# rwl/CSparse.py

Hardware: AMD Instinct MI355X
Metric: cs_gaxpy achieved HBM GB/s (algorithmic bytes / time), 5M x 5M CSC, 64 nnz/col (higher is better)
Workload: dtype f64; 1 GPU; cs_gaxpy y += A x on G-rand: 5000000 x 5000000 CSC, 64 distinct rows per column drawn uniformly from [0, n), ascending (SURVEY 8d), int32 indices, fp64 values; one independent matrix per GPU; row_draw=uniform, n=5000000, nnz=320000000, kernel=gaxpy_tiled, plan_key_bytes=3, parallelism=independent matrices, 1 per GPU, no data-path collective

## Files before the change

### csparse.py_amd/_csx.py

```python
import ctypes as C
import os

import numpy as np

_HERE = os.path.dirname(os.path.abspath(__file__))
LIB_PATH = os.environ.get("CSX_LIB") or os.path.join(_HERE, "libcsx.so")

OK, EINVAL, EZEROPIVOT, ENOTSPD, ERUNTIME = 0, 1, 2, 3, 4
TRI_L, TRI_LT, TRI_U, TRI_UT = 0, 1, 2, 3
GAXPY_AUTO, GAXPY_EXACT, GAXPY_WAVE, GAXPY_TILED, GAXPY_ATOMIC = 0, 1, 2, 3, 4

H = C.c_uint64
_i32p = C.POINTER(C.c_int32)
_f64p = C.POINTER(C.c_double)
_vp = C.c_void_p

_PROTOS = {
    "csx_init": [C.c_int],
    "csx_finalize": [],
    "csx_sync": [],
    "csx_set_stream": [_vp],
    "csx_device_info": [C.c_char_p, C.c_int, C.POINTER(C.c_int), C.POINTER(C.c_int64)],
    "csx_compress": [C.c_int32, C.c_int32, C.c_int64, _i32p, _i32p, _f64p, C.POINTER(H)],
    "csx_add": [H, H, C.c_double, C.c_double, C.POINTER(H)],
    "csx_dupl": [H, C.POINTER(H)],
    "csx_drop": [H, C.c_int, C.c_double, C.POINTER(H)],
    "csx_permute": [H, _i32p, _i32p, C.c_int, C.POINTER(H)],
    "csx_symperm": [H, _i32p, C.c_int, C.POINTER(H)],
    "csx_schol": [H, _i32p, _i32p],
    "csx_order_nd_host": [C.c_int32, _i32p, _i32p, _i32p],
    "csx_norm1": [H, _f64p],
    "csx_cholsol_set_order": [H, C.c_int],
    "csx_cholsol_growth": [H, _f64p],
    "csx_cholsol_sn_info": [H, _i32p, _i32p, _i32p, _i32p, _f64p],
    "csx_cholsol_sn_geometry": [H, C.POINTER(C.c_int64), C.c_int32, _i32p],
    "csx_cholsol_sn_launches": [H, C.POINTER(C.c_int64), C.c_int32, _i32p],
    "csx_csc_invalidate": [H],
    "csx_set_option": [C.c_char_p, C.c_int],
    "csx_get_option": [C.c_char_p, C.POINTER(C.c_int)],
    "csx_gaxpy_host": [C.c_int32, C.c_int32, _i32p, _i32p, _f64p, _f64p, _f64p],
    "csx_csc_col_block": [H, C.c_int32, C.c_int32, C.POINTER(H)],
    "csx_mem_trim": [],
    "csx_mem_info": [C.POINTER(C.c_int64), C.POINTER(C.c_int64), C.POINTER(C.c_int64)],
    "csx_timer_start": [],
    "csx_timer_stop": [_f64p],
    "csx_csc_upload": [C.c_int32, C.c_int32, _i32p, _i32p, _f64p, C.POINTER(H)],
    "csx_csc_alloc": [C.c_int32, C.c_int32, C.c_int32, C.c_int, C.POINTER(H)],
    "csx_csc_wrap": [C.c_int32, C.c_int32, C.c_int32, _vp, _vp, _vp, C.POINTER(H)],
    "csx_csc_info": [H, _i32p, _i32p, _i32p, C.POINTER(C.c_int)],
    "csx_csc_download": [H, _i32p, _i32p, _f64p],
    "csx_csc_ptrs": [H, C.POINTER(_vp), C.POINTER(_vp), C.POINTER(_vp)],
    "csx_free": [H],
    "csx_vec_alloc": [C.c_int64, C.POINTER(H)],
    "csx_vec_upload": [_f64p, C.c_int64, C.POINTER(H)],
    "csx_vec_wrap": [_vp, C.c_int64, C.POINTER(H)],
    "csx_vec_download": [H, _f64p, C.c_int64],
    "csx_vec_write": [H, _f64p, C.c_int64],
    "csx_vec_fill": [H, C.c_double],
    "csx_vec_copy": [H, H],
    "csx_vec_ptr": [H, C.POINTER(_vp), C.POINTER(C.c_int64)],
    "csx_ivec_upload": [_i32p, C.c_int64, C.POINTER(H)],
    "csx_ivec_download": [H, _i32p, C.c_int64],
    "csx_gaxpy": [H, H, H, C.c_int],
    "csx_gaxpy_prepare": [H, C.c_int],
    "csx_gaxpy_block": [H, H, H, C.c_int32, C.c_int],
    "csx_residual_block": [H, H, H, H, C.c_int32, C.c_int, _f64p, _f64p],
    "csx_residual_host": [C.c_int32, C.c_int32, _i32p, _i32p, _f64p, C.c_int32, C.c_int, _f64p, _f64p, _f64p, _f64p, _f64p],
    "csx_residual_sym_block": [H, H, H, H, C.c_int32, _f64p, _f64p],
    "csx_residual_sym_host": [C.c_int32, _i32p, _i32p, _f64p, C.c_int32, _f64p, _f64p, _f64p, _f64p, _f64p],
    "csx_norm1_sym": [H, _f64p],
    "csx_block_add_cols": [H, H, H, C.c_int64, C.c_int32, _i32p],
    "csx_block_select_cols": [H, H, C.c_int64, C.c_int32, _i32p],
    "csx_transpose": [H, C.c_int, C.POINTER(H)],
    "csx_cumsum": [H, H, C.c_int64, C.POINTER(C.c_int64)],
    "csx_prim_limits": [_i32p],
    "csx_prim_scan": [_i32p, _i32p, C.c_int64, C.c_int, C.POINTER(C.c_int64)],
    "csx_prim_suffix_min": [_i32p, C.c_int64],
    "csx_prim_expand_columns": [_i32p, C.c_int32, C.c_int32, _i32p],
    "csx_prim_boundaries": [_vp, C.c_int64, C.c_int32, _i32p, C.c_int],
    "csx_prim_sort": [_vp, _vp, _f64p, C.c_int64, C.c_uint32, _vp, _vp, _f64p, _i32p, C.c_int32, _i32p, C.c_int32, C.c_int],
    "csx_prim_sort_info": [C.POINTER(C.c_int64), C.c_int32],
    "csx_multiply": [H, H, C.POINTER(H)],
    "csx_spgemm_limits": [_i32p],
    "csx_spgemm_info": [C.POINTER(C.c_int64), C.c_int32, _i32p],
    "csx_tri_analyse": [H, C.c_int, C.POINTER(H)],
    "csx_tri_info": [H, _i32p, _i32p, _i32p],
    "csx_tri_solve": [H, H, C.c_int32],
    "csx_tri_set_order": [H, C.c_int],
    "csx_tri_solve_list": [H, _f64p, C.POINTER(C.c_int)],
    "csx_cholsol_solve_list": [H, _f64p, C.POINTER(C.c_int)],
    "csx_tri_order_info": [H, _i32p, _f64p],
    "csx_tri_components": [H, _i32p],
    "csx_tri_limits": [_i32p],
    "csx_tri_route_info": [H, C.c_int32, C.POINTER(C.c_int64), C.c_int32, _i32p],
    "csx_tri_launches": [H, C.POINTER(C.c_int64), C.c_int32, _i32p],
    "csx_cholsol_tri_route_info": [H, C.c_int, C.c_int32, C.POINTER(C.c_int64), C.c_int32, _i32p],
    "csx_cholsol_tri_launches": [H, C.c_int, C.POINTER(C.c_int64), C.c_int32, _i32p],
    "csx_permute_vec": [H, H, H, C.c_int32, C.c_int32, C.c_int],
    "csx_lusol_solve": [H, H, H, H, H, H, C.c_int32, C.POINTER(C.c_int)],
    "csx_lusol_solve_trans": [H, H, H, H, H, H, C.c_int32, C.POINTER(C.c_int)],
    "csx_schol_host": [C.c_int32, _i32p, _i32p, _i32p, _i32p],
    "csx_counts_host": [C.c_int32, C.c_int32, _i32p, _i32p, _i32p, _i32p, C.c_int, _i32p],
    "csx_chol": [H, _i32p, _i32p, _i32p, C.POINTER(H)],
    "csx_chol_info": [_i32p, _f64p],
    "csx_cholsol_plan": [H, _i32p, C.POINTER(H)],
    "csx_cholsol_factor": [H, C.c_int, C.POINTER(H), C.POINTER(H)],
    "csx_cholsol_factor_info": [C.POINTER(C.c_int32), C.POINTER(C.c_double), C.POINTER(C.c_double), C.POINTER(C.c_double)],
    "csx_cholsol_solve": [H, H, C.c_int32],
    "csx_cholsol_graph_info": [H, _i32p, _f64p],
    "csx_cholsol_info": [H, _i32p, _i32p, _i32p],
    "csx_qr_host": [C.c_int32, C.c_int32, C.c_int32, _i32p, _i32p, _f64p, _i32p, _i32p, _i32p, _i32p, C.c_int32, C.c_int32,
                    _i32p, _i32p, _f64p, _i32p, _i32p, _f64p, _f64p],
    "csx_qr_apply_host": [C.c_int32, _i32p, _i32p, _f64p, _f64p, C.c_int, _f64p],
    "csx_lu_blocks": [H, C.c_double, C.POINTER(H), C.POINTER(H), _i32p, C.POINTER(C.c_int)],
    "csx_block_limits": [_i32p],
    "csx_prim_components": [C.c_int32, _i32p, _i32p, C.c_int, C.c_int, C.c_int, _i32p, _vp, _i32p, _i32p, _i32p, _i32p, _i32p,
                            C.POINTER(C.c_int)],
    "csx_lu_etree": [H, C.c_double, C.POINTER(H), C.POINTER(H), _i32p, C.POINTER(C.c_int)],
    "csx_updown": [H, C.c_int, C.c_int32, _i32p, _f64p, _i32p, C.POINTER(C.c_int)],
    "csx_updown_block": [H, H, _i32p, _i32p, C.c_int, _i32p],
    "csx_updown_block_info": [_i32p, _i32p, _i32p, _f64p],
    "csx_updown_block_classes": [_i32p, _i32p],
    "csx_chol_inverse": [H, C.POINTER(H)],
    "csx_chol_inverse_info": [_i32p, _i32p, C.POINTER(C.c_int64), _f64p],
    "csx_csc_diag": [H, H],
    "csx_ldl_inverse": [H, H, C.POINTER(H)],
    "csx_slu_inverse": [H, H, C.POINTER(H), C.POINTER(H)],
    "csx_inverse_at": [H, H, H, H, C.c_int64, _i32p, _i32p, H, C.POINTER(C.c_int64)],
    "csx_spsolve": [H, H, _i32p, C.c_int, C.c_int, C.POINTER(H)],
    "csx_happly": [H, H, H, C.c_int32, C.c_int],
    "csx_sqr_host": [C.c_int32, C.c_int32, _i32p, _i32p, _i32p, _i32p, _i32p, _i32p, C.POINTER(C.c_int32),
                     C.POINTER(C.c_int64), C.POINTER(C.c_int64)],
    "csx_qr_blocks": [H, _i32p, _i32p, _i32p, C.c_int32, C.POINTER(H), C.POINTER(H), _f64p, C.POINTER(C.c_int)],
    "csx_gaxpy_plan_info": [H, C.POINTER(C.c_int), C.POINTER(C.c_int), C.POINTER(C.c_int)],
    "csx_gaxpy_plan_shape": [H, C.POINTER(C.c_int), C.POINTER(C.c_double)],
    "csx_gaxpy_plan_geometry": [H, C.POINTER(C.c_int64)],
    "csx_gaxpy_plan_groups": [H, _i32p],
    "csx_lu_host": [C.c_int32, _i32p, _i32p, _f64p, C.c_double, C.POINTER(_i32p), C.POINTER(_i32p),
                    C.POINTER(_f64p), C.POINTER(_i32p), C.POINTER(_i32p), C.POINTER(_f64p), _i32p],
    "csx_comm_unique_id": [C.POINTER(C.c_uint8)],
    "csx_comm_init": [C.c_int, C.c_int, C.POINTER(C.c_uint8)],
    "csx_comm_finalize": [],
    "csx_comm_info": [C.POINTER(C.c_int), C.POINTER(C.c_int), C.POINTER(C.c_int)],
    "csx_comm_barrier": [],
    "csx_comm_allreduce_host": [_f64p, C.c_int, C.c_int],
    "csx_comm_bcast_host": [_vp, C.c_int64, C.c_int],
    "csx_comm_bcast_csc": [C.POINTER(H), C.c_int],
    "csx_comm_bcast_vec": [H, C.c_int],
    "csx_comm_reduce_scatter_vec": [H, H],
    "csx_comm_allreduce_vec": [H],
    "csx_comm_scatter_blocks": [H, H, C.c_int64, C.c_int],
    "csx_comm_gather_blocks": [H, H, C.c_int64, C.c_int],
    "csx_block_cols": [H, C.c_int64, C.c_int32, C.c_int32, C.c_int32, H, C.c_int],
    "csx_gaxpy_sharded_plan": [H, C.POINTER(H)],
    "csx_gaxpy_sharded_rows": [H, _i32p, _i32p],
    "csx_gaxpy_sharded": [H, H, H, C.c_int],
    "csx_gaxpy_sharded_plan_for": [H, C.c_int, C.POINTER(H)],
    "csx_gaxpy_sharded_piece": [H, C.c_int, H],
    "csx_gaxpy_sharded_buffers": [H, C.POINTER(_vp), C.POINTER(_vp), C.POINTER(C.c_int64)],
    "csx_gaxpy_sharded_sum": [H, C.c_int, C.c_int, H],
    "csx_maxtrans": [H, C.c_int64, _i32p, _i32p],
    "csx_scc": [H, _i32p, _i32p, _i32p],
    "csx_dmperm": [H, C.c_int64, _i32p, _i32p, _i32p, _i32p, _i32p, _i32p, _i32p],
    "csx_dmperm_times": [_f64p],
    "csx_dmperm_rounds": [C.POINTER(C.c_int64)],
    "csx_btf_split": [H, _i32p, _i32p, _i32p, C.c_int32, _i32p, _i32p, _i32p, _i32p, _i32p, C.POINTER(H), C.POINTER(H)],
    "csx_btf_plan": [H, H, H, _i32p, _i32p, _i32p, _i32p, _i32p, C.c_int32, C.POINTER(H)],
    "csx_btf_solve": [H, H, H, C.c_int32],
    "csx_btf_solve_trans": [H, H, H, C.c_int32],
    "csx_btf_info": [H, C.POINTER(C.c_int64)],
    "csx_btf_limits": [_i32p],
    "csx_btf_refactor": [H, H, H, H, C.POINTER(C.c_int), _f64p, C.POINTER(C.c_int64)],
    "csx_btf_refactor_dx": [H, _f64p],
    "csx_lu_refactor_plan": [H, H, H, _i32p, _i32p, C.POINTER(H)],
    "csx_lu_refactor": [H, H, C.POINTER(C.c_int), _f64p, C.POINTER(C.c_int64)],
    "csx_chol_refactor_plan": [H, H, _i32p, C.POINTER(H)],
    "csx_chol_refactor": [H, H, C.POINTER(C.c_int), _i32p],
    "csx_chol_refactor_info": [C.POINTER(C.c_double), C.POINTER(C.c_double)],
    "csx_chol_refactor_window": [H, C.POINTER(C.c_int32)],
    "csx_chol_limits": [_i32p],
    "csx_cholsol_forest_plan": [C.c_int, C.c_int32, C.c_int32, C.c_int, C.c_int, C.POINTER(C.c_int32)],
    "csx_lu_refactor_host": [C.c_int32, _i32p, _i32p, _f64p, _i32p, _i32p, _i32p, _f64p, _i32p, _i32p, _f64p,
                             C.POINTER(C.c_int), _f64p],
    "csx_assemble_plan_host": [C.c_int32, C.c_int32, C.c_int64, _i32p, _i32p, _i32p, _i32p, _i32p, _i32p, _i32p],
    "csx_assemble_host": [C.c_int32, _i32p, _i32p, _f64p, _f64p],
    "csx_assemble_plan": [C.c_int32, C.c_int32, C.c_int64, _i32p, _i32p, C.POINTER(H)],
    "csx_assemble_matrix": [H, H, C.POINTER(H)],
    "csx_assemble": [H, H, H],
    "csx_assemble_plan_info": [H, C.POINTER(C.c_int64)],
    "csx_assemble_pullback": [H, H, H],
    "csx_assemble_pullback_host": [C.c_int32, C.c_int64, _i32p, _i32p, _f64p, _f64p],
    "csx_pattern_outer": [H, H, H, C.c_int32, C.c_int, C.c_double, H],
    "csx_pattern_outer_host": [C.c_int32, C.c_int32, _i32p, _i32p, C.c_int32, C.c_int, C.c_double, _f64p, _f64p, _f64p],
    "csx_pattern_outer_limits": [C.POINTER(C.c_int64)],
    "csx_multiply_plan_count": [C.c_int32, C.c_int32, C.c_int32, _i32p, _i32p, _i32p, _i32p, C.POINTER(C.c_int64),
                                C.POINTER(C.c_int64)],
    "csx_multiply_plan_host": [C.c_int32, C.c_int32, C.c_int32, _i32p, _i32p, _i32p, _i32p, _i32p, _i32p, _i32p, _i32p],
    "csx_multiply_fold_host": [C.c_int32, _i32p, _i32p, _f64p, _f64p, _f64p],
    "csx_multiply_plan": [H, H, C.POINTER(H)],
    "csx_multiply_plan_matrix": [H, H, H, H, C.POINTER(H)],
    "csx_multiply_plan_run": [H, H, H, H, H],
    "csx_multiply_plan_info": [H, C.POINTER(C.c_int64)],
    "csx_add_plan_host": [C.c_int32, C.c_int32, C.c_int32, C.POINTER(_i32p), C.POINTER(_i32p), _i32p, _i32p, _i32p, _i32p, _i32p],
    "csx_add_fold_host": [C.c_int32, C.c_int32, _i32p, _i32p, _i32p, _f64p, C.POINTER(_f64p), _f64p],
    "csx_add_plan": [C.c_int32, C.POINTER(H), C.POINTER(H)],
    "csx_add_plan_matrix": [H, _f64p, C.POINTER(H), C.POINTER(H)],
    "csx_add_plan_run": [H, _f64p, C.POINTER(H), H],
    "csx_add_plan_info": [H, C.POINTER(C.c_int64)],
    "csx_ldl_factor": [H, _i32p, _i32p, _i32p, C.c_double, C.POINTER(H), C.POINTER(C.c_int)],
    "csx_ldl_refactor": [H, H, C.c_double, C.POINTER(C.c_int)],
    "csx_ldl_parts": [H, C.POINTER(H), C.POINTER(H)],
    "csx_ldl_info": [H, C.POINTER(C.c_int64)],
    "csx_ldl_stats": [H, _f64p],
    "csx_ldl_window": [C.POINTER(C.c_int32)],
    "csx_block_div_rows": [H, H, C.c_int64, C.c_int32],
    "csx_ldl_host": [C.c_int32, _i32p, _i32p, _f64p, _i32p, _i32p, _i32p, C.c_double, _f64p, _f64p, C.POINTER(C.c_int64)],
    "csx_schur_factor": [H, _i32p, _i32p, _i32p, C.c_int32, C.c_double, C.POINTER(H), C.POINTER(C.c_int)],
    "csx_schur_refactor": [H, H, C.c_double, C.POINTER(C.c_int)],
    "csx_schur_parts": [H, C.POINTER(H), C.POINTER(H), C.POINTER(H)],
    "csx_schur_info": [H, C.POINTER(C.c_int64)],
    "csx_schur_stats": [H, _f64p],
    "csx_schur_host": [C.c_int32, _i32p, _i32p, _f64p, _i32p, _i32p, _i32p, C.c_int32, C.c_double, _f64p, _f64p, _f64p,
                       C.POINTER(C.c_int64)],
    "csx_slu_factor": [H, _i32p, _i32p, _i32p, _i32p, C.c_double, C.POINTER(H), C.POINTER(C.c_int)],
    "csx_slu_refactor": [H, H, C.c_double, C.POINTER(C.c_int)],
    "csx_slu_parts": [H, C.POINTER(H), C.POINTER(H)],
    "csx_slu_info": [H, C.POINTER(C.c_int64)],
    "csx_slu_stats": [H, _f64p],
    "csx_slu_window": [C.POINTER(C.c_int32), C.POINTER(C.c_int32)],
    "csx_slu_host": [C.c_int32, _i32p, _i32p, _f64p, _i32p, _i32p, _i32p, _i32p, C.c_double, _f64p, _f64p, C.POINTER(C.c_int64)],
    "csx_slu_batch_factor": [H, H, C.c_int32, _f64p, C.POINTER(H), C.POINTER(C.c_int)],
    "csx_slu_batch_refactor": [H, H, _f64p, C.POINTER(C.c_int)],
    "csx_slu_batch_norm1": [H, H, C.c_int32, _f64p],
    "csx_slu_batch_solve": [H, H, C.c_int32, C.c_int],
    "csx_slu_batch_info": [H, C.POINTER(C.c_int64), C.POINTER(C.c_int64)],
    "csx_slu_batch_stats": [H, _f64p],
    "csx_slu_batch_member": [H, C.c_int32, _f64p, _f64p],
    "csx_slu_batch_limits": [_i32p],
    "csx_ldl_batch_factor": [H, H, C.c_int32, _f64p, C.POINTER(H), C.POINTER(C.c_int)],
    "csx_ldl_batch_refactor": [H, H, _f64p, C.POINTER(C.c_int)],
    "csx_ldl_batch_norm1": [H, H, C.c_int32, _f64p],
    "csx_ldl_batch_solve": [H, H, C.c_int32],
    "csx_ldl_batch_info": [H, C.POINTER(C.c_int64), C.POINTER(C.c_int64)],
    "csx_ldl_batch_stats": [H, _f64p],
    "csx_ldl_batch_member": [H, C.c_int32, _f64p, _f64p],
    "csx_ldl_batch_d": [H, _f64p],
    "csx_ldl_batch_limits": [_i32p],
    "csx_hqr_symbolic_host": [C.c_int32, C.c_int32, C.c_int32, _i32p, _i32p, _i32p, _i32p, _i32p, _i32p, C.c_int32, C.c_int32,
                              _i32p, _i32p, _i32p, _i32p],
    "csx_hqr_host": [C.c_int32, C.c_int32, C.c_int32, _i32p, _i32p, _f64p, _i32p, _i32p, _i32p, _i32p, C.c_int32, C.c_int32,
                     _i32p, _i32p, _f64p, _i32p, _i32p, _f64p, _f64p],
    "csx_hqr_factor": [H, _i32p, _i32p, _i32p, _i32p, C.c_int32, C.POINTER(H), C.POINTER(C.c_int)],
    "csx_hqr_refactor": [H, H, C.POINTER(C.c_int)],
    "csx_hqr_parts": [H, C.POINTER(H), C.POINTER(H), C.POINTER(H)],
    "csx_hqr_info": [H, C.POINTER(C.c_int64)],
    "csx_hqr_stats": [H, _f64p],
    "csx_hqr_window": [C.POINTER(C.c_int32), C.POINTER(C.c_int32)],
    "csx_level_schedule": [C.c_int32, _i32p, C.c_int32, C.c_int32, C.POINTER(C.c_int64), C.c_int64, _i32p, C.POINTER(C.c_int32)],
    "csx_gmres_limits": [_i32p],
    "csx_gs_work_len": [C.c_int64, C.c_int32, C.c_int32, C.POINTER(C.c_int64)],
    "csx_gs_project": [H, C.c_int32, H, H, C.c_int64, C.c_int32, _i32p, C.c_int, _f64p],
    "csx_gs_update": [H, C.c_int32, H, H, C.c_int64, C.c_int32, _i32p, C.c_int, _f64p, _f64p],
    "csx_gs_scale": [H, H, C.c_int32, H, C.c_int64, C.c_int32, _i32p, _f64p],
    "csx_gs_combine": [H, C.c_int32, H, H, C.c_int64, C.c_int32, _i32p, _f64p, _i32p],
    "csx_gs_host": [C.c_int, C.c_int64, C.c_int32, C.c_int32, _f64p, _f64p, _i32p, C.c_int, _f64p, _i32p, _f64p],
    "csx_bgs_limits": [_i32p],
    "csx_bgs_work_len": [C.c_int64, C.c_int32, C.c_int32, C.c_int32, C.POINTER(C.c_int64)],
    "csx_bgs_gram": [H, C.c_int32, C.c_int32, H, C.c_int32, H, C.c_int64, C.c_int, _f64p],
    "csx_bgs_update": [H, C.c_int32, C.c_int32, H, C.c_int32, H, C.c_int64, _f64p],
    "csx_bgs_combine": [H, C.c_int32, C.c_int32, H, C.c_int32, H, C.c_int64, _f64p],
    "csx_bgs_host": [C.c_int, C.c_int64, C.c_int32, C.c_int32, C.c_int32, _f64p, _f64p, C.c_int, _f64p, _f64p],
    "csx_gen_grand": [C.c_int32, C.c_int32, C.c_uint64, C.POINTER(H)],
    "csx_gen_grand_uniform": [C.c_int32, C.c_int32, C.c_uint64, C.POINTER(H)],
    "csx_gen_gspd": [C.c_int32, C.c_int32, C.c_uint64, C.POINTER(H)],
    "csx_gen_vec": [C.c_int64, C.c_uint64, C.c_double, C.c_double, C.POINTER(H)],
    "csx_gen_rhs": [C.c_int32, C.c_int32, C.c_int32, C.POINTER(H)],
}

_lib = None
_ready = False


class CsxError(RuntimeError):
    pass


class NotPositiveDefinite(ArithmeticError):
    pass


def _share_torch_hip_runtime():
    import sys
    if "torch" in sys.modules:
        return "torch (already imported)"
    want = os.environ.get("CSX_SHARE_TORCH_HIP")
    if want == "0" or (want is None and (int(os.environ.get("WORLD_SIZE", "1")) <= 1
                                         or os.environ.get("CSX_COMM_BACKEND") != "gloo")):
        return None
    import importlib.util
    spec = importlib.util.find_spec("torch")
    if spec is None or not spec.origin:
        return None
    path = os.path.join(os.path.dirname(spec.origin), "lib", "libamdhip64.so")
    if not os.path.exists(path):
        return None
    C.CDLL(path, mode=C.RTLD_GLOBAL)
    return path


HIP_RUNTIME = None


def load():
    global _lib, HIP_RUNTIME
    if _lib is None:
        if not os.path.exists(LIB_PATH):
            raise ImportError("libcsx.so is not built: run `python csparse.py_amd/build.py` "
                              "(hipcc --offload-arch=gfx950); there is no CPU fallback")
        HIP_RUNTIME = _share_torch_hip_runtime()
        lib = C.CDLL(LIB_PATH)
        for name, args in _PROTOS.items():
            fn = getattr(lib, name)
            fn.argtypes = args
            fn.restype = C.c_int
        lib.csx_last_error.restype = C.c_char_p
        lib.csx_last_error.argtypes = []
        lib.csx_host_free.restype = None
        lib.csx_host_free.argtypes = [_vp]
        _lib = lib
    return _lib


def ldl_window():
    out = C.c_int32(0)
    check(load().csx_ldl_window(C.byref(out)), "csx_ldl_window")
    return out.value


_CHOL_LIMITS = ("CH_ACC", "CH_NARROW", "CH_SMALL_TREE", "CD_MAX", "CC_ACC", "CC_MAP", "CC_RUN_MIN", "CC_RUN_MAX", "CC_WAVES",
                "SN_MIN_WIDTH")


def chol_limits():
    out = (C.c_int32 * 16)()
    check(load().csx_chol_limits(out), "csx_chol_limits")
    d = {name: int(out[k]) for k, name in enumerate(_CHOL_LIMITS)}
    d["windows"] = tuple(int(out[k]) for k in range(10, 15))
    d["max_need"] = int(out[15])
    return d


FOREST_PLAN_KINDS = ("General", "EmitEqual", "Programs", "BlockListExact", "EmitRagged", "BlockListLite")


def cholsol_forest_plan(sparse, min_bs, max_bs, exact, dense_blocks):
    kind = C.c_int32(-1)
    check(load().csx_cholsol_forest_plan(int(sparse), min_bs, max_bs, int(exact), int(dense_blocks), C.byref(kind)),
          "csx_cholsol_forest_plan")
    return FOREST_PLAN_KINDS[kind.value]


def slu_window():
    a, b = C.c_int32(0), C.c_int32(0)
    check(load().csx_slu_window(C.byref(a), C.byref(b)), "csx_slu_window")
    return a.value, b.value


SLU_BATCH_LIMITS = ("MAX_MEMBERS", "WALK_WAVES", "SOLVE_THREADS", "SOLVE_FETCH", "RUN_WAVES", "RUN_FETCH")


def slu_batch_limits():
    out = (C.c_int32 * len(SLU_BATCH_LIMITS))()
    check(load().csx_slu_batch_limits(out), "csx_slu_batch_limits")
    return {name: int(out[k]) for k, name in enumerate(SLU_BATCH_LIMITS)}


def ldl_batch_limits():
    out = (C.c_int32 * len(SLU_BATCH_LIMITS))()
    check(load().csx_ldl_batch_limits(out), "csx_ldl_batch_limits")
    return {name: int(out[k]) for k, name in enumerate(SLU_BATCH_LIMITS)}


def hqr_window():
    a, b = C.c_int32(0), C.c_int32(0)
    check(load().csx_hqr_window(C.byref(a), C.byref(b)), "csx_hqr_window")
    return a.value, b.value


def level_schedule(level_ptr, waves, run_levels, work=None, run_work=0):
    lp = i32(level_ptr)
    nlev = len(lp) - 1
    out, count = np.zeros(3 * max(nlev, 1), np.int32), C.c_int32(0)
    w = None if work is None else np.ascontiguousarray(work, np.int64)
    check(load().csx_level_schedule(nlev, pi(lp), waves, run_levels, None if w is None else w.ctypes.data_as(C.POINTER(C.c_int64)),
                                    run_work, pi(out), C.byref(count)), "csx_level_schedule")
    return [(bool(out[3 * t]), int(out[3 * t + 1]), int(out[3 * t + 2])) for t in range(count.value)]


SN_GEOMETRY_PLAN = ("chunk", "has_relaxed", "matrix_cores", "leaf_subtrees", "leaf_cols", "leaf_tasks", "leaf_slots",
                    "fundamental", "relaxed")
SN_GEOMETRY_DIR = ("steps", "tasks", "max_step_tasks", "cut_lines", "slots", "narrow", "medium", "wide", "one_triangle_steps")
SN_LAUNCHES = ("outside_wg", "outside", "thin1", "thin2", "thin4", "thin8", "thin16", "thin32", "combine", "mfma_w128",
               "mfma_leaf_ct1", "mfma_leaf_ct4", "mfma_ct1", "mfma_ct4", "tri16", "tri32", "tri64", "leaf", "use0")


def _sn_fields(fn, plan, what):
    n = C.c_int32(0)
    check(fn(plan, None, 0, C.byref(n)), what)
    out = (C.c_int64 * n.value)()
    check(fn(plan, out, n.value, C.byref(n)), what)
    return list(out)


def cholsol_sn_geometry(plan):
    v = _sn_fields(lib().csx_cholsol_sn_geometry, plan, "csx_cholsol_sn_geometry")
    a, b = len(SN_GEOMETRY_PLAN), len(SN_GEOMETRY_DIR)
    assert len(v) == a + 2 * b
    g = dict(zip(SN_GEOMETRY_PLAN, v[:a]))
    g["fwd"] = dict(zip(SN_GEOMETRY_DIR, v[a:a + b]))
    g["bwd"] = dict(zip(SN_GEOMETRY_DIR, v[a + b:]))
    return g


def cholsol_sn_launches(plan):
    v = _sn_fields(lib().csx_cholsol_sn_launches, plan, "csx_cholsol_sn_launches")
    k = len(SN_LAUNCHES)
    assert len(v) == 2 * k
    return {"fwd": dict(zip(SN_LAUNCHES, v[:k])), "bwd": dict(zip(SN_LAUNCHES, v[k:]))}


TRI_LIMITS = ("NARROW", "CHB", "CH_SUF", "TRW_MIN_ROW", "TRW_MAX_RHS", "TR64_MIN_RHS", "TR64_RUN", "TR64_RUN_MIN", "TC_MAX_N",
              "TC_THREADS", "COMP_MIN_COUNT", "COMP_MAX_ROWS", "PUSH_MAX_RHS", "FEW_MAX_RHS", "FEW_CPW", "COMP_LDS_MAX", "FEW_TILE_LDS",
              "WINDOW_LDS_MAX", "COLUMNS_LDS_MAX", "CHAIN_LINKS_NUM", "CHAIN_LINKS_DEN", "CHAIN_LEVELS_NUM", "WCOL_WIDE_ENTRIES",
              "WCHAIN_WIDE_ENTRIES", "WINDOW_SLACK", "STRIP_SHORT_COLS", "TL_WAVES_MAX", "LV_MAX_ROUNDS", "LV_DEVICE_MIN_TERMS",
              "LAUNCH_COUNTERS")
TRI_ROUTES = ("Ragged", "CompPush", "FewLds", "Few", "Local", "WColumns", "WColChain", "Columns", "ColChain", "Sequential", "Levels")
TRI_ROUTE_INFO = ("route", "lds", "grid", "G", "waves", "tile_rows", "chunks", "window", "threads", "rounds", "mate",
                  "band", "links", "col_state", "levels", "sequential", "chain_ok", "ncomp", "comp_max", "push_terms", "few_cpw",
                  "few_rows", "few_terms", "guard", "schedule", "comps_found", "comp_rows_found", "kind", "n", "terms")
TRI_LAUNCHES = ("level", "levels_one_wg", "chain", "sequential", "local_fwd", "local_bwd", "few_fwd", "few_bwd", "few_lds_fwd",
                "few_lds_bwd", "push_fwd", "push_bwd", "ragged", "columns_l", "columns_u", "colchain_lt", "colchain_ut",
                "wcolumns_256", "wcolumns_1024", "wcolchain_lt_2", "wcolchain_lt_12", "wcolchain_ut_2", "wcolchain_ut_12",
                "level_rows", "run_prefix_rows", "levels_rows_one_wg", "level_rows64", "run_prefix64", "levels_rows64_one_wg",
                "level_of")


def tri_limits():
    out = (C.c_int32 * 32)()
    check(load().csx_tri_limits(out), "csx_tri_limits")
    return {name: int(out[k]) for k, name in enumerate(TRI_LIMITS)}


def tri_route_info(plan, nrhs, cholsol=None):
    if cholsol is None:
        v = _sn_fields(lambda h, out, cap, n: lib().csx_tri_route_info(h, nrhs, out, cap, n), plan, "csx_tri_route_info")
    else:
        v = _sn_fields(lambda h, out, cap, n: lib().csx_cholsol_tri_route_info(h, cholsol, nrhs, out, cap, n), plan,
                       "csx_cholsol_tri_route_info")
    assert len(v) == len(TRI_ROUTE_INFO)
    d = dict(zip(TRI_ROUTE_INFO, v))
    d["route"] = TRI_ROUTES[d["route"]]
    return d


def tri_launches(plan, cholsol=None):
    if cholsol is None:
        v = _sn_fields(lib().csx_tri_launches, plan, "csx_tri_launches")
    else:
        v = _sn_fields(lambda h, out, cap, n: lib().csx_cholsol_tri_launches(h, cholsol, out, cap, n), plan,
                       "csx_cholsol_tri_launches")
    assert len(v) == len(TRI_LAUNCHES)
    return {k: c for k, c in zip(TRI_LAUNCHES, v) if c}


PRIM_LIMITS = ("SCAN_TILE", "SM_TILE", "RS_TILE", "RS_BINS", "RS_DESC_STARTS", "RS_SEGS", "RS_CHUNK_MIN", "RS_CHUNK_DIV",
               "EXPAND_GRID_MAX")
SORT_INSTANCES = ("none", "keys", "a", "v", "av_flat_flat", "av_flat_packed", "av_packed_packed", "av_packed_flat", "short_first",
                  "short_middle", "short_last")
SORT_INFO = ("bits", "passes", "widths", "nblocks", "chunk", "nchunks", "packed", "k16", "key_misalign", "instances", "count")


def prim_limits():
    out = (C.c_int32 * len(PRIM_LIMITS))()
    check(load().csx_prim_limits(out), "csx_prim_limits")
    return {name: int(out[k]) for k, name in enumerate(PRIM_LIMITS)}


SPGEMM_LIMITS = ("SG_SEG", "SG_THREADS", "SG_DENSE_MAX", "SG_GLOBAL_WGS", "SG_HASH_MAXP", "HASH_LIMIT0", "HASH_LIMIT1", "HASH_LIMIT2",
                 "HASH_LIMIT3", "HASH_LIMIT4", "HASH_LIMIT5", "HASH_LIMIT6", "HASH_LIMIT7", "H2_MAXSEG", "H2_MAXLEN", "H2_MAXP",
                 "H1_SEG", "H1_MAXP", "H1_UN", "SGO_MAX", "SGO_SLOTS0", "SGO_CNT0", "SGO_SLOTS1", "SGO_CNT1", "SGO_SLOTS2", "SGO_CNT2",
                 "SGO_DENSE_WAVES", "SG_GRID_PER_CU", "INFO_FIELDS", "SGO_WAVES0", "SGO_WAVES1", "SGO_WAVES2", "SG_UN",
                 "SG_MIN_SLOTS", "SG_LDS_BUDGET", "SG_WGS_PER_CU_MAX", "SG_HASH_BINS", "SG_NARROW_BINS", "LAUNCH_SITES")
SPGEMM_SITES = (("products",) + tuple("spgemm_%s_%s" % (r, k) for r in ("symbolic", "values", "pattern")
                                      for k in ("dense", "hash", "global"))
                + tuple("hash1_%s_%d" % (v, b) for v in ("pattern", "values") for b in range(8))
                + tuple("hash2_%s_%d" % (v, b) for v in ("pattern", "values") for b in range(6))
                + ("compact", "dup_cols", "ordered2_0", "ordered2_1", "ordered2_2", "ordered_dense"))


def spgemm_limits():
    out = (C.c_int32 * 40)()
    check(load().csx_spgemm_limits(out), "csx_spgemm_limits")
    return {name: int(out[k]) for k, name in enumerate(SPGEMM_LIMITS)}


def spgemm_info():
    n = C.c_int32(0)
    out = (C.c_int64 * 256)()
    check(load().csx_spgemm_info(out, 256, C.byref(n)), "csx_spgemm_info")
    v, k = [int(x) for x in out[:n.value]], len(SPGEMM_SITES)
    assert n.value == 40 + 2 * k
    cnt, grid = v[40:40 + k], v[40 + k:]
    return {"bins": tuple(v[:32]), "one_pass": v[32], "global_wgs": v[33], "cus": v[34], "ordered": v[35], "classes": tuple(v[36:40]),
            "launches": {s: c for s, c in zip(SPGEMM_SITES, cnt) if c},
            "grids": {s: g for s, c, g in zip(SPGEMM_SITES, cnt, grid) if c}}


GMRES_LIMITS = ("GS_CHUNK", "GS_FAN", "GS_GROUP", "GS_TILE")
GS_PROJECT, GS_UPDATE, GS_SCALE, GS_COMBINE = 0, 1, 2, 3


def gmres_limits():
    out = (C.c_int32 * len(GMRES_LIMITS))()
    check(load().csx_gmres_limits(out), "csx_gmres_limits")
    return {name: int(out[k]) for k, name in enumerate(GMRES_LIMITS)}


def gs_work_len(rows, nrhs, nblocks):
    out = C.c_int64(0)
    check(load().csx_gs_work_len(rows, nrhs, nblocks, C.byref(out)), "csx_gs_work_len")
    return out.value


def gs_host(op, V, W, mask, coef=None, length=None, negate=False, nv=None):
    V = np.array(V, dtype=np.float64)
    nb, rows, k = V.shape
    nv = nb if nv is None else nv
    W = None if W is None else np.array(W, dtype=np.float64).reshape(rows, k)
    m = i32(mask)
    cf = None if coef is None else f64(coef)
    ln = None if length is None else i32(length)
    out = {GS_PROJECT: np.full((nv, k), np.nan), GS_UPDATE: np.full(k, np.nan), GS_SCALE: None,
           GS_COMBINE: np.full((rows, k), np.nan)}[op]
    check(load().csx_gs_host(op, rows, k, nv, pd(V), pd(W), pi(m), 1 if negate else 0, pd(cf), pi(ln), pd(out)), "csx_gs_host")
    return {GS_PROJECT: out, GS_UPDATE: (W, out), GS_SCALE: V, GS_COMBINE: out}[op]


PATTERN_OUTER_LIMITS = ("PO_LANES", "PO_CHUNK", "PO_WAVE_CHUNK", "PO_FLIGHT", "PO_KEPT")


def pattern_outer_limits():
    out = (C.c_int64 * len(PATTERN_OUTER_LIMITS))()
    check(load().csx_pattern_outer_limits(out), "csx_pattern_outer_limits")
    return {name: int(out[k]) for k, name in enumerate(PATTERN_OUTER_LIMITS)}


def pattern_outer_host(m, n, p, i, U, V, nrhs, alpha=1.0, sym=False):
    p, i = i32(p), i32(i)
    U, V = f64(np.asarray(U, dtype=np.float64).reshape(-1)), f64(np.asarray(V, dtype=np.float64).reshape(-1))
    out = np.full(max(int(p[n]), 1), np.nan)
    check(load().csx_pattern_outer_host(m, n, pi(p), pi(i), nrhs, 1 if sym else 0, float(alpha), pd(U), pd(V), pd(out)),
          "csx_pattern_outer_host")
    return out[:int(p[n])]


def assemble_pullback_host(sp, src, g):
    sp, src, g = i32(sp), i32(src), f64(g)
    nnz, nz = len(sp) - 1, len(src)
    out = np.full(max(nz, 1), np.nan)
    check(load().csx_assemble_pullback_host(nnz, nz, pi(sp), pi(src), pd(g), pd(out)), "csx_assemble_pullback_host")
    return out[:nz]


BGS_LIMITS = ("GS_CHUNK", "GS_FAN", "BGS_MAXW", "BGS_GROUP", "BGS_TILE")
BGS_GRAM, BGS_UPDATE, BGS_COMBINE = 0, 1, 2


def bgs_limits():
    out = (C.c_int32 * len(BGS_LIMITS))()
    check(load().csx_bgs_limits(out), "csx_bgs_limits")
    return {name: int(out[k]) for k, name in enumerate(BGS_LIMITS)}


def bgs_work_len(rows, b, q, nblocks):
    out = C.c_int64(0)
    check(load().csx_bgs_work_len(rows, b, q, nblocks, C.byref(out)), "csx_bgs_work_len")
    return out.value


def bgs_host(op, V, W=None, coef=None, negate=False, q=None):
    V = np.array(V, dtype=np.float64)
    nv, rows, b = V.shape
    W = None if W is None else np.array(W, dtype=np.float64)
    W = W[:, None] if W is not None and W.ndim == 1 else W
    cf = None if coef is None else f64(coef)
    q = W.shape[1] if W is not None else (int(q) if q is not None else cf.shape[-1])
    out = {BGS_GRAM: np.full((nv, b, q), np.nan), BGS_UPDATE: None, BGS_COMBINE: np.full((rows, q), np.nan)}[op]
    check(load().csx_bgs_host(op, rows, b, q, nv, pd(V), pd(W), 1 if negate else 0, pd(cf), pd(out)), "csx_bgs_host")
    return W if op == BGS_UPDATE else out


def _u32(a):
    return None if a is None else np.array(a, dtype=np.uint32)


def _vptr(a):
    return None if a is None else a.ctypes.data_as(_vp)


def prim_scan(values, in_place=False):
    a = np.array(values, dtype=np.int32)
    out, total = np.full(len(a) + 1, -1, np.int32), C.c_int64(-1)
    check(lib().csx_prim_scan(pi(a), pi(out), len(a), 1 if in_place else 0, C.byref(total)), "csx_prim_scan")
    return out, total.value, (None if in_place else a)


def prim_suffix_min(values):
    p = np.array(values, dtype=np.int32)
    check(lib().csx_prim_suffix_min(pi(p), len(p)), "csx_prim_suffix_min")
    return p


def prim_expand_columns(Ap, fill=-1):
    p = np.array(Ap, dtype=np.int32)
    col = np.full(int(p[-1]), fill, np.int32)
    check(lib().csx_prim_expand_columns(pi(p), len(p) - 1, len(col), pi(col)), "csx_prim_expand_columns")
    return col, p


def prim_boundaries(sorted_key, nkeys, misalign_words=0, fill=-1):
    k = _u32(sorted_key)
    ptr = np.full(nkeys + 1, fill, np.int32)
    check(lib().csx_prim_boundaries(_vptr(k), len(k), nkeys, pi(ptr), misalign_words), "csx_prim_boundaries")
    return ptr, k


def prim_sort(key, a=None, v=None, key_limit=0xFFFFFFFF, want_key=True, expand_ptr=None, nkeys=None, misalign_words=0):
    k, aa = _u32(key), _u32(a)
    vv = None if v is None else np.array(v, dtype=np.float64)
    xp = None if expand_ptr is None else np.array(expand_ptr, dtype=np.int32)
    n = len(k)
    ok = np.full(n, 0xDEADBEEF, np.uint32) if want_key else None
    oa = np.full(n, 0xDEADBEEF, np.uint32) if (aa is not None or xp is not None) else None
    ov = np.full(n, -777.0, np.float64) if vv is not None else None
    op = np.full(nkeys + 1, -1, np.int32) if nkeys is not None else None
    check(lib().csx_prim_sort(_vptr(k), _vptr(aa), pd(vv), n, key_limit, _vptr(ok), _vptr(oa), pd(ov), pi(xp),
                              0 if xp is None else len(xp) - 1, pi(op), 0 if nkeys is None else nkeys, misalign_words),
          "csx_prim_sort")
    return {"out_key": ok, "out_a": oa, "out_v": ov, "out_ptr": op, "key": k, "a": aa, "v": vv, "expand_ptr": xp}


def prim_sort_info():
    out = (C.c_int64 * 17)()
    check(load().csx_prim_sort_info(out, 17), "csx_prim_sort_info")
    v = [int(x) for x in out]
    passes = v[1]
    return {"bits": v[0], "passes": passes, "widths": tuple(v[2:2 + passes]), "nblocks": v[6], "chunk": v[7], "nchunks": v[8],
            "packed": v[9], "k16": v[10], "key_misalign": v[11], "instances": tuple(SORT_INSTANCES[i] for i in v[12:12 + passes]),
            "count": v[16]}


BLOCK_LIMITS = ("LU_MAX_M", "LU_MIN_COMPONENTS", "QR_MAX_M", "QR_MIN_COMPONENTS", "HAPPLY_MAX_LEVELS")


def block_limits():
    out = (C.c_int32 * len(BLOCK_LIMITS))()
    check(load().csx_block_limits(out), "csx_block_limits")
    return {name: int(out[k]) for k, name in enumerate(BLOCK_LIMITS)}


BTF_LIMITS = ("BTF_SMALL", "RF_MAX", "RF_WAVES", "RHS_TILE", "TERM_CHUNK", "TERM_GROUP")


def btf_limits():
    out = (C.c_int32 * len(BTF_LIMITS))()
    check(load().csx_btf_limits(out), "csx_btf_limits")
    return {name: int(out[k]) for k, name in enumerate(BTF_LIMITS)}


def prim_components(n, p, i, skip_first=0, skip_last=0, order=0):
    pp, ii = np.array(p, dtype=np.int32), np.array(i, dtype=np.int32)
    root, nodes, cop = np.full(n, -7, np.int32), np.full(n, 0xDEADBEEF, np.uint32), np.full(n, -7, np.int32)
    first, count = np.full(n, -7, np.int32), np.full(n, -7, np.int32)
    ncomp, maxc, bad = C.c_int32(-1), C.c_int32(-1), C.c_int(-1)
    check(lib().csx_prim_components(n, pi(pp), pi(ii), skip_first, skip_last, order, pi(root), _vptr(nodes), pi(first), pi(count),
                                    pi(cop), C.byref(ncomp), C.byref(maxc), C.byref(bad)), "csx_prim_components")
    out = {"ncomp": ncomp.value, "maxc": maxc.value, "malformed": bad.value, "p": pp, "i": ii,
           "root": None, "nodes": None, "first": None, "count": None, "comp_of_pos": None}
    if not bad.value:
        out.update(root=root, nodes=nodes, first=first[:ncomp.value], count=count[:ncomp.value], comp_of_pos=cop)
    return out


def exported_symbols():
    return sorted(list(_PROTOS) + ["csx_last_error", "csx_host_free"])


def check(status, what=""):
    if status == OK:
        return
    if status == EZEROPIVOT:
        raise ZeroDivisionError("float division by zero")
    if status == ENOTSPD:
        raise NotPositiveDefinite(what or "matrix is not positive definite")
    if status == EINVAL:
        raise ValueError("libcsx: bad argument" + (" in " + what if what else ""))
    raise CsxError("libcsx %s: %s" % (what, load().csx_last_error().decode("utf-8", "replace")))


def init(device=None):
    global _ready
    lib = load()
    if not _ready:
        if device is None:
            device = int(os.environ.get("CSX_DEVICE", os.environ.get("LOCAL_RANK", "0")))
        st = lib.csx_init(int(device))
        if st != OK:
            raise CsxError("csx_init(%d) failed: %s -- the MI355X path has no CPU fallback"
                           % (device, lib.csx_last_error().decode("utf-8", "replace")))
        _ready = True
    return lib


def lib():
    return init()


def i32(a):
    return np.ascontiguousarray(a, dtype=np.int32)


def f64(a):
    return np.ascontiguousarray(a, dtype=np.float64)


def pi(a):
    return None if a is None else a.ctypes.data_as(_i32p)


def pd(a):
    return None if a is None else a.ctypes.data_as(_f64p)


def new_handle():
    return H(0)


def free(h):
    if h and _lib is not None and _ready:
        _lib.csx_free(h)


def sync():
    check(lib().csx_sync(), "csx_sync")


def device_info():
    name = C.create_string_buffer(256)
    cus = C.c_int(0)
    mem = C.c_int64(0)
    check(lib().csx_device_info(name, 256, C.byref(cus), C.byref(mem)), "csx_device_info")
    return name.value.decode(), cus.value, mem.value


class option(object):

    def __init__(self, name, value):
        self.name, self.value = name.encode(), int(value)

    def __enter__(self):
        old = C.c_int(0)
        check(lib().csx_get_option(self.name, C.byref(old)), "csx_get_option")
        self.old = old.value
        check(lib().csx_set_option(self.name, self.value), "csx_set_option")
        return self

    def __exit__(self, *exc):
        check(lib().csx_set_option(self.name, self.old), "csx_set_option")
        return False


class Timer(object):

    def __enter__(self):
        check(lib().csx_timer_start(), "csx_timer_start")
        self.ms = None
        return self

    def __exit__(self, *exc):
        ms = C.c_double(0.0)
        check(lib().csx_timer_stop(C.byref(ms)), "csx_timer_stop")
        self.ms = ms.value
        return False
```

### csparse.py_amd/csrc/csx_gaxpy_tiled.hip

```cpp
#include <cstdint>
#include <cstdlib>

#include "csx_internal.h"

namespace csx {

constexpr int TL_WAVES = 4, TL_NG = 5;
constexpr int TL_GROUP = 256;
constexpr int TL_LDS_BYTES = 160 * 1024 - 256;
constexpr int TL_LDS_ROWS = TL_LDS_BYTES / 8 - 2;
typedef uint32_t u32x4 __attribute__((ext_vector_type(4)));
typedef uint32_t u32x3 __attribute__((ext_vector_type(3)));
typedef u32x3 u32x3_a4 __attribute__((aligned(4)));
typedef double f64x2 __attribute__((ext_vector_type(2)));

__global__ __launch_bounds__(256) void k_tile_keys(int64_t nnz, const int32_t *__restrict__ Ai,
                                                   const int32_t *__restrict__ col, int rb_bits, int32_t row_block,
                                                   int32_t slab_cols, int32_t nslab, uint32_t *__restrict__ tile_id,
                                                   uint32_t *__restrict__ packed) {
    int64_t p = (int64_t)blockIdx.x * blockDim.x + threadIdx.x;
    if (p >= nnz) return;
    const uint32_t i = (uint32_t)Ai[p], j = (uint32_t)col[p];
    const uint32_t s = j / (uint32_t)slab_cols, lc = j - s * (uint32_t)slab_cols;
    const uint32_t b = i / (uint32_t)row_block, lr = i - b * (uint32_t)row_block;
    tile_id[p] = b * (uint32_t)nslab + s;
    packed[p] = (lc << rb_bits) | lr;
}

__global__ __launch_bounds__(256) void k_padded_lengths(int64_t ntiles, const int32_t *__restrict__ sptr,
                                                        int32_t *__restrict__ ngroups) {
    int64_t t = (int64_t)blockIdx.x * blockDim.x + threadIdx.x;
    if (t < ntiles) ngroups[t] = (sptr[t + 1] - sptr[t] + TL_GROUP - 1) / TL_GROUP;
}

__global__ __launch_bounds__(256) void k_group_info(int64_t ntiles, int32_t nslab, const int32_t *__restrict__ sptr,
                                                    const int32_t *__restrict__ gptr, uint32_t *__restrict__ info) {
    int64_t t = (int64_t)blockIdx.x * blockDim.x + threadIdx.x;
    if (t >= ntiles) return;
    const int32_t len = sptr[t + 1] - sptr[t];
    const uint32_t slab = (uint32_t)(t % nslab);
    int32_t g = gptr[t];
    for (int32_t left = len; left > 0; left -= TL_GROUP, g++) info[g] = (slab << 9) | (uint32_t)min(left, TL_GROUP);
}

__global__ __launch_bounds__(256) void k_interleave(int64_t nnz, const uint32_t *__restrict__ stid,
                                                    const int32_t *__restrict__ sptr, const int32_t *__restrict__ gptr,
                                                    const uint32_t *__restrict__ skey, const double *__restrict__ sval,
                                                    uint32_t *__restrict__ okey, double *__restrict__ oval) {
    int64_t q = (int64_t)blockIdx.x * blockDim.x + threadIdx.x;
    if (q >= nnz) return;
    const uint32_t t = stid[q];
    const int32_t e = (int32_t)(q - sptr[t]);
    const int32_t g = e / TL_GROUP, w = e % TL_GROUP;
    const int64_t gbase = ((int64_t)gptr[t] + g) * TL_GROUP;
    const int l = w & 63, k = w >> 6;
    if (okey) okey[gbase + l * 4 + k] = skey[q];
    oval[gbase + (k >> 1) * 128 + l * 2 + (k & 1)] = sval[q];
}

__global__ __launch_bounds__(256) void k_run_span(int64_t nnz, const uint32_t *__restrict__ stid,
                                                  const int32_t *__restrict__ sptr, const uint32_t *__restrict__ skey,
                                                  int rb_bits, int *too_wide) {
    int64_t q = (int64_t)blockIdx.x * blockDim.x + threadIdx.x;
    if (q >= nnz) return;
    const int32_t e = (int32_t)(q - sptr[stid[q]]);
    const int64_t first = q - (e & 63);
    if ((skey[q] >> rb_bits) - (skey[first] >> rb_bits) >= 512u) *too_wide = 1;
}

__global__ __launch_bounds__(256) void k_interleave24(int64_t nnz, const uint32_t *__restrict__ stid,
                                                      const int32_t *__restrict__ sptr, const int32_t *__restrict__ gptr,
                                                      const uint32_t *__restrict__ skey, int rb_bits,
                                                      uint8_t *__restrict__ okey, uint32_t *__restrict__ obase) {
    int64_t q = (int64_t)blockIdx.x * blockDim.x + threadIdx.x;
    if (q >= nnz) return;
    const uint32_t t = stid[q];
    const int32_t e = (int32_t)(q - sptr[t]);
    const int32_t g = e / TL_GROUP, w = e % TL_GROUP;
    const int l = w & 63, k = w >> 6;
    const uint32_t rmask = (1u << rb_bits) - 1u;
    const uint32_t col = skey[q] >> rb_bits, col0 = skey[q - l] >> rb_bits;
    const uint32_t v = (skey[q] & rmask) | ((col - col0) << 15);
    const int64_t gg = (int64_t)gptr[t] + g;
    uint8_t *o = okey + gg * (TL_GROUP * 3) + l * 12 + k * 3;
    o[0] = (uint8_t)v;
    o[1] = (uint8_t)(v >> 8);
    o[2] = (uint8_t)(v >> 16);
    if (l == 0) obase[gg * 4 + k] = col;
}

__global__ __launch_bounds__(256) void k_fill_key24(uint8_t *p, int64_t nslots, uint32_t v) {
    int64_t i = (int64_t)blockIdx.x * blockDim.x + threadIdx.x;
    const int64_t stride = (int64_t)gridDim.x * blockDim.x;
    for (; i < nslots; i += stride) {
        p[3 * i] = (uint8_t)v;
        p[3 * i + 1] = (uint8_t)(v >> 8);
        p[3 * i + 2] = (uint8_t)(v >> 16);
    }
}

__global__ __launch_bounds__(256) void k_fill_keys(uint32_t *p, int64_t n, uint32_t v) {
    int64_t i = (int64_t)blockIdx.x * blockDim.x + threadIdx.x;
    const int64_t stride = (int64_t)gridDim.x * blockDim.x;
    for (; i < n; i += stride) p[i] = v;
}

struct KeyRegs {
    u32x4 kk;
    u32x4 base;
    uint32_t info;
};
struct ValRegs {
    f64x2 v0, v1;
};

constexpr int TP_KEYS2 = 1;
constexpr int TP_FULLSTEP = 2;
constexpr int TP_KEY12 = 4;
constexpr int TP_BULKTILE = 8;
constexpr int TP_ALL = 15;

template <bool NT, bool K24, bool KEY12>
__device__ __forceinline__ KeyRegs load_keys_t(const uint32_t *__restrict__ key, const uint32_t *__restrict__ info,
                                               const uint32_t *__restrict__ base, int32_t g, int lane) {
    KeyRegs r;
    if (K24) {
        const uint32_t *kp = key + (int64_t)g * (TL_GROUP * 3 / 4) + 3 * lane;
        if (KEY12) {
            const u32x3 k = __builtin_nontemporal_load(reinterpret_cast<const u32x3_a4 *>(kp));
            r.kk.x = k.x;
            r.kk.y = k.y;
            r.kk.z = k.z;
        } else {
            r.kk.x = __builtin_nontemporal_load(kp);
            r.kk.y = __builtin_nontemporal_load(kp + 1);
            r.kk.z = __builtin_nontemporal_load(kp + 2);
        }
        r.kk.w = 0;
        r.base = *reinterpret_cast<const u32x4 *>(base + 4 * (int64_t)g);
    } else {
        const uint32_t *kp = key + (int64_t)g * TL_GROUP + 4 * lane;
        r.kk = NT ? __builtin_nontemporal_load(reinterpret_cast<const u32x4 *>(kp)) : *reinterpret_cast<const u32x4 *>(kp);
        r.base = u32x4{0, 0, 0, 0};
    }
    r.info = info[g];
    return r;
}

template <bool NT>
__device__ __forceinline__ ValRegs load_vals_t(const double *__restrict__ val, int32_t g, int lane) {
    ValRegs r;
    const f64x2 *vp = reinterpret_cast<const f64x2 *>(val + (int64_t)g * TL_GROUP + 2 * lane);
    r.v0 = NT ? __builtin_nontemporal_load(vp) : *vp;
    r.v1 = NT ? __builtin_nontemporal_load(vp + 64) : vp[64];
    return r;
}

template <bool K24>
__device__ __forceinline__ u32x4 unpack_keys(const KeyRegs &k) {
    if (!K24) return k.kk;
    const uint32_t ka = k.kk.x, kb = k.kk.y, kc = k.kk.z;
    u32x4 r;
    r.x = ka & 0xFFFFFFu;
    r.y = (ka >> 24) | ((kb & 0xFFFFu) << 8);
    r.z = (kb >> 16) | ((kc & 0xFFu) << 16);
    r.w = kc >> 8;
    return r;
}

template <int HOW>
__device__ __forceinline__ double load_x(const double *p) {
    if (HOW == 1) return __hip_atomic_load(p, __ATOMIC_RELAXED, __HIP_MEMORY_SCOPE_AGENT);
    if (HOW == 2) return __builtin_nontemporal_load(p);
    return *p;
}

constexpr int tile_batch(int threads) { return threads > 256 ? 4 : 8; }

template <int T>
__device__ __forceinline__ void tile_fill(double *ytile, const double *__restrict__ src, int32_t rows) {
    constexpr int NB = tile_batch(T);
    const int tid = threadIdx.x;
    const int32_t head = (rows > 0 && (reinterpret_cast<uintptr_t>(src) & 8)) ? 1 : 0;
    const int32_t npairs = (rows - head) >> 1;
    const f64x2 *s2 = reinterpret_cast<const f64x2 *>(src + head);
    double *d = ytile + head;
    for (int32_t p0 = 0; p0 < npairs; p0 += NB * T) {
        f64x2 v[NB];
        int32_t q[NB];
#pragma unroll
        for (int i = 0; i < NB; i++) {
            const int32_t p = p0 + i * T + tid;
            q[i] = p < npairs ? p : npairs - 1;
            v[i] = s2[q[i]];
        }
#pragma unroll
        for (int i = 0; i < NB; i++) {
            d[2 * q[i]] = v[i].x;
            d[2 * q[i] + 1] = v[i].y;
        }
    }
    if (tid == 0 && head) ytile[0] = src[0];
    if (tid == T - 1 && ((rows - head) & 1)) ytile[rows - 1] = src[rows - 1];
}

template <int T>
__device__ __forceinline__ void tile_drain(const double *ytile, double *__restrict__ dst, int32_t rows) {
    const int tid = threadIdx.x;
    const int32_t head = (rows > 0 && (reinterpret_cast<uintptr_t>(dst) & 8)) ? 1 : 0;
    const int32_t npairs = (rows - head) >> 1;
    f64x2 *d2 = reinterpret_cast<f64x2 *>(dst + head);
    const double *s = ytile + head;
    constexpr int NB = tile_batch(T);
    for (int32_t p0 = 0; p0 < npairs; p0 += NB * T) {
        f64x2 v[NB];
        int32_t q[NB];
#pragma unroll
        for (int i = 0; i < NB; i++) {
            const int32_t p = p0 + i * T + tid;
            q[i] = p < npairs ? p : npairs - 1;
            v[i].x = s[2 * q[i]];
            v[i].y = s[2 * q[i] + 1];
        }
#pragma unroll
        for (int i = 0; i < NB; i++) d2[q[i]] = v[i];
    }
    if (tid == 0 && head) dst[0] = ytile[0];
    if (tid == T - 1 && ((rows - head) & 1)) dst[rows - 1] = ytile[rows - 1];
}

template <int VARIANT, int NW, int NG, bool K24, int PARTS>
struct TiledStep {
    static constexpr bool GATHER = !(VARIANT & 1) || VARIANT >= 5, ATOMIC = VARIANT != 3;
    static constexpr bool STREAM_NT = VARIANT != 2;
    static constexpr uint32_t CMASK = VARIANT == 5 ? 32767u : (VARIANT == 4 ? 255u : 0xffffffffu);
    static constexpr int XLOAD = VARIANT == 6 ? 1 : 0;
    static constexpr bool RING = VARIANT == 7;
    static constexpr int KD = (PARTS & TP_KEYS2) ? 2 : 1;
    static constexpr int NK = KD + 1;
    static constexpr int PERIOD = NK == 3 ? 6 : 2;
    static constexpr int STRIDE = NG * NW;

    static __device__ __forceinline__ int32_t clamp_group(int32_t gq, int32_t g0, int32_t gend, int32_t wave_s, int32_t wave_v) {
        int32_t gg = gq < gend ? gq : gend - 1;
        if (RING) gg = g0 + ((gg - g0) & 31);
        return gg - wave_s + wave_v;
    }
    static __device__ __forceinline__ void load_key_set(KeyRegs (&r)[NG], const uint32_t *__restrict__ key,
                                                        const uint32_t *__restrict__ info, const uint32_t *__restrict__ base,
                                                        int32_t g, int32_t g0, int32_t gend, int32_t wave_s, int32_t wave_v,
                                                        int lane) {
#pragma unroll
        for (int j = 0; j < NG; j++)
            r[j] = load_keys_t<STREAM_NT, K24, (PARTS & TP_KEY12) != 0>(key, info, base,
                                                                         clamp_group(g + j * NW, g0, gend, wave_s, wave_v), lane);
    }
    static __device__ __forceinline__ void load_val_set(ValRegs (&r)[NG], const double *__restrict__ val, int32_t g,
                                                        int32_t g0, int32_t gend, int32_t wave_s, int32_t wave_v, int lane) {
#pragma unroll
        for (int j = 0; j < NG; j++)
            r[j] = load_vals_t<STREAM_NT>(val, clamp_group(g + j * NW, g0, gend, wave_s, wave_v), lane);
    }

    template <int P, bool PRED, bool LOADS>
    static __device__ __forceinline__ void step(KeyRegs (&K)[NK][NG], ValRegs (&V)[2][NG], double *ytile,
                                                const uint32_t *__restrict__ key, const double *__restrict__ val,
                                                const uint32_t *__restrict__ info, const uint32_t *__restrict__ base,
                                                const double *__restrict__ x, int32_t g, int32_t g0, int32_t gend,
                                                int32_t wave_s, int32_t wave_v, int lane, int rb_bits, uint32_t rmask,
                                                int32_t slab_cols, double &sink) {
        constexpr int kc = P % NK, kn = (P + KD) % NK, vc = P % 2, vn = (P + 1) % 2;
        const int cshift = K24 ? 15 : rb_bits;
        double xv[NG][4];
        u32x4 kk[NG];
#pragma unroll
        for (int j = 0; j < NG; j++) {
            xv[j][0] = xv[j][1] = xv[j][2] = xv[j][3] = 1.0;
            kk[j] = unpack_keys<K24>(K[kc][j]);
            if (GATHER && (!PRED || j == 0 || g + j * NW < gend)) {
                const double *xs = x + (int64_t)(K[kc][j].info >> 9) * slab_cols;
                const u32x4 b = K[kc][j].base;
                xv[j][0] = load_x<XLOAD>(xs + ((b.x + (kk[j].x >> cshift)) & CMASK));
                xv[j][1] = load_x<XLOAD>(xs + ((b.y + (kk[j].y >> cshift)) & CMASK));
                xv[j][2] = load_x<XLOAD>(xs + ((b.z + (kk[j].z >> cshift)) & CMASK));
                xv[j][3] = load_x<XLOAD>(xs + ((b.w + (kk[j].w >> cshift)) & CMASK));
            }
        }
        if (LOADS) {
            load_key_set(K[kn], key, info, base, g + KD * STRIDE, g0, gend, wave_s, wave_v, lane);
            load_val_set(V[vn], val, g + STRIDE, g0, gend, wave_s, wave_v, lane);
        }
#pragma unroll
        for (int j = 0; j < NG; j++) {
            if (!PRED || j == 0 || g + j * NW < gend) {
                if (ATOMIC) {
                    unsafeAtomicAdd(&ytile[kk[j].x & rmask], V[vc][j].v0.x * xv[j][0]);
                    unsafeAtomicAdd(&ytile[kk[j].y & rmask], V[vc][j].v0.y * xv[j][1]);
                    unsafeAtomicAdd(&ytile[kk[j].z & rmask], V[vc][j].v1.x * xv[j][2]);
                    unsafeAtomicAdd(&ytile[kk[j].w & rmask], V[vc][j].v1.y * xv[j][3]);
                } else {
                    sink += V[vc][j].v0.x * xv[j][0] + V[vc][j].v0.y * xv[j][1] + V[vc][j].v1.x * xv[j][2] +
                            V[vc][j].v1.y * xv[j][3] + (double)((kk[j].x ^ kk[j].y ^ kk[j].z ^ kk[j].w) & 1u);
                }
            }
        }
    }

    template <int P>
    static __device__ __forceinline__ bool advance(KeyRegs (&K)[NK][NG], ValRegs (&V)[2][NG], double *ytile,
                                                   const uint32_t *__restrict__ key, const double *__restrict__ val,
                                                   const uint32_t *__restrict__ info, const uint32_t *__restrict__ base,
                                                   const double *__restrict__ x, int32_t &g, int32_t g0, int32_t gend,
                                                   int32_t wave_s, int32_t wave_v, int lane, int rb_bits, uint32_t rmask,
                                                   int32_t slab_cols, double &sink) {
        if (PARTS & TP_FULLSTEP) {
            if (g + (NG - 1) * NW < gend) {
                step<P, false, true>(K, V, ytile, key, val, info, base, x, g, g0, gend, wave_s, wave_v, lane, rb_bits, rmask,
                                     slab_cols, sink);
            } else {
                step<P, true, false>(K, V, ytile, key, val, info, base, x, g, g0, gend, wave_s, wave_v, lane, rb_bits, rmask,
                                     slab_cols, sink);
                return true;
            }
        } else {
            step<P, true, true>(K, V, ytile, key, val, info, base, x, g, g0, gend, wave_s, wave_v, lane, rb_bits, rmask,
                                slab_cols, sink);
        }
        g += STRIDE;
        return g >= gend;
    }
};

constexpr int tl_parts(bool k24) { return k24 ? TP_FULLSTEP | TP_BULKTILE : 0; }

template <int VARIANT, int NW, int NG, bool K24, int PARTS>
__global__ __launch_bounds__(64 * NW) void k_gaxpy_tiled(const int32_t *__restrict__ rb_gptr,
                                                         const uint32_t *__restrict__ group_info,
                                                         const uint32_t *__restrict__ tile_key,
                                                         const uint32_t *__restrict__ tile_base,
                                                         const double *__restrict__ tile_val,
                                                         const double *__restrict__ x, double *__restrict__ y,
                                                         int32_t m, int32_t nrb, int32_t row_block,
                                                         int32_t slab_cols, int rb_bits) {
    extern __shared__ __attribute__((aligned(16))) double ytile[];
    typedef TiledStep<VARIANT, NW, NG, K24, PARTS> S;
    const uint32_t rmask = K24 ? 0x7FFFu : (1u << rb_bits) - 1u;
    const int lane = threadIdx.x & 63;
    const int32_t wave_v = threadIdx.x >> 6, wave_s = __builtin_amdgcn_readfirstlane(wave_v);
    double sink = 0.0;
    for (int32_t rb = blockIdx.x; rb < nrb; rb += gridDim.x) {
        const int64_t row0 = (int64_t)rb * row_block;
        const int32_t rows = (int32_t)((row0 + row_block <= m) ? row_block : (m - row0));
        const int32_t gend = rb_gptr[rb + 1];
        const int32_t g0 = rb_gptr[rb];
        int32_t g = g0 + wave_s;
        KeyRegs K[S::NK][NG];
        ValRegs V[2][NG];
        if (g < gend) {
#pragma unroll
            for (int d = 0; d < S::KD; d++)
                S::load_key_set(K[d], tile_key, group_info, tile_base, g + d * S::STRIDE, g0, gend, wave_s, wave_v, lane);
            S::load_val_set(V[0], tile_val, g, g0, gend, wave_s, wave_v, lane);
        }
        if (PARTS & TP_BULKTILE) {
            tile_fill<64 * NW>(ytile, y + row0, rows);
        } else {
            for (int k = threadIdx.x; k < rows; k += 64 * NW) ytile[k] = y[row0 + k];
        }
        __syncthreads();
        if (g < gend) {
#define CSX_TILED_ADVANCE(P)                                                                                          \
    if (S::template advance<P>(K, V, ytile, tile_key, tile_val, group_info, tile_base, x, g, g0, gend, wave_s, wave_v, \
                               lane, rb_bits, rmask, slab_cols, sink))                                                 \
        break;
            for (;;) {
                CSX_TILED_ADVANCE(0)
                CSX_TILED_ADVANCE(1)
                if constexpr (S::PERIOD == 6) {
                    CSX_TILED_ADVANCE(2)
                    CSX_TILED_ADVANCE(3)
                    CSX_TILED_ADVANCE(4)
                    CSX_TILED_ADVANCE(5)
                }
            }
#undef CSX_TILED_ADVANCE
        }
        __syncthreads();
        if (!S::ATOMIC && sink == 12345.678) ytile[0] = sink;
        if (PARTS & TP_BULKTILE) {
            tile_drain<64 * NW>(ytile, y + row0, rows);
        } else {
            for (int k = threadIdx.x; k < rows; k += 64 * NW) y[row0 + k] = ytile[k];
        }
        __syncthreads();
    }
}

__global__ __launch_bounds__(256) void k_rb_group_ptr(int32_t nrb, int32_t nslab, const int32_t *__restrict__ gptr,
                                                      int32_t *__restrict__ rb_gptr) {
    int64_t b = (int64_t)blockIdx.x * blockDim.x + threadIdx.x;
    if (b <= nrb) rb_gptr[b] = gptr[(int64_t)b * nslab];
}

static int gaxpy_tiled_pick_shape(Csc *A);

int gaxpy_tiled_prepare(Csc *A) {
    if (A->tiled) return CSX_OK;
    if (!A->x) return CSX_EINVAL;
    hipStream_t s = ctx().stream;
    const int32_t nwg = ctx().cus > 0 ? ctx().cus : 256;
    const int32_t cap = TL_LDS_ROWS;
    int32_t rounds = 1;
    int32_t row_block;
    for (;;) {
        const int64_t nrb_try = (int64_t)nwg * rounds;
        row_block = (int32_t)(((int64_t)A->m + nrb_try - 1) / nrb_try);
        if (row_block <= cap) break;
        rounds++;
    }
    if (row_block < 1) row_block = 1;
    const int32_t nrb = (int32_t)(((int64_t)A->m + row_block - 1) / row_block);
    int rb_bits = 1;
    while ((1 << rb_bits) <= row_block) rb_bits++;
    double slab_kb = 1024.0;
#ifdef CSX_ABLATION
    if (const char *e = std::getenv("CSX_TILED_SLAB_KB")) slab_kb = std::atof(e) >= 8.0 ? std::atof(e) : slab_kb;
#endif
    int64_t slab_cols = (int64_t)(slab_kb * 1024 / 8);
    const int64_t max_cols_key = 1ll << (32 - rb_bits);
    if (slab_cols > max_cols_key) slab_cols = max_cols_key;
    if (slab_cols > A->n) slab_cols = A->n > 0 ? A->n : 1;
    int32_t nslab = (int32_t)(((int64_t)A->n + slab_cols - 1) / slab_cols);
    if (nslab < 1) nslab = 1;
    const int64_t ntiles = (int64_t)nrb * nslab;
    if (ntiles > 0x3fffffffll || nslab >= (1 << 22)) return CSX_EINVAL;

    std::unique_ptr<TiledPlan> t(new TiledPlan());
    t->rb_bits = rb_bits;
    t->row_block = row_block;
    t->nrb = nrb;
    t->nslab = nslab;
    t->slab_cols = (int32_t)slab_cols;
    {
        DevBuf<int32_t> col, sptr, gptr;
        DevBuf<uint32_t> tid, packed, stid, skey;
        DevBuf<double> sval;
        int64_t ngroups = 0;
        CSX_TRY(col.alloc((size_t)A->nnz));
        CSX_TRY(tid.alloc((size_t)A->nnz));
        CSX_TRY(packed.alloc((size_t)A->nnz));
        CSX_TRY(stid.alloc((size_t)A->nnz));
        CSX_TRY(skey.alloc((size_t)A->nnz));
        CSX_TRY(sval.alloc((size_t)A->nnz));
        CSX_TRY(sptr.alloc((size_t)ntiles + 1));
        CSX_TRY(gptr.alloc((size_t)ntiles + 1));
        CSX_TRY(t->tile_ptr.alloc((size_t)nrb + 1));
        CSX_TRY(expand_columns(A->p, A->n, A->nnz, col));
        if (A->nnz > 0) {
            int64_t blocks = ((int64_t)A->nnz + 255) / 256;
            hipLaunchKernelGGL(k_tile_keys, dim3((unsigned)blocks), dim3(256), 0, s, (int64_t)A->nnz, A->i, col, rb_bits,
                               row_block, t->slab_cols, t->nslab, tid, packed);
            CSX_LAUNCH_CHECK();
        }
        CSX_TRY(stable_sort_by_key(tid, packed, A->x, A->nnz, (uint32_t)ntiles, stid, skey, sval));
        CSX_TRY(boundaries_from_sorted(stid, A->nnz, (int32_t)ntiles, sptr));
        const unsigned tb = (unsigned)((ntiles + 256) / 256);
        hipLaunchKernelGGL(k_padded_lengths, dim3(tb), dim3(256), 0, s, ntiles, sptr, gptr);
        CSX_TRY(scan_exclusive_i32(gptr, gptr, ntiles, &ngroups));
        bool k24 = false;
        if (ngroups > 0 && rb_bits <= 15 && ctx().opt.gaxpy_keys24) {
            DevBuf<int> flag;
            int h = 1;
            CSX_TRY(flag.alloc(1));
            (void)hipMemsetAsync(flag, 0, sizeof(int), s);
            hipLaunchKernelGGL(k_run_span, dim3((unsigned)(((int64_t)A->nnz + 255) / 256)), dim3(256), 0, s, (int64_t)A->nnz,
                               stid, sptr, skey, rb_bits, flag);
            CSX_HIP(hipMemcpyAsync(&h, flag, sizeof(int), hipMemcpyDeviceToHost, s));
            CSX_HIP(hipStreamSynchronize(s));
            k24 = h == 0;
        }
        t->ngroups = ngroups;
        CSX_TRY(t->tile_len.alloc((size_t)ngroups));
        if (!k24) CSX_TRY(t->tile_key.alloc((size_t)ngroups * TL_GROUP));
        if (k24) CSX_TRY(t->tile_key24.alloc((size_t)ngroups * TL_GROUP * 3 + 16));
        if (k24) CSX_TRY(t->tile_base.alloc((size_t)ngroups * 4));
        CSX_TRY(t->tile_val.alloc((size_t)ngroups * TL_GROUP));
        if (ngroups > 0) {
            if (k24) {
                hipLaunchKernelGGL(k_fill_key24, dim3(2048), dim3(256), 0, s, t->tile_key24, (int64_t)ngroups * TL_GROUP,
                                   (uint32_t)row_block);
                (void)hipMemsetAsync(t->tile_base, 0, (size_t)ngroups * 4 * sizeof(uint32_t), s);
            } else {
                hipLaunchKernelGGL(k_fill_keys, dim3(2048), dim3(256), 0, s, t->tile_key, (int64_t)ngroups * TL_GROUP,
                                   (uint32_t)row_block);
            }
            (void)hipMemsetAsync(t->tile_val, 0, (size_t)ngroups * TL_GROUP * sizeof(double), s);
            hipLaunchKernelGGL(k_group_info, dim3(tb), dim3(256), 0, s, ntiles, nslab, sptr, gptr, (uint32_t *)t->tile_len.get());
            hipLaunchKernelGGL(k_interleave, dim3((unsigned)(((int64_t)A->nnz + 255) / 256)), dim3(256), 0, s,
                               (int64_t)A->nnz, stid, sptr, gptr, skey, sval, t->tile_key, t->tile_val);
            if (k24)
                hipLaunchKernelGGL(k_interleave24, dim3((unsigned)(((int64_t)A->nnz + 255) / 256)), dim3(256), 0, s,
                                   (int64_t)A->nnz, stid, sptr, gptr, skey, rb_bits, t->tile_key24, t->tile_base);
        }
        hipLaunchKernelGGL(k_rb_group_ptr, dim3((unsigned)((nrb + 256) / 256)), dim3(256), 0, s, nrb, nslab, gptr,
                           t->tile_ptr);
        CSX_LAUNCH_CHECK();
        CSX_HIP(hipStreamSynchronize(s));
    }
    A->tiled = std::move(t);
#ifndef CSX_ABLATION
    if (ctx().opt.gaxpy_tune_shape) CSX_TRY(gaxpy_tiled_pick_shape(A));
#endif
    return CSX_OK;
}

constexpr int TL_NSHAPES = 4;
static int gaxpy_tiled_launch(const Csc *A, const double *x, double *y, int shape);

static int gaxpy_tiled_pick_shape(Csc *A) {
    TiledPlan *t = A->tiled.get();
    if ((int64_t)A->nnz < (int64_t)1 << 24) return CSX_OK;
    hipStream_t s = ctx().stream;
    DevBuf<double> x, y;
    if (x.alloc((size_t)A->n) != CSX_OK || y.alloc((size_t)A->m) != CSX_OK) return CSX_OK;
    CSX_HIP(hipMemsetAsync(x, 0, (size_t)A->n * sizeof(double), s));
    CSX_HIP(hipMemsetAsync(y, 0, (size_t)A->m * sizeof(double), s));
    hipEvent_t e0, e1;
    CSX_HIP(hipEventCreate(&e0));
    CSX_HIP(hipEventCreate(&e1));
    int best = 0;
    int st = CSX_OK;
    for (int round = 0; round < 2 && st == CSX_OK; round++)
        for (int sh = 0; sh < TL_NSHAPES && st == CSX_OK; sh++) {
            if (round == 0) st = gaxpy_tiled_launch(A, x, y, sh);
            if (st != CSX_OK) break;
            (void)hipEventRecord(e0, s);
            for (int rep = 0; rep < 3 && st == CSX_OK; rep++) st = gaxpy_tiled_launch(A, x, y, sh);
            (void)hipEventRecord(e1, s);
            if (hipEventSynchronize(e1) != hipSuccess) st = CSX_ERUNTIME;
            float ms = 0.f;
            (void)hipEventElapsedTime(&ms, e0, e1);
            ms /= 3;
            if (round == 0 || ms < t->shape_ms[sh]) t->shape_ms[sh] = ms;
        }
    (void)hipEventDestroy(e0);
    (void)hipEventDestroy(e1);
    if (st != CSX_OK) return st;
    for (int sh = 1; sh < TL_NSHAPES; sh++)
        if (t->shape_ms[sh] < t->shape_ms[best]) best = sh;
    t->shape = best;
    return CSX_OK;
}

int gaxpy_tiled_shape(const TiledPlan *t) {
    const int forced = ctx().opt.gaxpy_shape;
    if (forced >= 0 && forced < TL_NSHAPES) return forced;
    return t->shape >= 0 && t->shape < TL_NSHAPES ? t->shape : 0;
}

int gaxpy_tiled_run(const Csc *A, const double *x, double *y) {
    return gaxpy_tiled_launch(A, x, y, gaxpy_tiled_shape(A->tiled.get()));
}

int gaxpy_tiled_group_counts(const TiledPlan *t, std::vector<int32_t> &groups) {
    std::vector<int32_t> ptr((size_t)t->nrb + 1);
    hipStream_t s = ctx().stream;
    CSX_HIP(hipMemcpyAsync(ptr.data(), t->tile_ptr, ptr.size() * sizeof(int32_t), hipMemcpyDeviceToHost, s));
    CSX_HIP(hipStreamSynchronize(s));
    groups.resize((size_t)t->nrb);
    for (int32_t b = 0; b < t->nrb; b++) groups[b] = ptr[b + 1] - ptr[b];
    return CSX_OK;
}

template <int V, int NW, int NG, bool K24, int PARTS>
static hipError_t gaxpy_tiled_allow_lds() {
    static int done_on = -1;
    if (done_on == ctx().device) return hipSuccess;
    const hipError_t e = hipFuncSetAttribute(reinterpret_cast<const void *>(&k_gaxpy_tiled<V, NW, NG, K24, PARTS>),
                                             hipFuncAttributeMaxDynamicSharedMemorySize, TL_LDS_BYTES);
    if (e == hipSuccess) done_on = ctx().device;
    return e;
}

static int gaxpy_tiled_launch(const Csc *A, const double *x, double *y, int shape) {
    const TiledPlan *t = A->tiled.get();
    hipStream_t s = ctx().stream;
    const size_t lds = (((size_t)(t->row_block + 1) * sizeof(double)) + 15) & ~(size_t)15;
    const int32_t nwg = ctx().cus > 0 ? ctx().cus : 256;
    const unsigned grid = (unsigned)(t->nrb < nwg ? t->nrb : nwg);
#define CSX_TILED_LAUNCH_K(V, NW, NG, K24, PARTS)                                                                    \
    {                                                                                                                \
        CSX_HIP((gaxpy_tiled_allow_lds<V, NW, NG, K24, PARTS>()));                                                   \
        hipLaunchKernelGGL((k_gaxpy_tiled<V, NW, NG, K24, PARTS>), dim3(grid), dim3(64 * NW), lds, s, t->tile_ptr,   \
                           (const uint32_t *)t->tile_len.get(),                                                      \
                           K24 ? reinterpret_cast<const uint32_t *>(t->tile_key24.get()) : t->tile_key.get(),        \
                           t->tile_base,                                                                             \
                           t->tile_val, x, y, A->m, t->nrb, t->row_block, t->slab_cols, t->rb_bits);                 \
    }
#define CSX_TILED_LAUNCH_P(V, NW, NG, P24, P32)                                                                      \
    {                                                                                                                \
        if (t->tile_key24) CSX_TILED_LAUNCH_K(V, NW, NG, true, P24) else CSX_TILED_LAUNCH_K(V, NW, NG, false, P32)   \
    }
#define CSX_TILED_LAUNCH(V, NW, NG) CSX_TILED_LAUNCH_P(V, NW, NG, tl_parts(true), tl_parts(false))
#ifdef CSX_ABLATION
    int code = 0;
    if (const char *e = std::getenv("CSX_TILED_VARIANT")) code = std::atoi(e);
    const int v = code % 100, nw = (code / 100) % 100 ? (code / 100) % 100 : TL_WAVES, ng = code / 10000 ? code / 10000 : TL_NG;
#define CSX_V(V)                                             \
    if (v == V) {                                            \
        if (nw == 16 && ng == 2) CSX_TILED_LAUNCH(V, 16, 2)  \
        else if (nw == 4 && ng == 5) CSX_TILED_LAUNCH(V, 4, 5) \
        else if (nw == 2 && ng == 10) CSX_TILED_LAUNCH(V, 2, 10) \
        else return CSX_EINVAL;                              \
    } else
#define CSX_OFF(MASK)                                                        \
    if (v == 10 + MASK) {                                                    \
        if (nw == 4 && ng == 5) CSX_TILED_LAUNCH_P(0, 4, 5, TP_ALL & ~(MASK), TP_ALL & ~(MASK)) \
        else return CSX_EINVAL;                                              \
    } else
    if (v == 0) {
        if (nw == 16 && ng == 1) CSX_TILED_LAUNCH(0, 16, 1)
        else if (nw == 16 && ng == 2) CSX_TILED_LAUNCH(0, 16, 2)
        else if (nw == 12 && ng == 2) CSX_TILED_LAUNCH(0, 12, 2)
        else if (nw == 12 && ng == 4) CSX_TILED_LAUNCH(0, 12, 4)
        else if (nw == 8 && ng == 2) CSX_TILED_LAUNCH(0, 8, 2)
        else if (nw == 8 && ng == 3) CSX_TILED_LAUNCH(0, 8, 3)
        else if (nw == 8 && ng == 4) CSX_TILED_LAUNCH(0, 8, 4)
        else if (nw == 4 && ng == 4) CSX_TILED_LAUNCH(0, 4, 4)
        else if (nw == 4 && ng == 5) CSX_TILED_LAUNCH(0, 4, 5)
        else if (nw == 4 && ng == 6) CSX_TILED_LAUNCH(0, 4, 6)
        else if (nw == 2 && ng == 6) CSX_TILED_LAUNCH(0, 2, 6)
        else if (nw == 2 && ng == 7) CSX_TILED_LAUNCH(0, 2, 7)
        else if (nw == 2 && ng == 8) CSX_TILED_LAUNCH(0, 2, 8)
        else if (nw == 2 && ng == 9) CSX_TILED_LAUNCH(0, 2, 9)
        else if (nw == 2 && ng == 10) CSX_TILED_LAUNCH(0, 2, 10)
        else if (nw == 2 && ng == 12) CSX_TILED_LAUNCH(0, 2, 12)
        else if (nw == 1 && ng == 10) CSX_TILED_LAUNCH(0, 1, 10)
        else if (nw == 1 && ng == 12) CSX_TILED_LAUNCH(0, 1, 12)
        else if (nw == 3 && ng == 5) CSX_TILED_LAUNCH(0, 3, 5)
        else if (nw == 3 && ng == 6) CSX_TILED_LAUNCH(0, 3, 6)
        else if (nw == 3 && ng == 7) CSX_TILED_LAUNCH(0, 3, 7)
        else if (nw == 3 && ng == 8) CSX_TILED_LAUNCH(0, 3, 8)
        else if (nw == 5 && ng == 4) CSX_TILED_LAUNCH(0, 5, 4)
        else if (nw == 6 && ng == 3) CSX_TILED_LAUNCH(0, 6, 3)
        else if (nw == 4 && ng == 7) CSX_TILED_LAUNCH(0, 4, 7)
        else return CSX_EINVAL;
    } else
    CSX_V(1) CSX_V(2) CSX_V(3) CSX_V(4) CSX_V(5) CSX_V(6) CSX_V(7)
    CSX_OFF(0) CSX_OFF(1) CSX_OFF(2) CSX_OFF(3) CSX_OFF(4) CSX_OFF(5) CSX_OFF(6) CSX_OFF(7) CSX_OFF(8) CSX_OFF(9)
    CSX_OFF(10) CSX_OFF(11) CSX_OFF(12) CSX_OFF(13) CSX_OFF(14) CSX_OFF(15) return CSX_EINVAL;
#undef CSX_V
#undef CSX_OFF
    (void)shape;
#else
    switch (shape) {
        case 1: CSX_TILED_LAUNCH(0, 2, 10) break;
        case 2: CSX_TILED_LAUNCH(0, 8, 4) break;
        case 3: CSX_TILED_LAUNCH(0, 2, 8) break;
        default: CSX_TILED_LAUNCH(0, TL_WAVES, TL_NG) break;
    }
#endif
#undef CSX_TILED_LAUNCH
#undef CSX_TILED_LAUNCH_P
#undef CSX_TILED_LAUNCH_K
    CSX_LAUNCH_CHECK();
    return CSX_OK;
}

}
```

### csparse.py_amd/csrc/csx_internal.h

```cpp
#pragma once
#include <cstdlib>
#include <hip/hip_runtime.h>

#include <cstdint>
#include <cstdio>
#include <memory>
#include <string>
#include <vector>

#include "../../include/csx.h"

namespace csx {

inline const char *ablation_env(const char *name) {
#ifdef CSX_ABLATION
    return std::getenv(name);
#else
    (void)name;
    return nullptr;
#endif
}


void set_error(const char *fmt, ...);

#define CSX_HIP(call)                                                                      \
    do {                                                                                   \
        hipError_t _e = (call);                                                            \
        if (_e != hipSuccess) {                                                            \
            csx::set_error("%s:%d %s -> %s", __FILE__, __LINE__, #call, hipGetErrorString(_e)); \
            return CSX_ERUNTIME;                                                           \
        }                                                                                  \
    } while (0)

#define CSX_TRY(call)            \
    do {                         \
        int _s = (call);         \
        if (_s != CSX_OK) return _s; \
    } while (0)

#define CSX_LAUNCH_CHECK() CSX_HIP(hipGetLastError())

int dmalloc(void **p, size_t bytes);
template <class T>
inline int dalloc(T **p, size_t count) { return dmalloc((void **)p, count * sizeof(T)); }
void dfree(void *p);
void pool_trim();
void pool_stats(size_t *cached, size_t *live);
void pool_set_limit(size_t bytes);

template <class T>
class DevBuf {
  public:
    DevBuf() = default;
    explicit DevBuf(T *owned) : p_(owned) {}
    DevBuf(const DevBuf &) = delete;
    DevBuf &operator=(const DevBuf &) = delete;
    DevBuf(DevBuf &&o) noexcept : p_(o.release()) {}
    DevBuf &operator=(DevBuf &&o) noexcept {
        if (this != &o) {
            reset();
            p_ = o.release();
        }
        return *this;
    }
    ~DevBuf() { dfree(p_); }
    int alloc(size_t count) {
        reset();
        return dalloc(&p_, count);
    }
    void reset() {
        dfree(p_);
        p_ = nullptr;
    }
    T *get() const { return p_; }
    operator T *() const { return p_; }
    T *release() {
        T *p = p_;
        p_ = nullptr;
        return p;
    }

  private:
    T *p_ = nullptr;
};

enum Kind : int { K_FREE = 0, K_CSC, K_VEC, K_IVEC, K_TRIPLAN, K_CHOLPLAN, K_SHARDPLAN, K_BTFPLAN, K_LUREFPLAN, K_ASMPLAN, K_CHOLREFPLAN, K_MULPLAN, K_ADDPLAN, K_LDLFACTOR, K_SLUFACTOR, K_HQRFACTOR, K_SCHURFACTOR, K_SLUBATCH, K_LDLBATCH };

struct Csc;

struct Gather {
    int32_t rows = 0;
    DevBuf<int32_t> ptr, idx;
    DevBuf<double> val;
};

struct TiledPlan {
    int32_t row_block = 0;
    int32_t nrb = 0;
    int32_t nslab = 0;
    int32_t slab_cols = 0;
    int64_t ngroups = 0;
    DevBuf<int32_t> tile_ptr;
    DevBuf<int32_t> tile_len;
    DevBuf<uint32_t> tile_key;
    DevBuf<double> tile_val;
    int rb_bits = 0;
    DevBuf<uint8_t> tile_key24;
    DevBuf<uint32_t> tile_base;
    int shape = -1;
    float shape_ms[4] = {0, 0, 0, 0};
};

constexpr int32_t HAPPLY_MAX_LEVELS = 4096;
struct HouseLevels {
    int32_t nlevels = 0;
    std::vector<int32_t> ptr;
    DevBuf<int32_t> cols;
};

struct InvSchedule {
    int32_t ndepths = 0;
    int32_t widest = 0;
    int64_t terms = 0;
    std::vector<int32_t> ptr;
    std::vector<int32_t> rows;
    DevBuf<int32_t> cols;
};

struct CliqueForest;

struct Csc {
    Csc();
    ~Csc();
    Csc(const Csc &) = delete;
    Csc &operator=(const Csc &) = delete;
    int32_t m = 0, n = 0, nnz = 0;
    int32_t *p = nullptr;
    int32_t *i = nullptr;
    double *x = nullptr;
    bool owns = true;
    bool trusted = true;
    std::unique_ptr<Gather> rows;
    std::unique_ptr<TiledPlan> tiled;
    std::unique_ptr<HouseLevels> house;
    std::unique_ptr<InvSchedule> inv;
    std::unique_ptr<CliqueForest> clique;
    bool rows_pending = false;
};

struct Vec {
    Vec() = default;
    ~Vec() {
        if (owns) dfree(d);
    }
    Vec(const Vec &) = delete;
    Vec &operator=(const Vec &) = delete;
    int64_t len = 0;
    void *d = nullptr;
    bool owns = true;
};

struct TriPlan;
struct CholPlan;
struct ShardPlan;
struct SnPlan;
struct BtfPlan;
void destroy(TriPlan *p);
void destroy(CholPlan *p);
void destroy(ShardPlan *p);
void destroy(BtfPlan *p);
void destroy(SnPlan *p);
int tri_analyse_raw(const Csc *T, int kind, TriPlan **out);
int tri_solve_raw(TriPlan *P, double *X, int32_t nrhs, bool relaxed);
int tri_solve_host_raw(TriPlan *P, double *x, bool *taken);
int tri_route_info_raw(TriPlan *P, int32_t nrhs, bool relaxed, int64_t *out, int32_t cap, int32_t *count);
int tri_launches_raw(const TriPlan *P, int64_t *out, int32_t cap, int32_t *count);
void tri_set_mate(TriPlan *P, TriPlan *mate);
void tri_set_level_hint(TriPlan *P, std::vector<int32_t> &&level);
void tri_gather_arrays(const TriPlan *P, const int32_t **ptr, const int32_t **idx, const double **val, const double **diag);
struct Refactor;
struct LuRefPlan;
void destroy(Refactor *p);
void destroy(LuRefPlan *p);
struct AsmPlan;
void destroy(AsmPlan *p);
struct MulPlan;
void destroy(MulPlan *p);
struct AddPlan;
void destroy(AddPlan *p);
struct CholAnalysis;
struct CholRefPlan;
void destroy(CholAnalysis *p);
void destroy(CholRefPlan *p);
struct LdlFactor;
void destroy(LdlFactor *p);
struct SluFactor;
void destroy(SluFactor *p);
struct SluBatch;
void destroy(SluBatch *p);
struct LdlBatch;
void destroy(LdlBatch *p);
struct HqrFactor;
void destroy(HqrFactor *p);
int hqr_symbolic(int32_t m, int32_t n, int32_t m2, const int32_t *Ap, const int32_t *Ai, const int32_t *q, const int32_t *parent,
                 const int32_t *pinv, const int32_t *leftmost, std::vector<int32_t> &Vp, std::vector<int32_t> &Vi,
                 std::vector<int32_t> &Rp, std::vector<int32_t> &Ri);

struct Object {
    Kind kind = K_FREE;
    void *ptr = nullptr;
    uint32_t gen = 0;
};

struct Options {
    int chol_band = 1;
    int chol_wband = 1;
    int chol_wband_nb = 16;
    int chol_supernodes = 1;
    int chol_dense_trees = 1;
    int chol_forest = 1;
    int chol_exact = 1;
    int chol_clique = 1;
    int cholsol_dense_blocks = 1;
    int spgemm_one_pass = 1;
    int tri_chain_walker = 1;
    int tri_components = 1;
    int tri_push = 1;
    int tri_columns = 1;
    int gaxpy_keys24 = 1;
    int gaxpy_tune_shape = 0;
    int gaxpy_shape = -1;
    int gaxpy_block_route = 0;
    int tri_row_waves = 1;
    int tri_levels_where = 0;
    int sort_short_keys = 1;
    int tri_host_chains = 0;
    int tri_graph = 2;
    int tri_supernodes = 1;
    int spgemm_ordered = 0;
    int sparseinv_walk = 1;
    int assemble_long = 64;
    int multiply_long = 64;
    int add_long = 64;
    int lu_etree = 0;
};

struct Context {
    Options opt;
    bool ready = false;
    int device = -1;
    hipStream_t own_stream = nullptr;
    hipStream_t stream = nullptr;
    hipStream_t side = nullptr;
    hipEvent_t ev0 = nullptr, ev1 = nullptr;
    int cus = 0;
    std::vector<Object> objects;
};

Context &ctx();
int require_ready();
csx_handle_t put(Kind k, void *ptr);
void *get(csx_handle_t h, Kind k);
int csc_fill_rows(Csc *A);
inline Csc *csc(csx_handle_t h) {
    Csc *A = (Csc *)get(h, K_CSC);
    if (A && A->rows_pending && csc_fill_rows(A) != CSX_OK) return nullptr;
    return A;
}
inline Vec *vec(csx_handle_t h) { return (Vec *)get(h, K_VEC); }
inline Vec *ivec(csx_handle_t h) { return (Vec *)get(h, K_IVEC); }

template <class T>
int upload(DevBuf<T> &d, const T *h, size_t count) {
    CSX_TRY(d.alloc(count));
    if (count) CSX_HIP(hipMemcpyAsync(d.get(), h, count * sizeof(T), hipMemcpyHostToDevice, ctx().stream));
    return CSX_OK;
}
template <class T>
int upload(DevBuf<T> &d, const std::vector<T> &h) { return upload(d, h.data(), h.size()); }
inline int download_i32(std::vector<int32_t> &h, const int32_t *d, size_t count) {
    h.resize(count);
    if (count) CSX_HIP(hipMemcpyAsync(h.data(), d, count * sizeof(int32_t), hipMemcpyDeviceToHost, ctx().stream));
    CSX_HIP(hipStreamSynchronize(ctx().stream));
    return CSX_OK;
}

int sn_build(const Csc *L, const int32_t *parent, const int32_t *Lp_h, const int32_t *Gp_h, const int32_t *Gp, const int32_t *Gi,
             const double *Gx, int32_t col_levels, SnPlan **out);
int sn_solve(SnPlan *P, bool forward, const int32_t *Gp, const int32_t *Gi, const double *Gx, const double *Gd, const Csc *L,
             double *X, int32_t nrhs);
int64_t sn_generation(const SnPlan *P);
int sn_prepare(SnPlan *P, int32_t nrhs);
void sn_info(const SnPlan *P, int32_t *nsn, int32_t *levels, int32_t *max_w);
void sn_info2(const SnPlan *P, int32_t *matrix_cores, double *growth);
int sn_geometry(const SnPlan *P, int64_t *out, int32_t cap);
int sn_launches(const SnPlan *P, int64_t *out, int32_t cap);
bool sn_usable(const SnPlan *P);

int scan_exclusive_i32(const int32_t *in, int32_t *out, int64_t n, int64_t *total_host);
int expand_columns(const int32_t *Ap, int32_t n, int32_t nnz, int32_t *col);
int stable_sort_by_key(const uint32_t *key, const uint32_t *a, const double *v, int64_t count,
                       uint32_t key_limit, uint32_t *out_key, uint32_t *out_a, double *out_v);
struct SortExtra {
    const int32_t *expand_ptr;
    int32_t expand_n;
    int32_t *out_ptr;
    int32_t nkeys;
};
int stable_sort_by_key_ex(const uint32_t *key, const uint32_t *a, const double *v, int64_t count, uint32_t key_limit,
                          uint32_t *out_key, uint32_t *out_a, double *out_v, const SortExtra *ex);
int suffix_min_i32(int32_t *p, int64_t n);
int boundaries_from_sorted(const uint32_t *sorted_key, int64_t count, int32_t nkeys, int32_t *ptr);

int build_row_gather(Csc *A);
int max_partials_host(const uint64_t *part, int64_t count, int32_t width, uint64_t *h);
int csc_validate(Csc *A);
int csc_copy_pattern(int32_t m, int32_t n, int32_t nnz, const int32_t *p, const int32_t *i, bool values,
                     std::unique_ptr<Csc> *out);
int transpose_device(const Csc *A, bool values, Csc *C);
int gaxpy_device(Csc *A, const double *x, double *y, int mode);
int gaxpy_prepare_device(Csc *A, int mode);
int col_block_device(const Csc *A, int32_t first, int32_t count, Csc *C);

constexpr int RF_MAX = 96;
constexpr int RF_WAVES = 4;
int refactor_build(const Csc *A, const int32_t *pinv, const Csc *L, const Csc *U, const std::vector<int32_t> &gid,
                   Refactor **out);
int refactor_run(Refactor *R, const Csc *A, const double *Ax, const Csc *L, const Csc *U, double *Lx, double *Ux, int *ok,
                 double *ratio);
void refactor_counts(const Refactor *R, int64_t *cols);
int rf_gather(int64_t cnt, const int32_t *map, const double *src, double *dst);
int rf_index_copy(const Csc *A, csx_handle_t *out);
int rf_index_map(const double *x, int64_t cnt, DevBuf<int32_t> &map);
int rf_keep_pattern(const Csc *A, DevBuf<int32_t> &p, DevBuf<int32_t> &i);
int rf_differ(int64_t cnt, const int32_t *a, const int32_t *b, int *flag, int *differ, int64_t cnt2 = 0,
              const int32_t *a2 = nullptr, const int32_t *b2 = nullptr);
int rf_values(csx_handle_t A2, int32_t m, int32_t n, int32_t nnz, const int32_t *p0, const int32_t *i0, int *flag,
              const double **x);

int chol_analysis_of_factor(const Csc *A, const int32_t *pinv, const Csc *L, const int32_t *parent_h, const int32_t *Lp_h,
                            CholAnalysis **out, bool *foreign);
int chol_analysis_refactor(CholAnalysis *An, const Csc *L, const double *Ax, double *Lx, hipEvent_t done, bool *notspd);
void chol_analysis_info(const CholAnalysis *An, int32_t *info);
int32_t chol_analysis_window(const CholAnalysis *An);
int chol_scatter(int64_t lnz, const int32_t *win, const double *Ax, double *Lx);
int chol_entry_map(const Csc *A, const int32_t *pinv, const int32_t *Lp, const int32_t *Li, int32_t lnz, int32_t *win, int *bad);
int chol_symbolic_device(const Csc *A, const int32_t *parent, const int32_t *cp, const int32_t *pinv, int32_t **Lp_out,
                         int32_t **Li_out, DevBuf<int32_t> *row_ptr_out, DevBuf<int32_t> *row_col_out, DevBuf<int32_t> *row_pos_out,
                         int32_t *cp_host_out);
int chol_row_view(int32_t n, int64_t lnz, const uint32_t *col, const int32_t *Li, DevBuf<int32_t> *row_ptr, DevBuf<int32_t> *row_col,
                  DevBuf<int32_t> *row_pos);

__device__ __forceinline__ void lds_barrier() { asm volatile("s_waitcnt lgkmcnt(0)\n\ts_barrier" ::: "memory"); }

constexpr int WAVE = 64;

}
```

### csparse.py_amd/csrc/csx_sort.hip

```cpp
#include "csx_internal.h"

namespace csx {

constexpr int SCAN_THREADS = 256;
constexpr int SCAN_ITEMS = 8;
constexpr int SCAN_TILE = SCAN_THREADS * SCAN_ITEMS;

__device__ __forceinline__ int wave_inclusive_scan(int v, int lane) {
#pragma unroll
    for (int d = 1; d < 64; d <<= 1) {
        int t = __shfl_up(v, d, 64);
        if (lane >= d) v += t;
    }
    return v;
}

__device__ __forceinline__ int block_exclusive_scan(int v, int *total) {
    __shared__ int wsum[SCAN_THREADS / 64];
    const int lane = threadIdx.x & 63, w = threadIdx.x >> 6;
    int inc = wave_inclusive_scan(v, lane);
    if (lane == 63) wsum[w] = inc;
    __syncthreads();
    int off = 0, tot = 0;
#pragma unroll
    for (int k = 0; k < SCAN_THREADS / 64; k++) {
        int s = wsum[k];
        if (k < w) off += s;
        tot += s;
    }
    __syncthreads();
    *total = tot;
    return off + inc - v;
}

__global__ __launch_bounds__(SCAN_THREADS) void k_scan_block_sums(const int32_t *in, int64_t n, int32_t *sums) {
    int64_t base = (int64_t)blockIdx.x * SCAN_TILE;
    int acc = 0;
#pragma unroll
    for (int k = 0; k < SCAN_ITEMS; k++) {
        int64_t idx = base + (int64_t)k * SCAN_THREADS + threadIdx.x;
        if (idx < n) acc += in[idx];
    }
    int tot;
    block_exclusive_scan(acc, &tot);
    if (threadIdx.x == 0) sums[blockIdx.x] = tot;
}

__global__ __launch_bounds__(SCAN_THREADS) void k_scan_apply(const int32_t *in, int32_t *out, int64_t n,
                                                             const int32_t *block_off) {
    int64_t base = (int64_t)blockIdx.x * SCAN_TILE + (int64_t)threadIdx.x * SCAN_ITEMS;
    int v[SCAN_ITEMS];
    int acc = 0;
#pragma unroll
    for (int k = 0; k < SCAN_ITEMS; k++) {
        v[k] = (base + k < n) ? in[base + k] : 0;
        acc += v[k];
    }
    int tot;
    int pre = block_exclusive_scan(acc, &tot) + (block_off ? block_off[blockIdx.x] : 0);
#pragma unroll
    for (int k = 0; k < SCAN_ITEMS; k++) {
        if (base + k < n) out[base + k] = pre;
        pre += v[k];
        if (base + k == n - 1) out[n] = pre;
    }
}

__global__ void k_set_i32(int32_t *p, int32_t v) { *p = v; }

int scan_exclusive_i32(const int32_t *in, int32_t *out, int64_t n, int64_t *total_host) {
    hipStream_t s = ctx().stream;
    if (n <= 0) {
        hipLaunchKernelGGL(k_set_i32, dim3(1), dim3(1), 0, s, out, 0);
        CSX_LAUNCH_CHECK();
        if (total_host) *total_host = 0;
        return CSX_OK;
    }
    int64_t nb = (n + SCAN_TILE - 1) / SCAN_TILE;
    DevBuf<int32_t> sums;
    if (nb > 1) {
        CSX_TRY(sums.alloc((size_t)nb + 1));
        hipLaunchKernelGGL(k_scan_block_sums, dim3((unsigned)nb), dim3(SCAN_THREADS), 0, s, in, n, sums);
        CSX_LAUNCH_CHECK();
        CSX_TRY(scan_exclusive_i32(sums, sums, nb, nullptr));
    }
    hipLaunchKernelGGL(k_scan_apply, dim3((unsigned)nb), dim3(SCAN_THREADS), 0, s, in, out, n, sums);
    CSX_LAUNCH_CHECK();
    if (total_host) {
        int32_t t = 0;
        CSX_HIP(hipMemcpyAsync(&t, out + n, sizeof t, hipMemcpyDeviceToHost, s));
        CSX_HIP(hipStreamSynchronize(s));
        *total_host = t;
    }
    return CSX_OK;
}

__global__ __launch_bounds__(256) void k_expand_columns(const int32_t *Ap, int32_t n, int32_t *col) {
    const int lane = threadIdx.x & 63;
    int64_t wave = ((int64_t)blockIdx.x * blockDim.x + threadIdx.x) >> 6;
    int64_t nwaves = ((int64_t)gridDim.x * blockDim.x) >> 6;
    for (int64_t j = wave; j < n; j += nwaves) {
        int32_t b = Ap[j], e = Ap[j + 1];
        for (int32_t p = b + lane; p < e; p += 64) col[p] = (int32_t)j;
    }
}

constexpr int EXPAND_GRID_MAX = 65536;

int expand_columns(const int32_t *Ap, int32_t n, int32_t nnz, int32_t *col) {
    if (n == 0 || nnz == 0) return CSX_OK;
    int64_t blocks = ((int64_t)n + 3) / 4;
    if (blocks > EXPAND_GRID_MAX) blocks = EXPAND_GRID_MAX;
    hipLaunchKernelGGL(k_expand_columns, dim3((unsigned)blocks), dim3(256), 0, ctx().stream, Ap, n, col);
    CSX_LAUNCH_CHECK();
    return CSX_OK;
}

constexpr int RS_THREADS = 256;
constexpr int RS_WAVES = RS_THREADS / 64;
constexpr int RS_ROUNDS = 8;
constexpr int RS_TILE = RS_THREADS * RS_ROUNDS;
constexpr int RS_BINS = 256;

struct __attribute__((packed, aligned(4))) Pay {
    uint32_t a, vlo, vhi;
};

__global__ __launch_bounds__(RS_THREADS) void k_rs_hist(const uint32_t *key, int64_t count, int shift, uint32_t mask,
                                                        int32_t *hist) {
    __shared__ int h[RS_BINS];
    h[threadIdx.x] = 0;
    __syncthreads();
    const int64_t base = (int64_t)blockIdx.x * RS_TILE;
    if (base + RS_TILE <= count && (reinterpret_cast<uintptr_t>(key) & 15) == 0) {
        typedef uint32_t u32x4h __attribute__((ext_vector_type(4)));
        const u32x4h *k4 = reinterpret_cast<const u32x4h *>(key + base);
        u32x4h v[RS_ROUNDS / 4];
#pragma unroll
        for (int r = 0; r < RS_ROUNDS / 4; r++) v[r] = k4[r * RS_THREADS + threadIdx.x];
#pragma unroll
        for (int r = 0; r < RS_ROUNDS / 4; r++) {
            atomicAdd(&h[(v[r].x >> shift) & mask], 1);
            atomicAdd(&h[(v[r].y >> shift) & mask], 1);
            atomicAdd(&h[(v[r].z >> shift) & mask], 1);
            atomicAdd(&h[(v[r].w >> shift) & mask], 1);
        }
    } else {
#pragma unroll 4
        for (int r = 0; r < RS_ROUNDS; r++) {
            int64_t idx = base + (int64_t)r * RS_THREADS + threadIdx.x;
            if (idx < count) atomicAdd(&h[(key[idx] >> shift) & mask], 1);
        }
    }
    __syncthreads();
    hist[(size_t)blockIdx.x * RS_BINS + threadIdx.x] = h[threadIdx.x];
}

__global__ __launch_bounds__(RS_THREADS) void k_rs_hist16(const uint16_t *key, int64_t count, int shift, uint32_t mask,
                                                          int32_t *hist) {
    __shared__ int h[RS_BINS];
    h[threadIdx.x] = 0;
    __syncthreads();
    const int64_t base = (int64_t)blockIdx.x * RS_TILE;
    if (base + RS_TILE <= count && (reinterpret_cast<uintptr_t>(key) & 15) == 0) {
        typedef uint32_t u32x2h __attribute__((ext_vector_type(2)));
        const u32x2h *k2 = reinterpret_cast<const u32x2h *>(key + base);
        u32x2h v[RS_ROUNDS / 4];
#pragma unroll
        for (int r = 0; r < RS_ROUNDS / 4; r++) v[r] = k2[r * RS_THREADS + threadIdx.x];
#pragma unroll
        for (int r = 0; r < RS_ROUNDS / 4; r++) {
            const uint32_t w2[2] = {v[r].x, v[r].y};
#pragma unroll
            for (int q = 0; q < 2; q++) {
                atomicAdd(&h[((w2[q] & 0xffffu) >> shift) & mask], 1);
                atomicAdd(&h[((w2[q] >> 16) >> shift) & mask], 1);
            }
        }
    } else {
#pragma unroll 4
        for (int r = 0; r < RS_ROUNDS; r++) {
            int64_t idx = base + (int64_t)r * RS_THREADS + threadIdx.x;
            if (idx < count) atomicAdd(&h[((uint32_t)key[idx] >> shift) & mask], 1);
        }
    }
    __syncthreads();
    hist[(size_t)blockIdx.x * RS_BINS + threadIdx.x] = h[threadIdx.x];
}

__global__ __launch_bounds__(RS_BINS) void k_rs_colsum(const int32_t *hist, uint32_t nblocks, uint32_t chunk,
                                                       int32_t *part) {
    const uint32_t t0 = blockIdx.x * chunk, t1 = min(t0 + chunk, nblocks);
    int s = 0;
#pragma unroll 8
    for (uint32_t t = t0; t < t1; t++) s += hist[(size_t)t * RS_BINS + threadIdx.x];
    part[(size_t)blockIdx.x * RS_BINS + threadIdx.x] = s;
}

constexpr int RS_SEGS = 4;
__global__ __launch_bounds__(RS_BINS * RS_SEGS) void k_rs_chunkscan(int32_t *part, uint32_t nchunks, int32_t *dbase) {
    __shared__ int segsum[RS_SEGS][RS_BINS];
    const int d = threadIdx.x & (RS_BINS - 1), sg = threadIdx.x / RS_BINS;
    const uint32_t per = (nchunks + RS_SEGS - 1) / RS_SEGS;
    const uint32_t c0 = min(sg * per, nchunks), c1 = min(c0 + per, nchunks);
    int run = 0;
#pragma unroll 8
    for (uint32_t c = c0; c < c1; c++) run += part[(size_t)c * RS_BINS + d];
    segsum[sg][d] = run;
    __syncthreads();
    int before = 0, total = 0;
#pragma unroll
    for (int k = 0; k < RS_SEGS; k++) {
        const int v = segsum[k][d];
        if (k < sg) before += v;
        total += v;
    }
    run = before;
#pragma unroll 8
    for (uint32_t c = c0; c < c1; c++) {
        const int v = part[(size_t)c * RS_BINS + d];
        part[(size_t)c * RS_BINS + d] = run;
        run += v;
    }
    __shared__ int wtot[RS_BINS / 64];
    const int lane = threadIdx.x & 63, w = threadIdx.x >> 6;
    int inc = 0;
    if (sg == 0) {
        inc = wave_inclusive_scan(total, lane);
        if (lane == 63) wtot[w] = inc;
    }
    __syncthreads();
    if (sg == 0) {
        int off = 0;
#pragma unroll
        for (int k = 0; k < RS_BINS / 64; k++)
            if (k < w) off += wtot[k];
        dbase[d] = off + inc - total;
    }
}

__global__ __launch_bounds__(RS_BINS) void k_rs_tileprefix(int32_t *hist, const int32_t *part, const int32_t *dbase,
                                                           uint32_t nblocks, uint32_t chunk) {
    const uint32_t t0 = blockIdx.x * chunk, t1 = min(t0 + chunk, nblocks);
    int run = part[(size_t)blockIdx.x * RS_BINS + threadIdx.x] + dbase[threadIdx.x];
#pragma unroll 8
    for (uint32_t t = t0; t < t1; t++) {
        const int v = hist[(size_t)t * RS_BINS + threadIdx.x];
        hist[(size_t)t * RS_BINS + threadIdx.x] = run;
        run += v;
    }
}

constexpr int RS_DESC_WORDS = 128;
constexpr int RS_DESC_STARTS = (RS_DESC_WORDS - 2) * 2;

__global__ void k_rs_tiledesc_head(const int32_t *Ap, int32_t n, int64_t count, uint32_t nblocks, uint32_t *desc) {
    const uint32_t t = blockIdx.x * blockDim.x + threadIdx.x;
    if (t >= nblocks) return;
    const int64_t tb = (int64_t)t * RS_TILE;
    int64_t te = tb + RS_TILE - 1;
    if (te > count - 1) te = count - 1;
    int32_t lo = 0, hi = n - 1;
    while (lo < hi) {
        const int32_t mid = lo + (hi - lo + 1) / 2;
        if ((int64_t)Ap[mid] <= tb) lo = mid;
        else hi = mid - 1;
    }
    const int32_t j0 = lo;
    hi = n - 1;
    while (lo < hi) {
        const int32_t mid = lo + (hi - lo + 1) / 2;
        if ((int64_t)Ap[mid] <= te) lo = mid;
        else hi = mid - 1;
    }
    desc[(size_t)t * RS_DESC_WORDS] = (uint32_t)j0;
    desc[(size_t)t * RS_DESC_WORDS + 1] = (uint32_t)(lo - j0);
}

__global__ void k_rs_tiledesc_starts(const int32_t *Ap, int32_t n, int64_t count, uint32_t *desc) {
    const int64_t j = (int64_t)blockIdx.x * blockDim.x + threadIdx.x;
    if (j >= n) return;
    const int64_t p = Ap[j];
    if (p >= count) return;
    const int64_t t = p / RS_TILE;
    const uint32_t rel = (uint32_t)(p - t * RS_TILE);
    if (rel == 0) return;
    const int64_t k = j - (int64_t)desc[(size_t)t * RS_DESC_WORDS] - 1;
    if (k < RS_DESC_STARTS) reinterpret_cast<uint16_t *>(desc + (size_t)t * RS_DESC_WORDS + 2)[k] = (uint16_t)rel;
}

struct RsArgs {
    const uint32_t *key, *a;
    const double *v;
    const Pay *pay;
    uint32_t *okey, *oa;
    double *ov;
    Pay *opay;
    const int32_t *goff;
    const int32_t *xp;
    const uint32_t *desc;
    int32_t *optr;
    int64_t count;
    int shift;
    uint32_t mask, nblocks;
    int flat;
    const uint16_t *key16;
    uint16_t *okey16;
    int k16_w0;
};

template <bool HAS_A, bool HAS_V, bool IN_AOS, bool OUT_AOS, int KM = 0>
__global__ __launch_bounds__(RS_THREADS) void k_rs_scatter(const RsArgs g) {
    static_assert(!(IN_AOS || OUT_AOS) || (HAS_A && HAS_V), "packed records carry both payloads");
    __shared__ int wh[RS_WAVES][RS_BINS];
    __shared__ int gbase[RS_BINS];
    __shared__ uint32_t s_key[RS_TILE];
    int *const wsum = reinterpret_cast<int *>(s_key);
    __shared__ __attribute__((aligned(16))) unsigned char s_raw[(HAS_A || HAS_V) ? (HAS_A ? 4 : 0) * RS_TILE + (HAS_V ? 8 : 0) * RS_TILE : 16];
    uint32_t *const s_a = reinterpret_cast<uint32_t *>(s_raw);
    double *const s_v = reinterpret_cast<double *>(s_raw + (HAS_A ? 4 * RS_TILE : 0));
    Pay *const s_pay = reinterpret_cast<Pay *>(s_raw);
    const int lane = threadIdx.x & 63, w = threadIdx.x >> 6;
    const int64_t count = g.count;
    const int shift = g.shift;
    const uint32_t mask = g.mask, nblocks = g.nblocks;
#pragma unroll
    for (int k = 0; k < RS_WAVES; k++) wh[k][threadIdx.x] = 0;
    uint32_t tile = blockIdx.x;
    if (!g.flat) {
        const uint32_t q = nblocks >> 3, rem = nblocks & 7u, x = blockIdx.x & 7u, kk = blockIdx.x >> 3;
        tile = x * q + (x < rem ? x : rem) + kk;
    }
    const int64_t tbase = (int64_t)tile * RS_TILE;
    const int64_t wbase = tbase + (int64_t)w * 64 * RS_ROUNDS;
    uint32_t kreg[RS_ROUNDS], areg[HAS_A ? RS_ROUNDS : 1];
    double vreg[HAS_V ? RS_ROUNDS : 1];
    const bool expand = HAS_A && !IN_AOS && g.xp != nullptr;
    uint32_t d0 = 0, d1 = 0;
    if (expand) {
        d0 = g.desc[(size_t)tile * RS_DESC_WORDS + lane];
        d1 = g.desc[(size_t)tile * RS_DESC_WORDS + 64 + lane];
    }
#pragma unroll
    for (int r = 0; r < RS_ROUNDS; r++) {
        const int64_t idx = wbase + r * 64 + lane;
        kreg[r] = KM >= 2 ? (uint32_t)g.key16[idx < count ? idx : count - 1] : g.key[idx < count ? idx : count - 1];
    }
#pragma unroll
    for (int r = 0; r < RS_ROUNDS; r++) {
        const int64_t idx = wbase + r * 64 + lane;
        const int64_t cl = idx < count ? idx : count - 1;
        if (IN_AOS) {
            const Pay pr = g.pay[cl];
            areg[r] = pr.a;
            vreg[r] = __hiloint2double((int)pr.vhi, (int)pr.vlo);
        } else {
            if (HAS_A && !g.xp) areg[r] = g.a[cl];
            if (HAS_V) vreg[r] = g.v[cl];
        }
    }
    if (expand) {
        const int32_t j0 = __builtin_amdgcn_readlane((int)d0, 0), K = __builtin_amdgcn_readlane((int)d0, 1);
        const int32_t j1 = j0 + K;
        if (K <= RS_DESC_STARTS) {
            uint32_t *const s_col = reinterpret_cast<uint32_t *>(s_raw);
            const int wu = __builtin_amdgcn_readfirstlane(w);
            for (int c = wu - 1; c < K; c += RS_WAVES) {
                int b = 0, e = RS_TILE;
                if (c >= 0) {
                    const int h = c + 4;
                    const uint32_t wd = (h >> 1) < 64 ? (uint32_t)__builtin_amdgcn_readlane((int)d0, (h >> 1) & 63)
                                                      : (uint32_t)__builtin_amdgcn_readlane((int)d1, (h >> 1) & 63);
                    b = (int)((wd >> (16 * (h & 1))) & 0xffffu);
                }
                if (c + 1 < K) {
                    const int h = c + 5;
                    const uint32_t wd = (h >> 1) < 64 ? (uint32_t)__builtin_amdgcn_readlane((int)d0, (h >> 1) & 63)
                                                      : (uint32_t)__builtin_amdgcn_readlane((int)d1, (h >> 1) & 63);
                    e = (int)((wd >> (16 * (h & 1))) & 0xffffu);
                }
                for (int q = b + lane; q < e; q += 64) s_col[q] = (uint32_t)(j0 + 1 + c);
            }
            lds_barrier();
#pragma unroll
            for (int r = 0; r < RS_ROUNDS; r++) areg[r] = s_col[w * 64 * RS_ROUNDS + r * 64 + lane];
        } else if (K <= RS_TILE) {
            for (int k = threadIdx.x; k < K; k += RS_THREADS) s_key[k] = (uint32_t)((int64_t)g.xp[j0 + 1 + k] - tbase);
            lds_barrier();
            int lo[RS_ROUNDS];
#pragma unroll
            for (int r = 0; r < RS_ROUNDS; r++) lo[r] = 0;
            int top = 1;
            while (top * 2 <= K) top *= 2;
            for (int half = top; half > 0; half >>= 1) {
#pragma unroll
                for (int r = 0; r < RS_ROUNDS; r++) {
                    const uint32_t li = (uint32_t)(w * 64 * RS_ROUNDS + r * 64 + lane);
                    const int mid = lo[r] + half;
                    if (mid <= K && s_key[mid - 1] <= li) lo[r] = mid;
                }
            }
#pragma unroll
            for (int r = 0; r < RS_ROUNDS; r++) areg[r] = (uint32_t)(j0 + lo[r]);
        } else {
#pragma unroll 1
            for (int r = 0; r < RS_ROUNDS; r++) {
                const int64_t pos = wbase + r * 64 + lane;
                int32_t lo = j0, hi = j1;
                while (lo < hi) {
                    const int32_t mid = lo + (hi - lo + 1) / 2;
                    if ((int64_t)g.xp[mid] <= pos) lo = mid;
                    else hi = mid - 1;
                }
                areg[r] = (uint32_t)lo;
            }
        }
    }
    if (KM == 1) {
#pragma unroll
        for (int r = 0; r < RS_ROUNDS; r++) areg[r] |= (kreg[r] & mask) << (32 - g.k16_w0);
    }
    lds_barrier();
    const unsigned long long lt = (lane == 0) ? 0ull : (~0ull >> (64 - lane));
    int rk[RS_ROUNDS];
#pragma unroll
    for (int r = 0; r < RS_ROUNDS; r++) {
        const int64_t idx = wbase + r * 64 + lane;
        const bool valid = idx < count;
        const uint32_t d = (kreg[r] >> shift) & mask;
        unsigned long long peers = __ballot(valid);
#pragma unroll
        for (int b = 0; b < 8; b++) {
            unsigned long long bal = __ballot((d >> b) & 1u);
            peers &= ((d >> b) & 1u) ? bal : ~bal;
        }
        const int rank = __popcll(peers & lt), cnt = __popcll(peers);
        rk[r] = rank | (cnt << 8);
        if (valid && rank == 0) atomicAdd(&wh[w][d], cnt);
    }
    lds_barrier();
    {
        const int d = threadIdx.x;
        int tot = 0;
#pragma unroll
        for (int k = 0; k < RS_WAVES; k++) tot += wh[k][d];
        int inc = tot;
#pragma unroll
        for (int dd = 1; dd < 64; dd <<= 1) {
            int t = __shfl_up(inc, dd, 64);
            if (lane >= dd) inc += t;
        }
        if (lane == 63) wsum[w] = inc;
        lds_barrier();
        int off = 0;
#pragma unroll
        for (int k = 0; k < RS_WAVES; k++)
            if (k < w) off += wsum[k];
        int run = off + inc - tot;
        gbase[d] = g.goff[(size_t)tile * RS_BINS + d] - run;
#pragma unroll
        for (int k = 0; k < RS_WAVES; k++) {
            int c = wh[k][d];
            wh[k][d] = run;
            run += c;
        }
    }
    lds_barrier();
#pragma unroll
    for (int r = 0; r < RS_ROUNDS; r++) {
        int64_t idx = wbase + r * 64 + lane;
        bool valid = idx < count;
        uint32_t k = kreg[r];
        uint32_t d = (k >> shift) & mask;
        const int rank = rk[r] & 255;
        int pos = 0;
        if (valid) pos = wh[w][d] + rank;
        __builtin_amdgcn_wave_barrier();
        if (valid && rank == 0) wh[w][d] = pos + (rk[r] >> 8);
        __builtin_amdgcn_wave_barrier();
        if (valid) {
            s_key[pos] = k;
            if (OUT_AOS) {
                Pay pr;
                pr.a = areg[r];
                pr.vlo = (uint32_t)__double2loint(vreg[r]);
                pr.vhi = (uint32_t)__double2hiint(vreg[r]);
                s_pay[pos] = pr;
            } else {
                if (HAS_A) s_a[pos] = areg[r];
                if (HAS_V) s_v[pos] = vreg[r];
            }
        }
    }
    lds_barrier();
    const int tcount = (int)((count - tbase) < RS_TILE ? (count - tbase) : RS_TILE);
    for (int i = threadIdx.x; i < tcount; i += RS_THREADS) {
        const uint32_t k = s_key[i];
        const int64_t gp = (int64_t)gbase[(k >> shift) & mask] + i;
        if (KM == 1) g.okey16[gp] = (uint16_t)(k >> g.k16_w0);
        else if (KM == 2) g.okey16[gp] = (uint16_t)k;
        else if (KM == 0 && g.okey) g.okey[gp] = k;
        if (OUT_AOS) {
            g.opay[gp] = s_pay[i];
        } else if (KM == 3) {
            const int ps = 32 - g.k16_w0;
            const uint32_t a = s_a[i], full = (k << g.k16_w0) | (a >> ps);
            g.oa[gp] = a & ((1u << ps) - 1u);
            if (HAS_V) g.ov[gp] = s_v[i];
            if (g.optr && (i == 0 || s_key[i - 1] != k || (s_a[i - 1] >> ps) != (a >> ps))) atomicMin(&g.optr[full], (int32_t)gp);
        } else {
            if (HAS_A) g.oa[gp] = s_a[i];
            if (HAS_V) g.ov[gp] = s_v[i];
        }
        if (KM == 0 && g.optr && (i == 0 || s_key[i - 1] != k)) atomicMin(&g.optr[k], (int32_t)gp);
    }
}

enum RsInstance : int { RSI_NONE = 0, RSI_KEYS, RSI_A, RSI_V, RSI_AV_FLAT_FLAT, RSI_AV_FLAT_PACKED, RSI_AV_PACKED_PACKED,
                        RSI_AV_PACKED_FLAT, RSI_SHORT_FIRST, RSI_SHORT_MIDDLE, RSI_SHORT_LAST };

template <bool HAS_A, bool HAS_V>
static int launch_scatter(bool in_aos, bool out_aos, dim3 grid, hipStream_t s, const RsArgs &g) {
    if constexpr (HAS_A && HAS_V) {
        if (in_aos && out_aos) {
            hipLaunchKernelGGL((k_rs_scatter<true, true, true, true>), grid, dim3(RS_THREADS), 0, s, g);
            return RSI_AV_PACKED_PACKED;
        }
        if (in_aos) {
            hipLaunchKernelGGL((k_rs_scatter<true, true, true, false>), grid, dim3(RS_THREADS), 0, s, g);
            return RSI_AV_PACKED_FLAT;
        }
        if (out_aos) {
            hipLaunchKernelGGL((k_rs_scatter<true, true, false, true>), grid, dim3(RS_THREADS), 0, s, g);
            return RSI_AV_FLAT_PACKED;
        }
        hipLaunchKernelGGL((k_rs_scatter<true, true, false, false>), grid, dim3(RS_THREADS), 0, s, g);
        return RSI_AV_FLAT_FLAT;
    } else {
        hipLaunchKernelGGL((k_rs_scatter<HAS_A, HAS_V, false, false>), grid, dim3(RS_THREADS), 0, s, g);
        return HAS_A ? RSI_A : HAS_V ? RSI_V : RSI_KEYS;
    }
}

constexpr int RS_MAX_PASSES = 4;
struct SortInfo {
    int64_t bits = 0, passes = 0, width[RS_MAX_PASSES] = {0, 0, 0, 0}, nblocks = 0, chunk = 0, nchunks = 0, packed = 0, k16 = 0,
            key_misalign = 0, instance[RS_MAX_PASSES] = {0, 0, 0, 0}, count = 0;
};
static SortInfo g_sort_info;

constexpr int SM_ITEMS = 8;
constexpr int SM_TILE = SCAN_THREADS * SM_ITEMS;

__global__ __launch_bounds__(SCAN_THREADS) void k_sufmin_block(const int32_t *p, int64_t n, int32_t *bm) {
    __shared__ int wmin[SCAN_THREADS / 64];
    const int64_t base = (int64_t)blockIdx.x * SM_TILE;
    int m = 0x7fffffff;
#pragma unroll
    for (int k = 0; k < SM_ITEMS; k++) {
        const int64_t idx = base + (int64_t)k * SCAN_THREADS + threadIdx.x;
        if (idx < n) m = min(m, p[idx]);
    }
#pragma unroll
    for (int d = 32; d >= 1; d >>= 1) m = min(m, __shfl_xor(m, d, 64));
    if ((threadIdx.x & 63) == 0) wmin[threadIdx.x >> 6] = m;
    __syncthreads();
    if (threadIdx.x == 0) {
#pragma unroll
        for (int k = 1; k < SCAN_THREADS / 64; k++) m = min(m, wmin[k]);
        bm[blockIdx.x] = m;
    }
}

__global__ __launch_bounds__(SCAN_THREADS) void k_sufmin_apply(int32_t *p, int64_t n, const int32_t *bm_suffix,
                                                               int64_t nb) {
    __shared__ int tmin[SCAN_THREADS];
    const int64_t base = (int64_t)blockIdx.x * SM_TILE + (int64_t)threadIdx.x * SM_ITEMS;
    int v[SM_ITEMS];
    int m = 0x7fffffff;
#pragma unroll
    for (int k = SM_ITEMS - 1; k >= 0; k--) {
        v[k] = (base + k < n) ? p[base + k] : 0x7fffffff;
        m = min(m, v[k]);
    }
    tmin[threadIdx.x] = m;
    __syncthreads();
    for (int d = 1; d < SCAN_THREADS; d <<= 1) {
        const int o = (threadIdx.x + d < SCAN_THREADS) ? tmin[threadIdx.x + d] : 0x7fffffff;
        __syncthreads();
        tmin[threadIdx.x] = min(tmin[threadIdx.x], o);
        __syncthreads();
    }
    int carry = (bm_suffix && (int64_t)blockIdx.x + 1 < nb) ? bm_suffix[blockIdx.x + 1] : 0x7fffffff;
    if (threadIdx.x + 1 < SCAN_THREADS) carry = min(carry, tmin[threadIdx.x + 1]);
#pragma unroll
    for (int k = SM_ITEMS - 1; k >= 0; k--) {
        carry = min(carry, v[k]);
        if (base + k < n) p[base + k] = carry;
    }
}

int suffix_min_i32(int32_t *p, int64_t n) {
    if (n <= 0) return CSX_OK;
    hipStream_t s = ctx().stream;
    const int64_t nb = (n + SM_TILE - 1) / SM_TILE;
    DevBuf<int32_t> bm;
    if (nb > 1) {
        CSX_TRY(bm.alloc((size_t)nb));
        hipLaunchKernelGGL(k_sufmin_block, dim3((unsigned)nb), dim3(SCAN_THREADS), 0, s, p, n, bm);
        CSX_LAUNCH_CHECK();
        CSX_TRY(suffix_min_i32(bm, nb));
    }
    hipLaunchKernelGGL(k_sufmin_apply, dim3((unsigned)nb), dim3(SCAN_THREADS), 0, s, p, n, bm, nb);
    CSX_LAUNCH_CHECK();
    if (bm) CSX_HIP(hipStreamSynchronize(s));
    return CSX_OK;
}

__global__ void k_ptr_init(int32_t *ptr, int32_t nkeys, int32_t count) {
    const int64_t i = (int64_t)blockIdx.x * blockDim.x + threadIdx.x;
    if (i < nkeys) ptr[i] = 0x7fffffff;
    else if (i == nkeys) ptr[i] = count;
}

constexpr uint32_t RS_CHUNK_MIN = 64, RS_CHUNK_DIV = 1024;

int stable_sort_by_key_ex(const uint32_t *key, const uint32_t *a, const double *v, int64_t count, uint32_t key_limit,
                          uint32_t *out_key, uint32_t *out_a, double *out_v, const SortExtra *ex) {
    hipStream_t s = ctx().stream;
    const int32_t *xp = ex ? ex->expand_ptr : nullptr;
    int32_t *optr = ex ? ex->out_ptr : nullptr;
    if (optr) {
        const int64_t nk = (int64_t)ex->nkeys + 1;
        hipLaunchKernelGGL(k_ptr_init, dim3((unsigned)((nk + 255) / 256)), dim3(256), 0, s, optr, ex->nkeys,
                           (int32_t)(count > 0 ? count : 0));
        CSX_LAUNCH_CHECK();
    }
    g_sort_info = SortInfo();
    if (count <= 0) return optr ? suffix_min_i32(optr, (int64_t)ex->nkeys + 1) : CSX_OK;
    int bits = 1;
    while (bits < 32 && (1ull << bits) < (unsigned long long)key_limit) bits++;
    const int passes = (bits + 7) / 8;
    const uint32_t nblocks = (uint32_t)((count + RS_TILE - 1) / RS_TILE);
    uint32_t chunk = (nblocks + RS_CHUNK_DIV - 1) / RS_CHUNK_DIV;
    if (chunk < RS_CHUNK_MIN) chunk = RS_CHUNK_MIN;
    const uint32_t nchunks = (nblocks + chunk - 1) / chunk;
    const bool has_a = a != nullptr || xp != nullptr, has_v = v != nullptr;
    const bool packed = has_a && has_v;
    const int w0 = bits / passes + (0 < bits % passes ? 1 : 0);
    const bool k16 = xp != nullptr && packed && passes == 3 && optr != nullptr && out_key == nullptr && bits - w0 <= 16 &&
                     (uint64_t)ex->expand_n <= (1ull << (32 - w0)) && ctx().opt.sort_short_keys;
    SortInfo &info = g_sort_info;
    info.bits = bits;
    info.passes = passes;
    info.nblocks = nblocks;
    info.chunk = chunk;
    info.nchunks = nchunks;
    info.packed = packed ? 1 : 0;
    info.k16 = k16 ? 1 : 0;
    info.key_misalign = (int64_t)((reinterpret_cast<uintptr_t>(key) & 15) / sizeof(uint32_t));
    info.count = count;

    DevBuf<int32_t> hist, part;
    DevBuf<uint32_t> desc;
    DevBuf<uint32_t> tk[2], ta[2];
    DevBuf<double> tv[2];
    DevBuf<Pay> tp[2];
    DevBuf<uint16_t> tk16[2];
    CSX_TRY(hist.alloc((size_t)RS_BINS * nblocks));
    CSX_TRY(part.alloc((size_t)RS_BINS * (nchunks + 1)));
    int32_t *const dbase = part + (size_t)RS_BINS * nchunks;
    if (xp) CSX_TRY(desc.alloc((size_t)nblocks * RS_DESC_WORDS));
    const int ntmp = passes > 2 ? 2 : passes - 1;
    for (int t = 0; t < ntmp; t++) {
        if (k16) CSX_TRY(tk16[t].alloc((size_t)count + 8));
        else CSX_TRY(tk[t].alloc((size_t)count));
        if (packed) {
            CSX_TRY(tp[t].alloc((size_t)count));
        } else {
            if (has_a) CSX_TRY(ta[t].alloc((size_t)count));
            if (has_v) CSX_TRY(tv[t].alloc((size_t)count));
        }
    }
    if (xp) {
        hipLaunchKernelGGL(k_rs_tiledesc_head, dim3((nblocks + 255) / 256), dim3(256), 0, s, xp, ex->expand_n, count, nblocks,
                           desc);
        CSX_LAUNCH_CHECK();
        hipLaunchKernelGGL(k_rs_tiledesc_starts, dim3((unsigned)(((int64_t)ex->expand_n + 255) / 256)), dim3(256), 0, s, xp,
                           ex->expand_n, count, desc);
        CSX_LAUNCH_CHECK();
    }
    RsArgs g{};
    g.key = key;
    g.a = a;
    g.v = v;
    g.xp = xp;
    g.desc = desc;
    g.count = count;
    g.nblocks = nblocks;
    g.flat = ablation_env("CSX_SORT_FLAT") ? 1 : 0;
    bool in_aos = false;
    int shift = 0;
    for (int ps = 0; ps < passes; ps++) {
        const bool last = ps == passes - 1;
        const int width = bits / passes + (ps < bits % passes ? 1 : 0);
        const bool out_aos = packed && !last;
        g.shift = shift;
        g.mask = (1u << width) - 1u;
        g.okey = last ? out_key : tk[ps & 1];
        g.oa = last ? out_a : ta[ps & 1];
        g.ov = last ? out_v : tv[ps & 1];
        g.opay = last ? nullptr : tp[ps & 1];
        g.optr = last ? optr : nullptr;
        g.goff = hist;
        if (k16) {
            g.k16_w0 = w0;
            g.okey16 = last ? nullptr : tk16[ps & 1];
            g.okey = nullptr;
            if (ps > 0) g.shift = shift - w0;
        }
        if (k16 && ps > 0) hipLaunchKernelGGL(k_rs_hist16, dim3(nblocks), dim3(RS_THREADS), 0, s, g.key16, count, g.shift, g.mask, hist);
        else hipLaunchKernelGGL(k_rs_hist, dim3(nblocks), dim3(RS_THREADS), 0, s, g.key, count, g.shift, g.mask, hist);
        hipLaunchKernelGGL(k_rs_colsum, dim3(nchunks), dim3(RS_BINS), 0, s, hist, nblocks, chunk, part);
        hipLaunchKernelGGL(k_rs_chunkscan, dim3(1), dim3(RS_BINS * RS_SEGS), 0, s, part, nchunks, dbase);
        hipLaunchKernelGGL(k_rs_tileprefix, dim3(nchunks), dim3(RS_BINS), 0, s, hist, part, dbase, nblocks, chunk);
        int inst;
        if (k16 && ps == 0) {
            hipLaunchKernelGGL((k_rs_scatter<true, true, false, true, 1>), dim3(nblocks), dim3(RS_THREADS), 0, s, g);
            inst = RSI_SHORT_FIRST;
        } else if (k16 && !last) {
            hipLaunchKernelGGL((k_rs_scatter<true, true, true, true, 2>), dim3(nblocks), dim3(RS_THREADS), 0, s, g);
            inst = RSI_SHORT_MIDDLE;
        } else if (k16) {
            hipLaunchKernelGGL((k_rs_scatter<true, true, true, false, 3>), dim3(nblocks), dim3(RS_THREADS), 0, s, g);
            inst = RSI_SHORT_LAST;
        } else if (has_a && has_v) inst = launch_scatter<true, true>(in_aos, out_aos, dim3(nblocks), s, g);
        else if (has_a) inst = launch_scatter<true, false>(false, false, dim3(nblocks), s, g);
        else if (has_v) inst = launch_scatter<false, true>(false, false, dim3(nblocks), s, g);
        else inst = launch_scatter<false, false>(false, false, dim3(nblocks), s, g);
        CSX_LAUNCH_CHECK();
        info.width[ps] = width;
        info.instance[ps] = inst;
        g.key = g.okey;
        g.key16 = g.okey16;
        g.a = g.oa;
        g.v = g.ov;
        g.pay = g.opay;
        g.xp = nullptr;
        in_aos = out_aos;
        shift += width;
    }
    if (optr) CSX_TRY(suffix_min_i32(optr, (int64_t)ex->nkeys + 1));
    CSX_HIP(hipStreamSynchronize(s));
    return CSX_OK;
}

int stable_sort_by_key(const uint32_t *key, const uint32_t *a, const double *v, int64_t count, uint32_t key_limit,
                       uint32_t *out_key, uint32_t *out_a, double *out_v) {
    return stable_sort_by_key_ex(key, a, v, count, key_limit, out_key, out_a, out_v, nullptr);
}

__global__ __launch_bounds__(256) void k_boundaries(const uint32_t *skey, int64_t count, int32_t nkeys, int32_t *ptr) {
    typedef uint32_t u32x4b __attribute__((ext_vector_type(4)));
    const int64_t q0 = ((int64_t)blockIdx.x * blockDim.x + threadIdx.x) * 4;
    if (q0 > count) return;
    int64_t prev = (q0 == 0) ? -1 : (int64_t)skey[q0 - 1];
    if (q0 + 4 <= count && (reinterpret_cast<uintptr_t>(skey) & 15) == 0) {
        const u32x4b v = *reinterpret_cast<const u32x4b *>(skey + q0);
        const uint32_t k4[4] = {v.x, v.y, v.z, v.w};
#pragma unroll
        for (int k = 0; k < 4; k++) {
            const int64_t cur = (int64_t)k4[k];
            for (int64_t r = prev + 1; r <= cur; r++) ptr[r] = (int32_t)(q0 + k);
            prev = cur;
        }
        return;
    }
    const int64_t qend = q0 + 4 <= count ? q0 + 4 : count + 1;
    for (int64_t q = q0; q < qend; q++) {
        const int64_t cur = (q == count) ? (int64_t)nkeys : (int64_t)skey[q];
        for (int64_t r = prev + 1; r <= cur; r++) ptr[r] = (int32_t)q;
        prev = cur;
    }
}

int boundaries_from_sorted(const uint32_t *sorted_key, int64_t count, int32_t nkeys, int32_t *ptr) {
    const int64_t threads = count / 4 + 1;
    const int64_t blocks = (threads + 255) / 256;
    hipLaunchKernelGGL(k_boundaries, dim3((unsigned)blocks), dim3(256), 0, ctx().stream, sorted_key, count, nkeys, ptr);
    CSX_LAUNCH_CHECK();
    return CSX_OK;
}

}

using namespace csx;

extern "C" int csx_cumsum(csx_handle_t hp, csx_handle_t hc, int64_t n, int64_t *total) {
    CSX_TRY(require_ready());
    Vec *p = ivec(hp), *c = ivec(hc);
    if (!p || !c || n < 0 || p->len < n + 1 || c->len < n) return CSX_EINVAL;
    CSX_TRY(scan_exclusive_i32((const int32_t *)c->d, (int32_t *)p->d, n, total));
    if (n)
        CSX_HIP(hipMemcpyAsync(c->d, p->d, (size_t)n * sizeof(int32_t), hipMemcpyDeviceToDevice, ctx().stream));
    return CSX_OK;
}

extern "C" int csx_prim_limits(int32_t *out) {
    if (!out) return CSX_EINVAL;
    const int32_t v[9] = {SCAN_TILE, SM_TILE, RS_TILE, RS_BINS, RS_DESC_STARTS, RS_SEGS, (int32_t)RS_CHUNK_MIN, (int32_t)RS_CHUNK_DIV,
                          EXPAND_GRID_MAX};
    for (int k = 0; k < 9; k++) out[k] = v[k];
    return CSX_OK;
}

extern "C" int csx_prim_sort_info(int64_t *out, int32_t cap) {
    if (!out || cap < 0) return CSX_EINVAL;
    const SortInfo &f = g_sort_info;
    const int64_t v[] = {f.bits, f.passes, f.width[0], f.width[1], f.width[2], f.width[3], f.nblocks, f.chunk, f.nchunks, f.packed,
                         f.k16, f.key_misalign, f.instance[0], f.instance[1], f.instance[2], f.instance[3], f.count};
    const int32_t nf = (int32_t)(sizeof v / sizeof v[0]);
    for (int32_t k = 0; k < nf && k < cap; k++) out[k] = v[k];
    return CSX_OK;
}

namespace {
template <class T>
int to_host(T *h, const T *d, size_t count) {
    if (count) CSX_HIP(hipMemcpyAsync(h, d, count * sizeof(T), hipMemcpyDeviceToHost, ctx().stream));
    return CSX_OK;
}
template <class T>
int to_device(T *d, const T *h, size_t count) {
    if (count) CSX_HIP(hipMemcpyAsync(d, h, count * sizeof(T), hipMemcpyHostToDevice, ctx().stream));
    return CSX_OK;
}
int alloc_misaligned(DevBuf<uint32_t> &buf, size_t count, int words, uint32_t **keys) {
    CSX_TRY(buf.alloc(count + 8));
    const uintptr_t base = (reinterpret_cast<uintptr_t>(buf.get()) + 15) & ~(uintptr_t)15;
    *keys = reinterpret_cast<uint32_t *>(base) + words;
    return CSX_OK;
}
constexpr size_t PRIM_GUARD = 256;
template <class T>
struct GuardedOut {
    DevBuf<T> d;
    size_t count = 0;
    unsigned char seen[PRIM_GUARD];
    int put(const T *h, size_t n) {
        count = n;
        CSX_TRY(d.alloc(n + PRIM_GUARD / sizeof(T)));
        CSX_TRY(to_device(d.get(), h, n));
        CSX_HIP(hipMemsetAsync(d.get() + n, 0xA5, PRIM_GUARD, ctx().stream));
        return CSX_OK;
    }
    int take(T *h) {
        CSX_TRY(to_host(h, (const T *)d.get(), count));
        CSX_HIP(hipMemcpyAsync(seen, d.get() + count, PRIM_GUARD, hipMemcpyDeviceToHost, ctx().stream));
        return CSX_OK;
    }
    bool intact() const {
        for (size_t k = 0; k < PRIM_GUARD; k++)
            if (seen[k] != 0xA5) return false;
        return true;
    }
};
int guard_verdict(bool intact, const char *what) {
    if (intact) return CSX_OK;
    set_error("%s: a store past the end of an output array", what);
    return CSX_ERUNTIME;
}
bool pointers_ok(const int32_t *p, int64_t n, int64_t count) {
    if (p[0] != 0 || (int64_t)p[n] != count) return false;
    for (int64_t j = 0; j < n; j++)
        if (p[j] > p[j + 1]) return false;
    return true;
}
}

extern "C" int csx_prim_scan(int32_t *in, int32_t *out, int64_t n, int in_place, int64_t *total) {
    if (n < 0 || !out || (n > 0 && !in)) return CSX_EINVAL;
    CSX_TRY(require_ready());
    DevBuf<int32_t> din;
    GuardedOut<int32_t> dout;
    CSX_TRY(dout.put(out, (size_t)n + 1));
    if (in_place) {
        CSX_TRY(to_device(dout.d.get(), (const int32_t *)in, (size_t)n));
        CSX_TRY(scan_exclusive_i32(dout.d, dout.d, n, total));
    } else {
        CSX_TRY(upload(din, (const int32_t *)in, (size_t)n));
        CSX_TRY(scan_exclusive_i32(din, dout.d, n, total));
        CSX_TRY(to_host(in, (const int32_t *)din.get(), (size_t)n));
    }
    CSX_TRY(dout.take(out));
    CSX_HIP(hipStreamSynchronize(ctx().stream));
    return guard_verdict(dout.intact(), "csx_prim_scan");
}

extern "C" int csx_prim_suffix_min(int32_t *p, int64_t n) {
    if (n < 0 || (n > 0 && !p)) return CSX_EINVAL;
    CSX_TRY(require_ready());
    GuardedOut<int32_t> d;
    CSX_TRY(d.put(p, (size_t)n));
    CSX_TRY(suffix_min_i32(d.d, n));
    CSX_TRY(d.take(p));
    CSX_HIP(hipStreamSynchronize(ctx().stream));
    return guard_verdict(d.intact(), "csx_prim_suffix_min");
}

extern "C" int csx_prim_expand_columns(int32_t *Ap, int32_t n, int32_t nnz, int32_t *col) {
    if (n < 0 || nnz < 0 || !Ap || (nnz > 0 && !col) || !pointers_ok(Ap, n, nnz)) return CSX_EINVAL;
    CSX_TRY(require_ready());
    DevBuf<int32_t> dp;
    GuardedOut<int32_t> dc;
    CSX_TRY(upload(dp, (const int32_t *)Ap, (size_t)n + 1));
    CSX_TRY(dc.put(col, (size_t)nnz));
    CSX_TRY(expand_columns(dp, n, nnz, dc.d));
    CSX_TRY(to_host(Ap, (const int32_t *)dp.get(), (size_t)n + 1));
    CSX_TRY(dc.take(col));
    CSX_HIP(hipStreamSynchronize(ctx().stream));
    return guard_verdict(dc.intact(), "csx_prim_expand_columns");
}

extern "C" int csx_prim_boundaries(uint32_t *sorted_key, int64_t count, int32_t nkeys, int32_t *ptr, int misalign_words) {
    if (count < 0 || nkeys < 0 || !ptr || (count > 0 && !sorted_key) || misalign_words < 0 || misalign_words > 3) return CSX_EINVAL;
    for (int64_t q = 0; q < count; q++)
        if (sorted_key[q] >= (uint32_t)nkeys || (q > 0 && sorted_key[q - 1] > sorted_key[q])) return CSX_EINVAL;
    CSX_TRY(require_ready());
    DevBuf<uint32_t> kbuf;
    GuardedOut<int32_t> dp;
    uint32_t *dk = nullptr;
    CSX_TRY(alloc_misaligned(kbuf, (size_t)count, misalign_words, &dk));
    CSX_TRY(to_device(dk, (const uint32_t *)sorted_key, (size_t)count));
    CSX_TRY(dp.put(ptr, (size_t)nkeys + 1));
    CSX_TRY(boundaries_from_sorted(dk, count, nkeys, dp.d));
    CSX_TRY(to_host(sorted_key, (const uint32_t *)dk, (size_t)count));
    CSX_TRY(dp.take(ptr));
    CSX_HIP(hipStreamSynchronize(ctx().stream));
    return guard_verdict(dp.intact(), "csx_prim_boundaries");
}

extern "C" int csx_prim_sort(uint32_t *key, uint32_t *a, double *v, int64_t count, uint32_t key_limit, uint32_t *out_key,
                             uint32_t *out_a, double *out_v, int32_t *expand_ptr, int32_t expand_n, int32_t *out_ptr, int32_t nkeys,
                             int misalign_words) {
    if (count < 0 || (count > 0 && !key) || misalign_words < 0 || misalign_words > 3) return CSX_EINVAL;
    if (((a || expand_ptr) && !out_a) || (v && !out_v)) return CSX_EINVAL;
    if (a && expand_ptr) return CSX_EINVAL;
    if (expand_ptr && (expand_n < 1 || !pointers_ok(expand_ptr, expand_n, count))) return CSX_EINVAL;
    if (out_ptr) {
        if (nkeys < 0) return CSX_EINVAL;
        for (int64_t q = 0; q < count; q++)
            if (key[q] >= (uint32_t)nkeys) return CSX_EINVAL;
    }
    CSX_TRY(require_ready());
    hipStream_t s = ctx().stream;
    const size_t cnt = (size_t)count;
    DevBuf<uint32_t> kbuf, da;
    DevBuf<double> dv;
    DevBuf<int32_t> dxp;
    GuardedOut<uint32_t> dok, doa;
    GuardedOut<double> dov;
    GuardedOut<int32_t> dop;
    uint32_t *dk = nullptr;
    CSX_TRY(alloc_misaligned(kbuf, cnt, misalign_words, &dk));
    CSX_TRY(to_device(dk, (const uint32_t *)key, cnt));
    if (a) CSX_TRY(upload(da, (const uint32_t *)a, cnt));
    if (v) CSX_TRY(upload(dv, (const double *)v, cnt));
    if (expand_ptr) CSX_TRY(upload(dxp, (const int32_t *)expand_ptr, (size_t)expand_n + 1));
    const bool with_a = a || expand_ptr;
    if (out_key) CSX_TRY(dok.put(out_key, cnt));
    if (with_a) CSX_TRY(doa.put(out_a, cnt));
    if (v) CSX_TRY(dov.put(out_v, cnt));
    if (out_ptr) CSX_TRY(dop.put(out_ptr, (size_t)nkeys + 1));
    const SortExtra ex{expand_ptr ? dxp.get() : nullptr, expand_n, out_ptr ? dop.d.get() : nullptr, nkeys};
    CSX_TRY(stable_sort_by_key_ex(dk, a ? da.get() : nullptr, v ? dv.get() : nullptr, count, key_limit, out_key ? dok.d.get() : nullptr,
                                  with_a ? doa.d.get() : nullptr, v ? dov.d.get() : nullptr, (expand_ptr || out_ptr) ? &ex : nullptr));
    CSX_TRY(to_host(key, (const uint32_t *)dk, cnt));
    if (a) CSX_TRY(to_host(a, (const uint32_t *)da.get(), cnt));
    if (v) CSX_TRY(to_host(v, (const double *)dv.get(), cnt));
    if (expand_ptr) CSX_TRY(to_host(expand_ptr, (const int32_t *)dxp.get(), (size_t)expand_n + 1));
    if (out_key) CSX_TRY(dok.take(out_key));
    if (with_a) CSX_TRY(doa.take(out_a));
    if (v) CSX_TRY(dov.take(out_v));
    if (out_ptr) CSX_TRY(dop.take(out_ptr));
    CSX_HIP(hipStreamSynchronize(s));
    return guard_verdict((!out_key || dok.intact()) && (!with_a || doa.intact()) && (!v || dov.intact()) && (!out_ptr || dop.intact()),
                         "csx_prim_sort");
}
```

### include/csx.h

```cpp
#ifndef CSX_H
#define CSX_H

#include <stddef.h>
#include <stdint.h>

#ifdef __cplusplus
extern "C" {
#endif

typedef uint64_t csx_handle_t;

enum {
    CSX_OK = 0,
    CSX_EINVAL = 1,
    CSX_EZEROPIVOT = 2,
    CSX_ENOTSPD = 3,
    CSX_ERUNTIME = 4
};

enum { CSX_TRI_L = 0, CSX_TRI_LT = 1, CSX_TRI_U = 2, CSX_TRI_UT = 3 };

enum {
    CSX_GAXPY_AUTO = 0,
    CSX_GAXPY_EXACT = 1,
    CSX_GAXPY_WAVE = 2,
    CSX_GAXPY_TILED = 3,
    CSX_GAXPY_ATOMIC = 4
};

int csx_init(int device);
int csx_finalize(void);
const char *csx_last_error(void);
int csx_sync(void);
int csx_set_stream(void *hip_stream);
int csx_device_info(char *name, int name_cap, int *compute_units, int64_t *hbm_bytes);
int csx_mem_trim(void);
int csx_mem_info(int64_t *cached_bytes, int64_t *live_bytes, int64_t *device_free_bytes);
int csx_set_option(const char *name, int value);
int csx_get_option(const char *name, int *value);
int csx_timer_start(void);
int csx_timer_stop(double *ms);

int csx_csc_upload(int32_t m, int32_t n, const int32_t *p, const int32_t *i, const double *x ,
                   csx_handle_t *out);
int csx_csc_alloc(int32_t m, int32_t n, int32_t nnz, int values, csx_handle_t *out);
int csx_csc_wrap(int32_t m, int32_t n, int32_t nnz, void *d_p, void *d_i, void *d_x ,
                 csx_handle_t *out);
int csx_csc_info(csx_handle_t A, int32_t *m, int32_t *n, int32_t *nnz, int *has_values);
int csx_csc_download(csx_handle_t A, int32_t *p, int32_t *i, double *x );
int csx_csc_ptrs(csx_handle_t A, void **d_p, void **d_i, void **d_x);
int csx_csc_invalidate(csx_handle_t A);
int csx_free(csx_handle_t h);

int csx_vec_alloc(int64_t len, csx_handle_t *out);
int csx_vec_upload(const double *src, int64_t len, csx_handle_t *out);
int csx_vec_wrap(void *d_ptr, int64_t len, csx_handle_t *out);
int csx_vec_download(csx_handle_t v, double *dst, int64_t len);
int csx_vec_write(csx_handle_t v, const double *src, int64_t len);
int csx_vec_fill(csx_handle_t v, double value);
int csx_vec_copy(csx_handle_t src, csx_handle_t dst);
int csx_vec_ptr(csx_handle_t v, void **d_ptr, int64_t *len);
int csx_ivec_upload(const int32_t *src, int64_t len, csx_handle_t *out);
int csx_ivec_download(csx_handle_t v, int32_t *dst, int64_t len);


int csx_gaxpy(csx_handle_t A, csx_handle_t x, csx_handle_t y, int mode);
int csx_gaxpy_prepare(csx_handle_t A, int mode);
int csx_gaxpy_plan_info(csx_handle_t A, int *has_rows, int *has_tiled, int *key_bytes);
int csx_gaxpy_plan_shape(csx_handle_t A, int *shape, double *ms4);
int csx_gaxpy_plan_geometry(csx_handle_t A, int64_t *info);
int csx_gaxpy_plan_groups(csx_handle_t A, int32_t *groups);
int csx_gaxpy_host(int32_t m, int32_t n, const int32_t *p, const int32_t *i, const double *x, const double *xv,
                   double *yv);
int csx_gaxpy_block(csx_handle_t A, csx_handle_t X, csx_handle_t Y, int32_t nrhs, int mode);

int csx_residual_block(csx_handle_t A, csx_handle_t X, csx_handle_t B, csx_handle_t R, int32_t nrhs, int trans,
                       double *omega, double *rnorm);
int csx_residual_host(int32_t m, int32_t n, const int32_t *p, const int32_t *i, const double *x, int32_t nrhs, int trans,
                      const double *X, const double *B, double *R , double *omega, double *rnorm);
int csx_residual_sym_block(csx_handle_t A, csx_handle_t X, csx_handle_t B, csx_handle_t R, int32_t nrhs, double *omega,
                           double *rnorm);
int csx_residual_sym_host(int32_t n, const int32_t *p, const int32_t *i, const double *x, int32_t nrhs, const double *X,
                          const double *B, double *R , double *omega, double *rnorm);
int csx_norm1_sym(csx_handle_t A, double *out);
int csx_block_add_cols(csx_handle_t X, csx_handle_t D, csx_handle_t out, int64_t rows, int32_t nrhs, const int32_t *mask);
int csx_block_select_cols(csx_handle_t src, csx_handle_t dst, int64_t rows, int32_t nrhs, const int32_t *mask);

int csx_transpose(csx_handle_t A, int values, csx_handle_t *out);

int csx_cumsum(csx_handle_t p, csx_handle_t c, int64_t n, int64_t *total);

int csx_prim_limits(int32_t *out);
int csx_prim_scan(int32_t *in, int32_t *out, int64_t n, int in_place, int64_t *total);
int csx_prim_suffix_min(int32_t *p, int64_t n);
int csx_prim_expand_columns(int32_t *Ap, int32_t n, int32_t nnz, int32_t *col);
int csx_prim_boundaries(uint32_t *sorted_key, int64_t count, int32_t nkeys, int32_t *ptr, int misalign_words);
int csx_prim_sort(uint32_t *key, uint32_t *a, double *v, int64_t count, uint32_t key_limit, uint32_t *out_key, uint32_t *out_a,
                  double *out_v, int32_t *expand_ptr, int32_t expand_n, int32_t *out_ptr, int32_t nkeys, int misalign_words);
int csx_prim_sort_info(int64_t *out, int32_t cap);

int csx_multiply(csx_handle_t A, csx_handle_t B, csx_handle_t *out);
int csx_spgemm_limits(int32_t *out);
int csx_spgemm_info(int64_t *out, int32_t cap, int32_t *count);

int csx_tri_analyse(csx_handle_t T, int kind, csx_handle_t *plan);
int csx_tri_info(csx_handle_t plan, int32_t *n, int32_t *levels, int32_t *sequential);
int csx_tri_solve(csx_handle_t plan, csx_handle_t X, int32_t nrhs);
int csx_tri_solve_list(csx_handle_t plan, double *x, int *taken);
int csx_cholsol_solve_list(csx_handle_t plan, double *b, int *taken);
int csx_tri_set_order(csx_handle_t plan, int exact);
int csx_tri_order_info(csx_handle_t plan, int32_t *matrix_cores, double *growth);
int csx_tri_components(csx_handle_t plan, int32_t *ncomp);
int csx_tri_limits(int32_t *out);
int csx_tri_route_info(csx_handle_t plan, int32_t nrhs, int64_t *out, int32_t cap, int32_t *count);
int csx_tri_launches(csx_handle_t plan, int64_t *out, int32_t cap, int32_t *count);
int csx_cholsol_tri_route_info(csx_handle_t plan, int backward, int32_t nrhs, int64_t *out, int32_t cap, int32_t *count);
int csx_cholsol_tri_launches(csx_handle_t plan, int backward, int64_t *out, int32_t cap, int32_t *count);

int csx_permute_vec(csx_handle_t p, csx_handle_t b, csx_handle_t x, int32_t n, int32_t nrhs, int inverse);
int csx_lusol_solve(csx_handle_t planL, csx_handle_t planU, csx_handle_t pinv, csx_handle_t q, csx_handle_t b, csx_handle_t work,
                    int32_t nrhs, int *fused);
int csx_lusol_solve_trans(csx_handle_t planUT, csx_handle_t planLT, csx_handle_t pinv, csx_handle_t q, csx_handle_t b,
                          csx_handle_t work, int32_t nrhs, int *fused);

int csx_schol_host(int32_t n, const int32_t *Ap, const int32_t *Ai, int32_t *parent, int32_t *cp);
int csx_counts_host(int32_t m, int32_t n, const int32_t *Ap, const int32_t *Ai, const int32_t *parent, const int32_t *post,
                    int ata, int32_t *colcount);
int csx_schol(csx_handle_t A, int32_t *parent, int32_t *cp);

int csx_order_nd_host(int32_t n, const int32_t *Ap, const int32_t *Ai, int32_t *perm);

int csx_chol(csx_handle_t A, const int32_t *parent, const int32_t *cp, const int32_t *pinv,
             csx_handle_t *L);
int csx_chol_info(int32_t *path, double *numeric_ms);

int csx_cholsol_plan(csx_handle_t L, const int32_t *pinv , csx_handle_t *plan);
int csx_cholsol_factor(csx_handle_t A, int exact, csx_handle_t *L, csx_handle_t *plan);
int csx_cholsol_factor_info(int32_t *path, double *analysis_ms, double *numeric_ms, double *call_ms);
int csx_cholsol_forest_plan(int sparse, int32_t min_bs, int32_t max_bs, int exact, int dense_blocks, int32_t *kind);
int csx_cholsol_info(csx_handle_t plan, int32_t *path, int32_t *ntrees, int32_t *max_nodes);
int csx_cholsol_solve(csx_handle_t plan, csx_handle_t B, int32_t nrhs);
int csx_cholsol_set_order(csx_handle_t plan, int exact);
int csx_cholsol_growth(csx_handle_t plan, double *growth);
int csx_cholsol_sn_info(csx_handle_t plan, int32_t *supernodes, int32_t *steps, int32_t *max_width, int32_t *matrix_cores,
                        double *growth);
int csx_cholsol_sn_geometry(csx_handle_t plan, int64_t *out, int32_t cap, int32_t *count);
int csx_cholsol_sn_launches(csx_handle_t plan, int64_t *out, int32_t cap, int32_t *count);

int csx_cholsol_graph_info(csx_handle_t plan, int32_t *captures, double *last_capture_ms);

int csx_compress(int32_t m, int32_t n, int64_t nz, const int32_t *Ti, const int32_t *Tj, const double *Tx,
                 csx_handle_t *out);
int csx_add(csx_handle_t A, csx_handle_t B, double alpha, double beta, csx_handle_t *out);
int csx_dupl(csx_handle_t A, csx_handle_t *out);
int csx_drop(csx_handle_t A, int mode, double tol, csx_handle_t *out);
int csx_permute(csx_handle_t A, const int32_t *pinv, const int32_t *q, int values, csx_handle_t *out);
int csx_symperm(csx_handle_t A, const int32_t *pinv, int values, csx_handle_t *out);
int csx_norm1(csx_handle_t A, double *out);
int csx_csc_col_block(csx_handle_t A, int32_t first, int32_t count, csx_handle_t *out);

int csx_updown(csx_handle_t L, int sigma, int32_t cnz, const int32_t *Ci, const double *Cx, const int32_t *parent,
               int *ok);

int csx_updown_block(csx_handle_t L, csx_handle_t C, const int32_t *sigma, const int32_t *parent, int flags, int32_t *applied);
int csx_updown_block_info(int32_t *chunks, int32_t *union_columns, int32_t *groups, double *kernel_ms);
int csx_updown_block_classes(int32_t counts[4], int32_t *replayed);

int csx_chol_inverse(csx_handle_t L, csx_handle_t *Z);
int csx_chol_inverse_info(int32_t *depths, int32_t *widest, int64_t *terms, double *kernel_ms);
int csx_csc_diag(csx_handle_t M, csx_handle_t out);
int csx_ldl_inverse(csx_handle_t L, csx_handle_t d, csx_handle_t *Z);
int csx_slu_inverse(csx_handle_t L, csx_handle_t Ut, csx_handle_t *ZL, csx_handle_t *ZUt);
int csx_inverse_at(csx_handle_t ZL, csx_handle_t ZUt, csx_handle_t rmap, csx_handle_t cmap, int64_t count, const int32_t *rows,
                   const int32_t *cols, csx_handle_t out, int64_t *missing);

int csx_lu_host(int32_t n, const int32_t *Ap, const int32_t *Ai, const double *Ax, double tol,
                int32_t **Lp, int32_t **Li, double **Lx, int32_t **Up, int32_t **Ui, double **Ux,
                int32_t *pinv);
void csx_host_free(void *p);

int csx_qr_host(int32_t m, int32_t n, int32_t m2, const int32_t *Ap, const int32_t *Ai, const double *Ax,
                const int32_t *q , const int32_t *parent, const int32_t *pinv, const int32_t *leftmost,
                int32_t vcap, int32_t rcap, int32_t *Vp, int32_t *Vi, double *Vx, int32_t *Rp, int32_t *Ri, double *Rx,
                double *beta);
int csx_qr_apply_host(int32_t n, const int32_t *Vp, const int32_t *Vi, const double *Vx, const double *beta, int transpose,
                      double *x);
int csx_happly(csx_handle_t V, csx_handle_t beta, csx_handle_t X, int32_t nrhs, int transpose);
int csx_sqr_host(int32_t m, int32_t n, const int32_t *Ap, const int32_t *Ai, int32_t *parent, int32_t *cp, int32_t *pinv,
                 int32_t *leftmost, int32_t *m2, int64_t *vnz, int64_t *rnz);
int csx_qr_blocks(csx_handle_t A, const int32_t *parent, const int32_t *pinv, const int32_t *leftmost, int32_t m2,
                  csx_handle_t *V, csx_handle_t *R, double *beta, int *done);
int csx_lu_blocks(csx_handle_t A, double tol, csx_handle_t *L, csx_handle_t *U, int32_t *pinv, int *done);

int csx_block_limits(int32_t *out);
int csx_prim_components(int32_t n, int32_t *p, int32_t *i, int skip_first, int skip_last, int order, int32_t *root,
                        uint32_t *nodes, int32_t *first, int32_t *count, int32_t *comp_of_pos, int32_t *ncomp, int32_t *maxc,
                        int *malformed);

int csx_lu_etree(csx_handle_t A, double tol, csx_handle_t *L, csx_handle_t *U, int32_t *pinv, int *done);

int csx_spsolve(csx_handle_t G, csx_handle_t B, const int32_t *pinv , int lo, int values, csx_handle_t *X);

#define CSX_COMM_ID_BYTES 128
int csx_comm_unique_id(uint8_t *id128);
int csx_comm_init(int rank, int world, const uint8_t *id128 );
int csx_comm_finalize(void);
int csx_comm_info(int *rank, int *world, int *uses_rccl);
int csx_comm_barrier(void);
int csx_comm_allreduce_host(double *vals, int count, int op);
int csx_comm_bcast_host(void *buf, int64_t bytes, int root);
int csx_comm_bcast_csc(csx_handle_t *A, int root);
int csx_comm_bcast_vec(csx_handle_t v, int root);
int csx_comm_reduce_scatter_vec(csx_handle_t full, csx_handle_t out);
int csx_comm_allreduce_vec(csx_handle_t v);
int csx_comm_scatter_blocks(csx_handle_t src, csx_handle_t dst, int64_t len, int root);
int csx_comm_gather_blocks(csx_handle_t block, csx_handle_t out, int64_t len, int root);
int csx_block_cols(csx_handle_t B, int64_t n, int32_t K, int32_t c0, int32_t k, csx_handle_t out, int back);
int csx_gaxpy_sharded_plan(csx_handle_t block, csx_handle_t *plan);
int csx_gaxpy_sharded_rows(csx_handle_t plan, int32_t *first, int32_t *count);
int csx_gaxpy_sharded(csx_handle_t plan, csx_handle_t x, csx_handle_t y_mine, int how);
int csx_gaxpy_sharded_plan_for(csx_handle_t block, int world, csx_handle_t *plan);
int csx_gaxpy_sharded_piece(csx_handle_t plan, int q, csx_handle_t x);
int csx_gaxpy_sharded_buffers(csx_handle_t plan, void **work, void **recv, int64_t *chunk);
int csx_gaxpy_sharded_sum(csx_handle_t plan, int rank, int world, csx_handle_t y_mine);

int csx_maxtrans(csx_handle_t A, int64_t seed, int32_t *jimatch, int32_t *sprank);
int csx_scc(csx_handle_t A, int32_t *p, int32_t *r, int32_t *nb);
int csx_dmperm(csx_handle_t A, int64_t seed, int32_t *p, int32_t *q, int32_t *r, int32_t *s, int32_t *nb, int32_t *rr,
               int32_t *cc);
int csx_dmperm_times(double *ms);
int csx_dmperm_rounds(int64_t *rounds);

int csx_btf_split(csx_handle_t A, const int32_t *p, const int32_t *q, const int32_t *r, int32_t nb, int32_t *p_out,
                  int32_t *q_out, int32_t *r_out, int32_t *level, int32_t *nlevels, csx_handle_t *D, csx_handle_t *F);
int csx_btf_plan(csx_handle_t L, csx_handle_t U, csx_handle_t F, const int32_t *pinv, const int32_t *p, const int32_t *q,
                 const int32_t *r, const int32_t *level, int32_t nb, csx_handle_t *plan);
int csx_btf_solve(csx_handle_t plan, csx_handle_t B, csx_handle_t work, int32_t nrhs);
int csx_btf_solve_trans(csx_handle_t plan, csx_handle_t B, csx_handle_t work, int32_t nrhs);
int csx_btf_info(csx_handle_t plan, int64_t *info);
int csx_btf_limits(int32_t *out);

int csx_lu_refactor_host(int32_t n, const int32_t *Ap, const int32_t *Ai, const double *Ax, const int32_t *pinv,
                         const int32_t *Lp, const int32_t *Li, double *Lx, const int32_t *Up, const int32_t *Ui, double *Ux,
                         int *ok, double *ratio);
int csx_btf_refactor(csx_handle_t plan, csx_handle_t A, csx_handle_t A2, csx_handle_t D, int *ok, double *ratio,
                     int64_t *cols);
int csx_btf_refactor_dx(csx_handle_t plan, double *Dx);
int csx_lu_refactor_plan(csx_handle_t L, csx_handle_t U, csx_handle_t A, const int32_t *q, const int32_t *pinv,
                         csx_handle_t *plan);
int csx_lu_refactor(csx_handle_t plan, csx_handle_t A2, int *ok, double *ratio, int64_t *cols);

int csx_chol_refactor_plan(csx_handle_t A, csx_handle_t L, const int32_t *pinv, csx_handle_t *plan);
int csx_chol_refactor(csx_handle_t plan, csx_handle_t A2, int *ok, int32_t *info);
int csx_chol_refactor_info(double *numeric_ms, double *call_ms);
int csx_chol_refactor_window(csx_handle_t plan, int32_t *window);
int csx_chol_limits(int32_t *out);

int csx_assemble_plan_host(int32_t m, int32_t n, int64_t nz, const int32_t *Ti, const int32_t *Tj, int32_t *Cp, int32_t *Ci,
                           int32_t *sp, int32_t *src, int32_t *nnz);
int csx_assemble_host(int32_t nnz, const int32_t *sp, const int32_t *src, const double *Tx, double *Cx);
int csx_assemble_plan(int32_t m, int32_t n, int64_t nz, const int32_t *Ti, const int32_t *Tj, csx_handle_t *plan);
int csx_assemble_matrix(csx_handle_t plan, csx_handle_t Tx, csx_handle_t *A);
int csx_assemble(csx_handle_t plan, csx_handle_t Tx, csx_handle_t out);
int csx_assemble_plan_info(csx_handle_t plan, int64_t *info);

int csx_multiply_plan_count(int32_t m, int32_t k, int32_t n, const int32_t *Ap, const int32_t *Ai, const int32_t *Bp,
                            const int32_t *Bi, int64_t *nnz, int64_t *products);
int csx_multiply_plan_host(int32_t m, int32_t k, int32_t n, const int32_t *Ap, const int32_t *Ai, const int32_t *Bp,
                           const int32_t *Bi, int32_t *Cp, int32_t *Ci, int32_t *sp, int32_t *pair);
int csx_multiply_fold_host(int32_t nnz, const int32_t *sp, const int32_t *pair, const double *Ax, const double *Bx, double *Cx);
int csx_multiply_plan(csx_handle_t A, csx_handle_t B, csx_handle_t *plan);
int csx_multiply_plan_matrix(csx_handle_t plan, csx_handle_t Ax, csx_handle_t Bx, csx_handle_t d, csx_handle_t *C);
int csx_multiply_plan_run(csx_handle_t plan, csx_handle_t Ax, csx_handle_t Bx, csx_handle_t d, csx_handle_t out);
int csx_multiply_plan_info(csx_handle_t plan, int64_t *info);

int csx_add_plan_host(int32_t m, int32_t n, int32_t k, const int32_t *const *Ap, const int32_t *const *Ai, int32_t *Cp,
                      int32_t *Ci, int32_t *sp, int32_t *src, int32_t *nnz);
int csx_add_fold_host(int32_t nnz, int32_t k, const int32_t *sp, const int32_t *src, const int32_t *off, const double *coef,
                      const double *const *X, double *Cx);
int csx_add_plan(int32_t k, const csx_handle_t *operands, csx_handle_t *plan);
int csx_add_plan_matrix(csx_handle_t plan, const double *coef, const csx_handle_t *X, csx_handle_t *C);
int csx_add_plan_run(csx_handle_t plan, const double *coef, const csx_handle_t *X, csx_handle_t out);
int csx_add_plan_info(csx_handle_t plan, int64_t *info);

int csx_ldl_factor(csx_handle_t A, const int32_t *parent, const int32_t *cp, const int32_t *pinv, double tau, csx_handle_t *F,
                   int *ok);
int csx_ldl_refactor(csx_handle_t F, csx_handle_t A2, double tau, int *ok);
int csx_ldl_parts(csx_handle_t F, csx_handle_t *L, csx_handle_t *d);
int csx_ldl_info(csx_handle_t F, int64_t *info);
int csx_ldl_stats(csx_handle_t F, double *out);
int csx_ldl_window(int32_t *entries);
int csx_block_div_rows(csx_handle_t X, csx_handle_t d, int64_t rows, int32_t nrhs);
int csx_ldl_host(int32_t n, const int32_t *Ap, const int32_t *Ai, const double *Ax, const int32_t *pinv, const int32_t *Lp,
                 const int32_t *Li, double tau, double *Lx, double *d, int64_t *info);

int csx_schur_factor(csx_handle_t A, const int32_t *parent, const int32_t *cp, const int32_t *pinv, int32_t n1, double tau,
                     csx_handle_t *F, int *ok);
int csx_schur_refactor(csx_handle_t F, csx_handle_t A2, double tau, int *ok);
int csx_schur_parts(csx_handle_t F, csx_handle_t *Lp, csx_handle_t *d, csx_handle_t *S);
int csx_schur_info(csx_handle_t F, int64_t *info);
int csx_schur_stats(csx_handle_t F, double *out);
int csx_schur_host(int32_t n, const int32_t *Ap, const int32_t *Ai, const double *Ax, const int32_t *pinv, const int32_t *Lfp,
                   const int32_t *Lfi, int32_t n1, double tau, double *Lpx, double *d, double *S, int64_t *info);

int csx_slu_factor(csx_handle_t A, const int32_t *parent, const int32_t *cp, const int32_t *prow, const int32_t *pinv, double tau,
                   csx_handle_t *F, int *ok);
int csx_slu_refactor(csx_handle_t F, csx_handle_t A2, double tau, int *ok);
int csx_slu_parts(csx_handle_t F, csx_handle_t *L, csx_handle_t *Ut);
int csx_slu_info(csx_handle_t F, int64_t *info);
int csx_slu_stats(csx_handle_t F, double *out);
int csx_slu_window(int32_t *entries, int32_t *run_levels);
int csx_slu_host(int32_t n, const int32_t *Ap, const int32_t *Ai, const double *Ax, const int32_t *prow, const int32_t *pinv,
                 const int32_t *Lp, const int32_t *Li, double tau, double *Lx, double *Utx, int64_t *info);

int csx_slu_batch_factor(csx_handle_t F, csx_handle_t V, int32_t B, const double *tau, csx_handle_t *batch, int *ok);
int csx_slu_batch_refactor(csx_handle_t batch, csx_handle_t V, const double *tau, int *ok);
int csx_slu_batch_norm1(csx_handle_t F, csx_handle_t V, int32_t B, double *out);
int csx_slu_batch_solve(csx_handle_t batch, csx_handle_t X, int32_t r, int trans);
int csx_slu_batch_info(csx_handle_t batch, int64_t *shared, int64_t *members);
int csx_slu_batch_stats(csx_handle_t batch, double *out);
int csx_slu_batch_member(csx_handle_t batch, int32_t m, double *Lx, double *Utx);
int csx_slu_batch_limits(int32_t *out);

int csx_ldl_batch_factor(csx_handle_t F, csx_handle_t V, int32_t B, const double *tau, csx_handle_t *batch, int *ok);
int csx_ldl_batch_refactor(csx_handle_t batch, csx_handle_t V, const double *tau, int *ok);
int csx_ldl_batch_norm1(csx_handle_t F, csx_handle_t V, int32_t B, double *out);
int csx_ldl_batch_solve(csx_handle_t batch, csx_handle_t X, int32_t r);
int csx_ldl_batch_info(csx_handle_t batch, int64_t *shared, int64_t *members);
int csx_ldl_batch_stats(csx_handle_t batch, double *out);
int csx_ldl_batch_member(csx_handle_t batch, int32_t m, double *Lx, double *d);
int csx_ldl_batch_d(csx_handle_t batch, double *out);
int csx_ldl_batch_limits(int32_t *out);

int csx_hqr_symbolic_host(int32_t m, int32_t n, int32_t m2, const int32_t *Ap, const int32_t *Ai, const int32_t *q,
                          const int32_t *parent, const int32_t *pinv, const int32_t *leftmost, int32_t vcap, int32_t rcap,
                          int32_t *Vp, int32_t *Vi, int32_t *Rp, int32_t *Ri);
int csx_hqr_host(int32_t m, int32_t n, int32_t m2, const int32_t *Ap, const int32_t *Ai, const double *Ax, const int32_t *q,
                 const int32_t *parent, const int32_t *pinv, const int32_t *leftmost, int32_t vcap, int32_t rcap, int32_t *Vp,
                 int32_t *Vi, double *Vx, int32_t *Rp, int32_t *Ri, double *Rx, double *beta);
int csx_hqr_factor(csx_handle_t A, const int32_t *q, const int32_t *parent, const int32_t *pinv, const int32_t *leftmost,
                   int32_t m2, csx_handle_t *F, int *ok);
int csx_hqr_refactor(csx_handle_t F, csx_handle_t A2, int *ok);
int csx_hqr_parts(csx_handle_t F, csx_handle_t *V, csx_handle_t *R, csx_handle_t *beta);
int csx_hqr_info(csx_handle_t F, int64_t *info);
int csx_hqr_stats(csx_handle_t F, double *out);
int csx_hqr_window(int32_t *entries, int32_t *run_levels);
int csx_level_schedule(int32_t nlev, const int32_t *level_ptr, int32_t waves, int32_t run_levels, const int64_t *work,
                       int64_t run_work, int32_t *launches, int32_t *count);

int csx_gmres_limits(int32_t *out);
int csx_gs_work_len(int64_t rows, int32_t nrhs, int32_t nblocks, int64_t *len);
int csx_gs_project(csx_handle_t V, int32_t nv, csx_handle_t W, csx_handle_t work, int64_t rows, int32_t nrhs, const int32_t *mask,
                   int negate, double *h);
int csx_gs_update(csx_handle_t V, int32_t nv, csx_handle_t W, csx_handle_t work, int64_t rows, int32_t nrhs, const int32_t *mask,
                  int negate, const double *h, double *nrm2);
int csx_gs_scale(csx_handle_t W, csx_handle_t V, int32_t slot, csx_handle_t work, int64_t rows, int32_t nrhs, const int32_t *mask,
                 const double *s);
int csx_gs_combine(csx_handle_t V, int32_t nv, csx_handle_t U, csx_handle_t work, int64_t rows, int32_t nrhs, const int32_t *mask,
                   const double *y, const int32_t *len);
int csx_gs_host(int op, int64_t rows, int32_t nrhs, int32_t nv, double *V, double *W, const int32_t *mask, int negate,
                const double *coef, const int32_t *len, double *out);

int csx_bgs_limits(int32_t *out);
int csx_bgs_work_len(int64_t rows, int32_t b, int32_t q, int32_t nblocks, int64_t *len);
int csx_bgs_gram(csx_handle_t V, int32_t nv, int32_t b, csx_handle_t W, int32_t q, csx_handle_t work, int64_t rows, int negate,
                 double *out);
int csx_bgs_update(csx_handle_t V, int32_t nv, int32_t b, csx_handle_t W, int32_t q, csx_handle_t work, int64_t rows,
                   const double *H);
int csx_bgs_combine(csx_handle_t V, int32_t nv, int32_t b, csx_handle_t U, int32_t q, csx_handle_t work, int64_t rows,
                    const double *S);
int csx_bgs_host(int op, int64_t rows, int32_t b, int32_t q, int32_t nv, const double *V, double *W, int negate, const double *coef,
                 double *out);

int csx_pattern_outer(csx_handle_t A, csx_handle_t U, csx_handle_t V, int32_t nrhs, int mode, double alpha, csx_handle_t out);
int csx_pattern_outer_host(int32_t m, int32_t n, const int32_t *p, const int32_t *i, int32_t nrhs, int mode, double alpha,
                           const double *U, const double *V, double *out);
int csx_pattern_outer_limits(int64_t *out);
int csx_assemble_pullback(csx_handle_t plan, csx_handle_t g, csx_handle_t out);
int csx_assemble_pullback_host(int32_t nnz, int64_t nz, const int32_t *sp, const int32_t *src, const double *g, double *out);

int csx_gen_grand(int32_t n, int32_t per_col, uint64_t seed, csx_handle_t *out);
int csx_gen_grand_uniform(int32_t n, int32_t per_col, uint64_t seed, csx_handle_t *out);
int csx_gen_gspd(int32_t nblocks, int32_t bs, uint64_t seed, csx_handle_t *out);
int csx_gen_vec(int64_t len, uint64_t seed, double lo, double hi, csx_handle_t *out);
int csx_gen_rhs(int32_t n, int32_t nrhs, int32_t col0, csx_handle_t *out);

#ifdef __cplusplus
}
#endif
#endif
```

Baseline: 5757 GB/s.

## Rebuild tiled gaxpy plan construction with presorted-radix sort and group layout kernel

Reworks how the tiled gaxpy plan is built. Column ids are now found per chunk with an LDS binary search instead of a full column expansion. Tile ids become power-of-two-packed keys so the radix sort can skip the low bits that are already sorted, and a per-group layout kernel writes interleaved keys, 24-bit keys and values through shared memory. This targets the cost of the plan preparation (sort passes, scattered interleave writes), not the steady-state SpMV kernel, which the metric times. It adds plan-array export and a presorted sort API.

```diff
diff --git a/csparse.py_amd/_csx.py b/csparse.py_amd/_csx.py
--- a/csparse.py_amd/_csx.py
+++ b/csparse.py_amd/_csx.py
@@ -79,6 +79,7 @@
     "csx_prim_expand_columns": [_i32p, C.c_int32, C.c_int32, _i32p],
     "csx_prim_boundaries": [_vp, C.c_int64, C.c_int32, _i32p, C.c_int],
     "csx_prim_sort": [_vp, _vp, _f64p, C.c_int64, C.c_uint32, _vp, _vp, _f64p, _i32p, C.c_int32, _i32p, C.c_int32, C.c_int],
+    "csx_prim_sort_presorted": [_vp, _vp, _f64p, C.c_int64, C.c_uint32, _vp, _vp, _f64p, _i32p, C.c_int32, C.c_int, C.c_int],
     "csx_prim_sort_info": [C.POINTER(C.c_int64), C.c_int32],
     "csx_multiply": [H, H, C.POINTER(H)],
     "csx_spgemm_limits": [_i32p],
@@ -136,6 +137,7 @@
     "csx_gaxpy_plan_shape": [H, C.POINTER(C.c_int), C.POINTER(C.c_double)],
     "csx_gaxpy_plan_geometry": [H, C.POINTER(C.c_int64)],
     "csx_gaxpy_plan_groups": [H, _i32p],
+    "csx_gaxpy_plan_arrays": [H, C.c_int, _vp, C.c_int64, C.POINTER(C.c_int64)],
     "csx_lu_host": [C.c_int32, _i32p, _i32p, _f64p, C.c_double, C.POINTER(_i32p), C.POINTER(_i32p),
                     C.POINTER(_f64p), C.POINTER(_i32p), C.POINTER(_i32p), C.POINTER(_f64p), _i32p],
     "csx_comm_unique_id": [C.POINTER(C.c_uint8)],
@@ -650,6 +652,34 @@
     return {"out_key": ok, "out_a": oa, "out_v": ov, "out_ptr": op, "key": k, "a": aa, "v": vv, "expand_ptr": xp}
 
 
+def prim_sort_presorted(key, low_bits, a=None, v=None, key_limit=0xFFFFFFFF, want_key=True, nkeys=None, misalign_words=0):
+    k, aa = _u32(key), _u32(a)
+    vv = None if v is None else np.array(v, dtype=np.float64)
+    n = len(k)
+    ok = np.full(n, 0xDEADBEEF, np.uint32) if want_key else None
+    oa = np.full(n, 0xDEADBEEF, np.uint32) if aa is not None else None
+    ov = np.full(n, -777.0, np.float64) if vv is not None else None
+    op = np.full(nkeys + 1, -1, np.int32) if nkeys is not None else None
+    check(lib().csx_prim_sort_presorted(_vptr(k), _vptr(aa), pd(vv), n, key_limit, _vptr(ok), _vptr(oa), pd(ov), pi(op),
+                                        0 if nkeys is None else nkeys, misalign_words, low_bits), "csx_prim_sort_presorted")
+    return {"out_key": ok, "out_a": oa, "out_v": ov, "out_ptr": op, "key": k, "a": aa, "v": vv}
+
+
+PLAN_ARRAYS = (("rb_gptr", np.int32), ("group_info", np.uint32), ("keys", np.uint8), ("tile_base", np.uint32),
+               ("tile_val", np.float64))
+
+
+def gaxpy_plan_arrays(hA):
+    out = {}
+    for which, (name, dt) in enumerate(PLAN_ARRAYS):
+        nbytes = C.c_int64(-1)
+        check(lib().csx_gaxpy_plan_arrays(hA, which, None, 0, C.byref(nbytes)), "csx_gaxpy_plan_arrays")
+        buf = np.zeros(nbytes.value // np.dtype(dt).itemsize, dt)
+        check(lib().csx_gaxpy_plan_arrays(hA, which, _vptr(buf), buf.nbytes, None), "csx_gaxpy_plan_arrays")
+        out[name] = buf
+    return out
+
+
 def prim_sort_info():
     out = (C.c_int64 * 17)()
     check(load().csx_prim_sort_info(out, 17), "csx_prim_sort_info")
diff --git a/csparse.py_amd/csrc/csx_gaxpy_tiled.hip b/csparse.py_amd/csrc/csx_gaxpy_tiled.hip
--- a/csparse.py_amd/csrc/csx_gaxpy_tiled.hip
+++ b/csparse.py_amd/csrc/csx_gaxpy_tiled.hip
@@ -14,95 +14,154 @@
 typedef u32x3 u32x3_a4 __attribute__((aligned(4)));
 typedef double f64x2 __attribute__((ext_vector_type(2)));
 
-__global__ __launch_bounds__(256) void k_tile_keys(int64_t nnz, const int32_t *__restrict__ Ai,
-                                                   const int32_t *__restrict__ col, int rb_bits, int32_t row_block,
-                                                   int32_t slab_cols, int32_t nslab, uint32_t *__restrict__ tile_id,
-                                                   uint32_t *__restrict__ packed) {
-    int64_t p = (int64_t)blockIdx.x * blockDim.x + threadIdx.x;
-    if (p >= nnz) return;
-    const uint32_t i = (uint32_t)Ai[p], j = (uint32_t)col[p];
-    const uint32_t s = j / (uint32_t)slab_cols, lc = j - s * (uint32_t)slab_cols;
-    const uint32_t b = i / (uint32_t)row_block, lr = i - b * (uint32_t)row_block;
-    tile_id[p] = b * (uint32_t)nslab + s;
-    packed[p] = (lc << rb_bits) | lr;
-}
-
-__global__ __launch_bounds__(256) void k_padded_lengths(int64_t ntiles, const int32_t *__restrict__ sptr,
-                                                        int32_t *__restrict__ ngroups) {
-    int64_t t = (int64_t)blockIdx.x * blockDim.x + threadIdx.x;
-    if (t < ntiles) ngroups[t] = (sptr[t + 1] - sptr[t] + TL_GROUP - 1) / TL_GROUP;
+constexpr int TK_THREADS = 256, TK_PER = 8;
+constexpr int TK_CHUNK = TK_THREADS * TK_PER;
+constexpr int TK_LDS_COLS = 2048;
+
+__global__ __launch_bounds__(256) void k_chunk_columns(const int32_t *__restrict__ Ap, int32_t n, int64_t nchunks,
+                                                       int32_t *__restrict__ jstart) {
+    const int64_t c = (int64_t)blockIdx.x * blockDim.x + threadIdx.x;
+    if (c > nchunks) return;
+    int32_t lo = 0, hi = n - 1;
+    if (c < nchunks) {
+        const int64_t pos = c * TK_CHUNK;
+        while (lo < hi) {
+            const int32_t mid = lo + (hi - lo + 1) / 2;
+            if ((int64_t)Ap[mid] <= pos) lo = mid;
+            else hi = mid - 1;
+        }
+    } else {
+        lo = hi;
+    }
+    jstart[c] = lo;
+}
+
+__global__ __launch_bounds__(TK_THREADS) void k_tile_keys(int64_t nnz, const int32_t *__restrict__ Ap,
+                                                          const int32_t *__restrict__ Ai, const int32_t *__restrict__ jstart,
+                                                          int rb_bits, int32_t row_block, int32_t slab_cols, int sbits,
+                                                          uint32_t *__restrict__ tile_id, uint32_t *__restrict__ packed) {
+    __shared__ int32_t s_start[TK_LDS_COLS];
+    const int64_t base = (int64_t)blockIdx.x * TK_CHUNK;
+    const int32_t j0 = jstart[blockIdx.x], K = jstart[blockIdx.x + 1] - j0;
+    uint32_t row[TK_PER];
+#pragma unroll
+    for (int r = 0; r < TK_PER; r++) {
+        const int64_t p = base + r * TK_THREADS + threadIdx.x;
+        row[r] = (uint32_t)Ai[p < nnz ? p : nnz - 1];
+    }
+    int32_t cnt[TK_PER];
+#pragma unroll
+    for (int r = 0; r < TK_PER; r++) cnt[r] = 0;
+    if (K <= TK_LDS_COLS) {
+        for (int k = threadIdx.x; k < K; k += TK_THREADS) s_start[k] = Ap[j0 + 1 + k];
+        __syncthreads();
+        int top = 1;
+        while (top * 2 <= K) top *= 2;
+        for (int half = top; half > 0; half >>= 1) {
+#pragma unroll
+            for (int r = 0; r < TK_PER; r++) {
+                const int64_t p = base + r * TK_THREADS + threadIdx.x;
+                const int mid = cnt[r] + half;
+                if (mid <= K && (int64_t)s_start[mid - 1] <= p) cnt[r] = mid;
+            }
+        }
+    } else {
+#pragma unroll 1
+        for (int r = 0; r < TK_PER; r++) {
+            const int64_t p = base + r * TK_THREADS + threadIdx.x;
+            int32_t lo = j0, hi = j0 + K;
+            while (lo < hi) {
+                const int32_t mid = lo + (hi - lo + 1) / 2;
+                if ((int64_t)Ap[mid] <= p) lo = mid;
+                else hi = mid - 1;
+            }
+            cnt[r] = lo - j0;
+        }
+    }
+#pragma unroll
+    for (int r = 0; r < TK_PER; r++) {
+        const int64_t p = base + r * TK_THREADS + threadIdx.x;
+        if (p >= nnz) continue;
+        const uint32_t i = row[r], j = (uint32_t)(j0 + cnt[r]);
+        const uint32_t s = j / (uint32_t)slab_cols, lc = j - s * (uint32_t)slab_cols;
+        const uint32_t b = i / (uint32_t)row_block, lr = i - b * (uint32_t)row_block;
+        tile_id[p] = (b << sbits) | s;
+        packed[p] = (lc << rb_bits) | lr;
+    }
+}
+
+__global__ __launch_bounds__(256) void k_tile_ranges(int64_t ntiles, int32_t nslab, int sbits, int32_t nnz,
+                                                     const int32_t *__restrict__ kptr, int32_t *__restrict__ sptr,
+                                                     int32_t *__restrict__ ngroups) {
+    const int64_t t = (int64_t)blockIdx.x * blockDim.x + threadIdx.x;
+    if (t > ntiles) return;
+    if (t == ntiles) {
+        sptr[t] = nnz;
+        return;
+    }
+    const int64_t k = ((t / nslab) << sbits) | (t % nslab);
+    const int32_t b = kptr[k], e = kptr[k + 1];
+    sptr[t] = b;
+    ngroups[t] = (e - b + TL_GROUP - 1) / TL_GROUP;
 }
 
 __global__ __launch_bounds__(256) void k_group_info(int64_t ntiles, int32_t nslab, const int32_t *__restrict__ sptr,
-                                                    const int32_t *__restrict__ gptr, uint32_t *__restrict__ info) {
+                                                    const int32_t *__restrict__ gptr, uint32_t *__restrict__ info,
+                                                    int32_t *__restrict__ gsrc) {
     int64_t t = (int64_t)blockIdx.x * blockDim.x + threadIdx.x;
     if (t >= ntiles) return;
     const int32_t len = sptr[t + 1] - sptr[t];
     const uint32_t slab = (uint32_t)(t % nslab);
-    int32_t g = gptr[t];
-    for (int32_t left = len; left > 0; left -= TL_GROUP, g++) info[g] = (slab << 9) | (uint32_t)min(left, TL_GROUP);
-}
-
-__global__ __launch_bounds__(256) void k_interleave(int64_t nnz, const uint32_t *__restrict__ stid,
-                                                    const int32_t *__restrict__ sptr, const int32_t *__restrict__ gptr,
-                                                    const uint32_t *__restrict__ skey, const double *__restrict__ sval,
-                                                    uint32_t *__restrict__ okey, double *__restrict__ oval) {
-    int64_t q = (int64_t)blockIdx.x * blockDim.x + threadIdx.x;
-    if (q >= nnz) return;
-    const uint32_t t = stid[q];
-    const int32_t e = (int32_t)(q - sptr[t]);
-    const int32_t g = e / TL_GROUP, w = e % TL_GROUP;
-    const int64_t gbase = ((int64_t)gptr[t] + g) * TL_GROUP;
-    const int l = w & 63, k = w >> 6;
-    if (okey) okey[gbase + l * 4 + k] = skey[q];
-    oval[gbase + (k >> 1) * 128 + l * 2 + (k & 1)] = sval[q];
-}
-
-__global__ __launch_bounds__(256) void k_run_span(int64_t nnz, const uint32_t *__restrict__ stid,
-                                                  const int32_t *__restrict__ sptr, const uint32_t *__restrict__ skey,
-                                                  int rb_bits, int *too_wide) {
-    int64_t q = (int64_t)blockIdx.x * blockDim.x + threadIdx.x;
-    if (q >= nnz) return;
-    const int32_t e = (int32_t)(q - sptr[stid[q]]);
-    const int64_t first = q - (e & 63);
-    if ((skey[q] >> rb_bits) - (skey[first] >> rb_bits) >= 512u) *too_wide = 1;
-}
-
-__global__ __launch_bounds__(256) void k_interleave24(int64_t nnz, const uint32_t *__restrict__ stid,
-                                                      const int32_t *__restrict__ sptr, const int32_t *__restrict__ gptr,
-                                                      const uint32_t *__restrict__ skey, int rb_bits,
-                                                      uint8_t *__restrict__ okey, uint32_t *__restrict__ obase) {
-    int64_t q = (int64_t)blockIdx.x * blockDim.x + threadIdx.x;
-    if (q >= nnz) return;
-    const uint32_t t = stid[q];
-    const int32_t e = (int32_t)(q - sptr[t]);
-    const int32_t g = e / TL_GROUP, w = e % TL_GROUP;
-    const int l = w & 63, k = w >> 6;
-    const uint32_t rmask = (1u << rb_bits) - 1u;
-    const uint32_t col = skey[q] >> rb_bits, col0 = skey[q - l] >> rb_bits;
-    const uint32_t v = (skey[q] & rmask) | ((col - col0) << 15);
-    const int64_t gg = (int64_t)gptr[t] + g;
-    uint8_t *o = okey + gg * (TL_GROUP * 3) + l * 12 + k * 3;
-    o[0] = (uint8_t)v;
-    o[1] = (uint8_t)(v >> 8);
-    o[2] = (uint8_t)(v >> 16);
-    if (l == 0) obase[gg * 4 + k] = col;
-}
-
-__global__ __launch_bounds__(256) void k_fill_key24(uint8_t *p, int64_t nslots, uint32_t v) {
-    int64_t i = (int64_t)blockIdx.x * blockDim.x + threadIdx.x;
-    const int64_t stride = (int64_t)gridDim.x * blockDim.x;
-    for (; i < nslots; i += stride) {
-        p[3 * i] = (uint8_t)v;
-        p[3 * i + 1] = (uint8_t)(v >> 8);
-        p[3 * i + 2] = (uint8_t)(v >> 16);
-    }
-}
-
-__global__ __launch_bounds__(256) void k_fill_keys(uint32_t *p, int64_t n, uint32_t v) {
-    int64_t i = (int64_t)blockIdx.x * blockDim.x + threadIdx.x;
-    const int64_t stride = (int64_t)gridDim.x * blockDim.x;
-    for (; i < n; i += stride) p[i] = v;
+    int32_t g = gptr[t], q = sptr[t];
+    for (int32_t left = len; left > 0; left -= TL_GROUP, q += TL_GROUP, g++) {
+        info[g] = (slab << 9) | (uint32_t)min(left, TL_GROUP);
+        gsrc[g] = q;
+    }
+}
+
+constexpr int TL_LAY_KEY32 = 1, TL_LAY_KEY24 = 2, TL_LAY_VAL = 4;
+
+template <int WHAT>
+__global__ __launch_bounds__(TL_GROUP) void k_layout(const int32_t *__restrict__ gtotal, const uint32_t *__restrict__ info,
+                                                     const int32_t *__restrict__ gsrc, const uint32_t *__restrict__ skey,
+                                                     const double *__restrict__ sval, int rb_bits, uint32_t row_block,
+                                                     uint32_t *__restrict__ okey, uint32_t *__restrict__ okey24,
+                                                     uint32_t *__restrict__ obase, double *__restrict__ oval,
+                                                     int *__restrict__ too_wide) {
+    __shared__ uint32_t s_k[4][64];
+    __shared__ double s_v[4][64];
+    __shared__ uint32_t s_b[4];
+    const int64_t gg = blockIdx.x;
+    if (gg >= (int64_t)*gtotal) return;
+    const int w = threadIdx.x, l = w & 63, k = w >> 6;
+    const int cnt = (int)(info[gg] & 511u);
+    const bool valid = w < cnt;
+    const int64_t q = (int64_t)gsrc[gg] + w;
+    const uint32_t key = valid ? skey[q] : row_block;
+    if (WHAT & TL_LAY_VAL) s_v[k][l] = valid ? sval[q] : 0.0;
+    if (WHAT & TL_LAY_KEY24) {
+        const uint32_t col = key >> rb_bits;
+        const uint32_t off = col - (uint32_t)__shfl((int)col, 0, 64);
+        if (valid && off >= 512u) *too_wide = 1;
+        s_k[k][l] = valid ? (((key & ((1u << rb_bits) - 1u)) | (off << 15)) & 0xFFFFFFu) : row_block;
+        if (l == 0) s_b[k] = valid ? col : 0u;
+    } else {
+        s_k[k][l] = key;
+    }
+    __syncthreads();
+    if (WHAT & TL_LAY_KEY32) okey[gg * TL_GROUP + w] = s_k[w & 3][w >> 2];
+    if (WHAT & TL_LAY_KEY24) {
+        if (w < TL_GROUP * 3 / 4) {
+            const int ln = w / 3, part = w - 3 * ln;
+            const uint32_t v0 = s_k[0][ln], v1 = s_k[1][ln], v2 = s_k[2][ln], v3 = s_k[3][ln];
+            okey24[gg * (TL_GROUP * 3 / 4) + w] = part == 0 ? (v0 | (v1 << 24)) : part == 1 ? ((v1 >> 8) | (v2 << 16)) : ((v2 >> 16) | (v3 << 8));
+        }
+        if (w < 4) obase[gg * 4 + w] = s_b[w];
+    }
+    if (WHAT & TL_LAY_VAL) {
+        const int within = w & 127;
+        oval[gg * TL_GROUP + w] = s_v[(w >> 7) * 2 + (within & 1)][within >> 1];
+    }
 }
 
 struct KeyRegs {
@@ -435,6 +494,10 @@
     const int64_t ntiles = (int64_t)nrb * nslab;
     if (ntiles > 0x3fffffffll || nslab >= (1 << 22)) return CSX_EINVAL;
 
+    int sbits = 0;
+    while ((1 << sbits) < nslab) sbits++;
+    const int64_t nkeys = (int64_t)nrb << sbits;
+
     std::unique_ptr<TiledPlan> t(new TiledPlan());
     t->rb_bits = rb_bits;
     t->row_block = row_block;
@@ -442,70 +505,80 @@
     t->nslab = nslab;
     t->slab_cols = (int32_t)slab_cols;
     {
-        DevBuf<int32_t> col, sptr, gptr;
-        DevBuf<uint32_t> tid, packed, stid, skey;
+        const int64_t nnz = A->nnz;
+        const int64_t nchunks = (nnz + TK_CHUNK - 1) / TK_CHUNK;
+        const int64_t groups_max = nnz / TL_GROUP + (ntiles < nnz ? ntiles : nnz);
+        const bool try24 = rb_bits <= 15 && ctx().opt.gaxpy_keys24;
+        DevBuf<int32_t> jstart, kptr, sptr, gptr, gsrc;
+        DevBuf<uint32_t> tid, packed, skey;
         DevBuf<double> sval;
-        int64_t ngroups = 0;
-        CSX_TRY(col.alloc((size_t)A->nnz));
-        CSX_TRY(tid.alloc((size_t)A->nnz));
-        CSX_TRY(packed.alloc((size_t)A->nnz));
-        CSX_TRY(stid.alloc((size_t)A->nnz));
-        CSX_TRY(skey.alloc((size_t)A->nnz));
-        CSX_TRY(sval.alloc((size_t)A->nnz));
+        DevBuf<int> flag;
+        CSX_TRY(jstart.alloc((size_t)nchunks + 1));
+        CSX_TRY(tid.alloc((size_t)nnz));
+        CSX_TRY(packed.alloc((size_t)nnz));
+        CSX_TRY(skey.alloc((size_t)nnz));
+        CSX_TRY(sval.alloc((size_t)nnz));
+        CSX_TRY(kptr.alloc((size_t)nkeys + 1));
         CSX_TRY(sptr.alloc((size_t)ntiles + 1));
         CSX_TRY(gptr.alloc((size_t)ntiles + 1));
+        CSX_TRY(gsrc.alloc((size_t)groups_max));
+        CSX_TRY(flag.alloc(1));
         CSX_TRY(t->tile_ptr.alloc((size_t)nrb + 1));
-        CSX_TRY(expand_columns(A->p, A->n, A->nnz, col));
-        if (A->nnz > 0) {
-            int64_t blocks = ((int64_t)A->nnz + 255) / 256;
-            hipLaunchKernelGGL(k_tile_keys, dim3((unsigned)blocks), dim3(256), 0, s, (int64_t)A->nnz, A->i, col, rb_bits,
-                               row_block, t->slab_cols, t->nslab, tid, packed);
+        CSX_TRY(t->tile_len.alloc((size_t)groups_max));
+        CSX_TRY(t->tile_val.alloc((size_t)groups_max * TL_GROUP));
+        if (try24) {
+            CSX_TRY(t->tile_key24.alloc((size_t)groups_max * TL_GROUP * 3 + 16));
+            CSX_TRY(t->tile_base.alloc((size_t)groups_max * 4));
+        } else {
+            CSX_TRY(t->tile_key.alloc((size_t)groups_max * TL_GROUP));
+        }
+        if (nnz > 0) {
+            hipLaunchKernelGGL(k_chunk_columns, dim3((unsigned)((nchunks + 256) / 256)), dim3(256), 0, s, A->p, A->n, nchunks,
+                               jstart);
+            hipLaunchKernelGGL(k_tile_keys, dim3((unsigned)nchunks), dim3(TK_THREADS), 0, s, nnz, A->p, A->i, jstart, rb_bits,
+                               row_block, t->slab_cols, sbits, tid, packed);
             CSX_LAUNCH_CHECK();
         }
-        CSX_TRY(stable_sort_by_key(tid, packed, A->x, A->nnz, (uint32_t)ntiles, stid, skey, sval));
-        CSX_TRY(boundaries_from_sorted(stid, A->nnz, (int32_t)ntiles, sptr));
+        const SortExtra ex{nullptr, 0, kptr, (int32_t)nkeys, nrb == 1 ? 32 : sbits};
+        CSX_TRY(stable_sort_by_key_ex(tid, packed, A->x, nnz, (uint32_t)nkeys, nullptr, skey, sval, &ex));
         const unsigned tb = (unsigned)((ntiles + 256) / 256);
-        hipLaunchKernelGGL(k_padded_lengths, dim3(tb), dim3(256), 0, s, ntiles, sptr, gptr);
-        CSX_TRY(scan_exclusive_i32(gptr, gptr, ntiles, &ngroups));
-        bool k24 = false;
-        if (ngroups > 0 && rb_bits <= 15 && ctx().opt.gaxpy_keys24) {
-            DevBuf<int> flag;
-            int h = 1;
-            CSX_TRY(flag.alloc(1));
-            (void)hipMemsetAsync(flag, 0, sizeof(int), s);
-            hipLaunchKernelGGL(k_run_span, dim3((unsigned)(((int64_t)A->nnz + 255) / 256)), dim3(256), 0, s, (int64_t)A->nnz,
-                               stid, sptr, skey, rb_bits, flag);
-            CSX_HIP(hipMemcpyAsync(&h, flag, sizeof(int), hipMemcpyDeviceToHost, s));
-            CSX_HIP(hipStreamSynchronize(s));
-            k24 = h == 0;
-        }
-        t->ngroups = ngroups;
-        CSX_TRY(t->tile_len.alloc((size_t)ngroups));
-        if (!k24) CSX_TRY(t->tile_key.alloc((size_t)ngroups * TL_GROUP));
-        if (k24) CSX_TRY(t->tile_key24.alloc((size_t)ngroups * TL_GROUP * 3 + 16));
-        if (k24) CSX_TRY(t->tile_base.alloc((size_t)ngroups * 4));
-        CSX_TRY(t->tile_val.alloc((size_t)ngroups * TL_GROUP));
-        if (ngroups > 0) {
-            if (k24) {
-                hipLaunchKernelGGL(k_fill_key24, dim3(2048), dim3(256), 0, s, t->tile_key24, (int64_t)ngroups * TL_GROUP,
-                                   (uint32_t)row_block);
-                (void)hipMemsetAsync(t->tile_base, 0, (size_t)ngroups * 4 * sizeof(uint32_t), s);
-            } else {
-                hipLaunchKernelGGL(k_fill_keys, dim3(2048), dim3(256), 0, s, t->tile_key, (int64_t)ngroups * TL_GROUP,
-                                   (uint32_t)row_block);
+        hipLaunchKernelGGL(k_tile_ranges, dim3(tb), dim3(256), 0, s, ntiles, nslab, sbits, (int32_t)nnz, kptr, sptr, gptr);
+        CSX_TRY(scan_exclusive_i32(gptr, gptr, ntiles, nullptr));
+        hipLaunchKernelGGL(k_rb_group_ptr, dim3((unsigned)((nrb + 256) / 256)), dim3(256), 0, s, nrb, nslab, gptr, t->tile_ptr);
+        CSX_HIP(hipMemsetAsync(flag, 0, sizeof(int), s));
+        const int32_t *gtotal = gptr + ntiles;
+        uint32_t *key24w = reinterpret_cast<uint32_t *>(t->tile_key24.get());
+        if (groups_max > 0) {
+            hipLaunchKernelGGL(k_group_info, dim3(tb), dim3(256), 0, s, ntiles, nslab, sptr, gptr, (uint32_t *)t->tile_len.get(),
+                               gsrc);
+            if (try24)
+                hipLaunchKernelGGL((k_layout<TL_LAY_KEY24 | TL_LAY_VAL>), dim3((unsigned)groups_max), dim3(TL_GROUP), 0, s, gtotal,
+                                   (const uint32_t *)t->tile_len.get(), gsrc, skey, sval, rb_bits, (uint32_t)row_block, nullptr,
+                                   key24w, t->tile_base, t->tile_val, flag);
+            else
+                hipLaunchKernelGGL((k_layout<TL_LAY_KEY32 | TL_LAY_VAL>), dim3((unsigned)groups_max), dim3(TL_GROUP), 0, s, gtotal,
+                                   (const uint32_t *)t->tile_len.get(), gsrc, skey, sval, rb_bits, (uint32_t)row_block, t->tile_key,
+                                   nullptr, nullptr, t->tile_val, flag);
+        }
+        CSX_LAUNCH_CHECK();
+        int32_t total = 0;
+        int wide = 0;
+        CSX_HIP(hipMemcpyAsync(&total, gtotal, sizeof total, hipMemcpyDeviceToHost, s));
+        CSX_HIP(hipMemcpyAsync(&wide, flag, sizeof wide, hipMemcpyDeviceToHost, s));
+        CSX_HIP(hipStreamSynchronize(s));
+        t->ngroups = total;
+        if (try24 && (wide || total == 0)) {
+            t->tile_key24.reset();
+            t->tile_base.reset();
+            CSX_TRY(t->tile_key.alloc((size_t)groups_max * TL_GROUP));
+            if (total > 0) {
+                hipLaunchKernelGGL((k_layout<TL_LAY_KEY32>), dim3((unsigned)groups_max), dim3(TL_GROUP), 0, s, gtotal,
+                                   (const uint32_t *)t->tile_len.get(), gsrc, skey, sval, rb_bits, (uint32_t)row_block, t->tile_key,
+                                   nullptr, nullptr, nullptr, flag);
+                CSX_LAUNCH_CHECK();
+                CSX_HIP(hipStreamSynchronize(s));
             }
-            (void)hipMemsetAsync(t->tile_val, 0, (size_t)ngroups * TL_GROUP * sizeof(double), s);
-            hipLaunchKernelGGL(k_group_info, dim3(tb), dim3(256), 0, s, ntiles, nslab, sptr, gptr, (uint32_t *)t->tile_len.get());
-            hipLaunchKernelGGL(k_interleave, dim3((unsigned)(((int64_t)A->nnz + 255) / 256)), dim3(256), 0, s,
-                               (int64_t)A->nnz, stid, sptr, gptr, skey, sval, t->tile_key, t->tile_val);
-            if (k24)
-                hipLaunchKernelGGL(k_interleave24, dim3((unsigned)(((int64_t)A->nnz + 255) / 256)), dim3(256), 0, s,
-                                   (int64_t)A->nnz, stid, sptr, gptr, skey, rb_bits, t->tile_key24, t->tile_base);
-        }
-        hipLaunchKernelGGL(k_rb_group_ptr, dim3((unsigned)((nrb + 256) / 256)), dim3(256), 0, s, nrb, nslab, gptr,
-                           t->tile_ptr);
-        CSX_LAUNCH_CHECK();
-        CSX_HIP(hipStreamSynchronize(s));
+        }
     }
     A->tiled = std::move(t);
 #ifndef CSX_ABLATION
@@ -668,3 +741,30 @@
 }
 
 }
+
+using namespace csx;
+
+extern "C" int csx_gaxpy_plan_arrays(csx_handle_t hA, int which, void *dst, int64_t cap_bytes, int64_t *bytes_out) {
+    CSX_TRY(require_ready());
+    Csc *A = csc(hA);
+    if (!A || !A->tiled || which < 0 || which > 4 || cap_bytes < 0) return CSX_EINVAL;
+    const TiledPlan *t = A->tiled.get();
+    const bool k24 = (bool)t->tile_key24;
+    const void *src = nullptr;
+    int64_t bytes = 0;
+    switch (which) {
+        case 0: src = t->tile_ptr.get(), bytes = ((int64_t)t->nrb + 1) * 4; break;
+        case 1: src = t->tile_len.get(), bytes = t->ngroups * 4; break;
+        case 2: src = k24 ? (const void *)t->tile_key24.get() : (const void *)t->tile_key.get(), bytes = t->ngroups * TL_GROUP * (k24 ? 3 : 4); break;
+        case 3: src = t->tile_base.get(), bytes = k24 ? t->ngroups * 16 : 0; break;
+        default: src = t->tile_val.get(), bytes = t->ngroups * TL_GROUP * 8; break;
+    }
+    if (bytes_out) *bytes_out = bytes;
+    if (!dst) return CSX_OK;
+    if (cap_bytes < bytes) return CSX_EINVAL;
+    if (bytes > 0) {
+        CSX_HIP(hipMemcpyAsync(dst, src, (size_t)bytes, hipMemcpyDeviceToHost, ctx().stream));
+        CSX_HIP(hipStreamSynchronize(ctx().stream));
+    }
+    return CSX_OK;
+}
diff --git a/csparse.py_amd/csrc/csx_internal.h b/csparse.py_amd/csrc/csx_internal.h
--- a/csparse.py_amd/csrc/csx_internal.h
+++ b/csparse.py_amd/csrc/csx_internal.h
@@ -307,6 +307,7 @@
     int32_t expand_n;
     int32_t *out_ptr;
     int32_t nkeys;
+    int presorted_low_bits;
 };
 int stable_sort_by_key_ex(const uint32_t *key, const uint32_t *a, const double *v, int64_t count, uint32_t key_limit,
                           uint32_t *out_key, uint32_t *out_a, double *out_v, const SortExtra *ex);
diff --git a/csparse.py_amd/csrc/csx_sort.hip b/csparse.py_amd/csrc/csx_sort.hip
--- a/csparse.py_amd/csrc/csx_sort.hip
+++ b/csparse.py_amd/csrc/csx_sort.hip
@@ -640,14 +640,29 @@
     if (count <= 0) return optr ? suffix_min_i32(optr, (int64_t)ex->nkeys + 1) : CSX_OK;
     int bits = 1;
     while (bits < 32 && (1ull << bits) < (unsigned long long)key_limit) bits++;
-    const int passes = (bits + 7) / 8;
+    int low = ex ? ex->presorted_low_bits : 0;
+    if (low < 0 || (low > 0 && xp)) return CSX_EINVAL;
+    if (low > bits) low = bits;
+    if (low > 0 && (uint64_t)key_limit <= (1ull << low)) low = bits;
+    const int sbits = bits - low;
+    const int passes = (sbits + 7) / 8;
+    if (passes == 0) {
+        g_sort_info.bits = bits;
+        g_sort_info.count = count;
+        g_sort_info.key_misalign = (int64_t)((reinterpret_cast<uintptr_t>(key) & 15) / sizeof(uint32_t));
+        if (out_key) CSX_HIP(hipMemcpyAsync(out_key, key, (size_t)count * sizeof(uint32_t), hipMemcpyDeviceToDevice, s));
+        if (a) CSX_HIP(hipMemcpyAsync(out_a, a, (size_t)count * sizeof(uint32_t), hipMemcpyDeviceToDevice, s));
+        if (v) CSX_HIP(hipMemcpyAsync(out_v, v, (size_t)count * sizeof(double), hipMemcpyDeviceToDevice, s));
+        if (optr) CSX_TRY(boundaries_from_sorted(key, count, ex->nkeys, optr));
+        return CSX_OK;
+    }
     const uint32_t nblocks = (uint32_t)((count + RS_TILE - 1) / RS_TILE);
     uint32_t chunk = (nblocks + RS_CHUNK_DIV - 1) / RS_CHUNK_DIV;
     if (chunk < RS_CHUNK_MIN) chunk = RS_CHUNK_MIN;
     const uint32_t nchunks = (nblocks + chunk - 1) / chunk;
     const bool has_a = a != nullptr || xp != nullptr, has_v = v != nullptr;
     const bool packed = has_a && has_v;
-    const int w0 = bits / passes + (0 < bits % passes ? 1 : 0);
+    const int w0 = sbits / passes + (0 < sbits % passes ? 1 : 0);
     const bool k16 = xp != nullptr && packed && passes == 3 && optr != nullptr && out_key == nullptr && bits - w0 <= 16 &&
                      (uint64_t)ex->expand_n <= (1ull << (32 - w0)) && ctx().opt.sort_short_keys;
     SortInfo &info = g_sort_info;
@@ -700,10 +715,10 @@
     g.nblocks = nblocks;
     g.flat = ablation_env("CSX_SORT_FLAT") ? 1 : 0;
     bool in_aos = false;
-    int shift = 0;
+    int shift = low;
     for (int ps = 0; ps < passes; ps++) {
         const bool last = ps == passes - 1;
-        const int width = bits / passes + (ps < bits % passes ? 1 : 0);
+        const int width = sbits / passes + (ps < sbits % passes ? 1 : 0);
         const bool out_aos = packed && !last;
         g.shift = shift;
         g.mask = (1u << width) - 1u;
@@ -940,10 +955,11 @@
     return guard_verdict(dp.intact(), "csx_prim_boundaries");
 }
 
-extern "C" int csx_prim_sort(uint32_t *key, uint32_t *a, double *v, int64_t count, uint32_t key_limit, uint32_t *out_key,
-                             uint32_t *out_a, double *out_v, int32_t *expand_ptr, int32_t expand_n, int32_t *out_ptr, int32_t nkeys,
-                             int misalign_words) {
+static int prim_sort(uint32_t *key, uint32_t *a, double *v, int64_t count, uint32_t key_limit, uint32_t *out_key, uint32_t *out_a,
+                     double *out_v, int32_t *expand_ptr, int32_t expand_n, int32_t *out_ptr, int32_t nkeys, int misalign_words,
+                     int low_bits) {
     if (count < 0 || (count > 0 && !key) || misalign_words < 0 || misalign_words > 3) return CSX_EINVAL;
+    if (low_bits < 0 || low_bits > 32 || (low_bits > 0 && expand_ptr)) return CSX_EINVAL;
     if (((a || expand_ptr) && !out_a) || (v && !out_v)) return CSX_EINVAL;
     if (a && expand_ptr) return CSX_EINVAL;
     if (expand_ptr && (expand_n < 1 || !pointers_ok(expand_ptr, expand_n, count))) return CSX_EINVAL;
@@ -972,9 +988,10 @@
     if (with_a) CSX_TRY(doa.put(out_a, cnt));
     if (v) CSX_TRY(dov.put(out_v, cnt));
     if (out_ptr) CSX_TRY(dop.put(out_ptr, (size_t)nkeys + 1));
-    const SortExtra ex{expand_ptr ? dxp.get() : nullptr, expand_n, out_ptr ? dop.d.get() : nullptr, nkeys};
+    const SortExtra ex{expand_ptr ? dxp.get() : nullptr, expand_n, out_ptr ? dop.d.get() : nullptr, nkeys, low_bits};
     CSX_TRY(stable_sort_by_key_ex(dk, a ? da.get() : nullptr, v ? dv.get() : nullptr, count, key_limit, out_key ? dok.d.get() : nullptr,
-                                  with_a ? doa.d.get() : nullptr, v ? dov.d.get() : nullptr, (expand_ptr || out_ptr) ? &ex : nullptr));
+                                  with_a ? doa.d.get() : nullptr, v ? dov.d.get() : nullptr,
+                                  (expand_ptr || out_ptr || low_bits) ? &ex : nullptr));
     CSX_TRY(to_host(key, (const uint32_t *)dk, cnt));
     if (a) CSX_TRY(to_host(a, (const uint32_t *)da.get(), cnt));
     if (v) CSX_TRY(to_host(v, (const double *)dv.get(), cnt));
@@ -987,3 +1004,15 @@
     return guard_verdict((!out_key || dok.intact()) && (!with_a || doa.intact()) && (!v || dov.intact()) && (!out_ptr || dop.intact()),
                          "csx_prim_sort");
 }
+
+extern "C" int csx_prim_sort(uint32_t *key, uint32_t *a, double *v, int64_t count, uint32_t key_limit, uint32_t *out_key,
+                             uint32_t *out_a, double *out_v, int32_t *expand_ptr, int32_t expand_n, int32_t *out_ptr, int32_t nkeys,
+                             int misalign_words) {
+    return prim_sort(key, a, v, count, key_limit, out_key, out_a, out_v, expand_ptr, expand_n, out_ptr, nkeys, misalign_words, 0);
+}
+
+extern "C" int csx_prim_sort_presorted(uint32_t *key, uint32_t *a, double *v, int64_t count, uint32_t key_limit, uint32_t *out_key,
+                                       uint32_t *out_a, double *out_v, int32_t *out_ptr, int32_t nkeys, int misalign_words,
+                                       int low_bits) {
+    return prim_sort(key, a, v, count, key_limit, out_key, out_a, out_v, nullptr, 0, out_ptr, nkeys, misalign_words, low_bits);
+}
diff --git a/include/csx.h b/include/csx.h
--- a/include/csx.h
+++ b/include/csx.h
@@ -70,6 +70,7 @@
 int csx_gaxpy_plan_shape(csx_handle_t A, int *shape, double *ms4);
 int csx_gaxpy_plan_geometry(csx_handle_t A, int64_t *info);
 int csx_gaxpy_plan_groups(csx_handle_t A, int32_t *groups);
+int csx_gaxpy_plan_arrays(csx_handle_t A, int which, void *dst, int64_t cap_bytes, int64_t *bytes_out);
 int csx_gaxpy_host(int32_t m, int32_t n, const int32_t *p, const int32_t *i, const double *x, const double *xv,
                    double *yv);
 int csx_gaxpy_block(csx_handle_t A, csx_handle_t X, csx_handle_t Y, int32_t nrhs, int mode);
@@ -97,6 +98,8 @@
 int csx_prim_boundaries(uint32_t *sorted_key, int64_t count, int32_t nkeys, int32_t *ptr, int misalign_words);
 int csx_prim_sort(uint32_t *key, uint32_t *a, double *v, int64_t count, uint32_t key_limit, uint32_t *out_key, uint32_t *out_a,
                   double *out_v, int32_t *expand_ptr, int32_t expand_n, int32_t *out_ptr, int32_t nkeys, int misalign_words);
+int csx_prim_sort_presorted(uint32_t *key, uint32_t *a, double *v, int64_t count, uint32_t key_limit, uint32_t *out_key,
+                            uint32_t *out_a, double *out_v, int32_t *out_ptr, int32_t nkeys, int misalign_words, int low_bits);
 int csx_prim_sort_info(int64_t *out, int32_t cap);
 
 int csx_multiply(csx_handle_t A, csx_handle_t B, csx_handle_t *out);
```

After: 5772 GB/s, median of 6. No clear change (+0.2%).
